# crowsonkb/style_transfer

Hardware: AMD Instinct MI355X
Metric: tile-iterations/sec, VGG-19 2048px/1024-tile (fwd+bwd, Gram/content losses, regularizers, Adam step) (higher is better)
Workload: dtype f32 (fp16x2-split MFMA, fp32 accumulate)

## Files before the change

include/stx.h:

```cpp
#ifndef STX_H_
#define STX_H_

#include <stddef.h>
#include <stdint.h>

#ifdef __cplusplus
extern "C" {
#endif

typedef struct stx_engine stx_engine;

typedef enum stx_status {
    STX_OK = 0,
    STX_ERR_ARG = -1,
    STX_ERR_HIP = -2,
    STX_ERR_STATE = -3,
    STX_ERR_UNSUPPORTED = -4,
    STX_ERR_NOMEM = -5
} stx_status;

typedef enum stx_mem { STX_HOST = 0, STX_DEVICE = 1 } stx_mem;

typedef enum stx_layer_type {
    STX_LAYER_INPUT = 0, STX_LAYER_CONV = 1, STX_LAYER_RELU = 2, STX_LAYER_POOL = 3
} stx_layer_type;

typedef enum stx_pool_mode { STX_POOL_MAX = 0, STX_POOL_AVE = 1 } stx_pool_mode;

typedef struct stx_layer_desc {
    const char *name;
    int type;
    const char *bottom;
    const char *top;
    int num_output;
    int kernel_size;
    int pad;
    int stride;
    int pool_mode;
} stx_layer_desc;

const char *stx_version(void);
const char *stx_last_error(void);
int stx_reread_env(void);
int stx_device_count(int *count);
int stx_device_name(int device, char *buf, size_t buf_len);

int stx_engine_create(int device, const stx_layer_desc *layers, int n_layers, stx_engine **out);
int stx_engine_create_shared(stx_engine *primary, stx_engine **out);
void stx_engine_destroy(stx_engine *e);
int stx_set_conv_weights(stx_engine *e, const char *conv_layer, const float *weights,
                         const float *bias, int mem);
int stx_sync(stx_engine *e);
int stx_fence(stx_engine *e, unsigned long long *ticket);
int stx_fence_wait(stx_engine *e, unsigned long long ticket);
int stx_engine_wait(stx_engine *e, stx_engine *other);
typedef enum stx_query {
    STX_Q_SHARED_ENGINES = 0,
    STX_Q_TARGET_UPLOADS = 1,
    STX_Q_TARGET_BYTES = 2,
    STX_Q_WEIGHT_BYTES = 3,
    STX_Q_TILE_EVALS = 4,
    STX_Q_PEERS_WITHOUT_ACCESS = 5,
    STX_Q_TILE_IO_DIRECT = 6,
    STX_Q_INJECT_SPECIALISED = 7,
    STX_Q_INJECT_VARIANTS = 8
} stx_query;
int stx_engine_query(stx_engine *e, int what, double *value);
int stx_engine_device(stx_engine *e, int *device);
int stx_engine_stream(stx_engine *e, void **hip_stream);

int stx_malloc(stx_engine *e, size_t bytes, void **dev_ptr);
int stx_free(stx_engine *e, void *dev_ptr);
int stx_memset_async(stx_engine *e, void *dev_ptr, int value, size_t bytes);
int stx_memcpy_async(stx_engine *e, void *dst, int dst_mem, const void *src, int src_mem,
                     size_t bytes);

typedef struct stx_content_target {
    int content_index;
    const char *layer;
    int channels, height, width;
    const float *features;
    int mem;
} stx_content_target;

typedef struct stx_style_target {
    int style_index;
    const char *layer;
    int channels;
    const float *gram;
    int mem;
} stx_style_target;

int stx_set_contents_and_styles(stx_engine *e, const stx_content_target *contents, int n_contents,
                                const stx_style_target *styles, int n_styles);

typedef struct stx_style_mask {
    int style_index;
    int H, W;
    const float *mask;
    int mem;
} stx_style_mask;
int stx_set_style_masks(stx_engine *e, const stx_style_mask *masks, int n);

int stx_set_content_mask(stx_engine *e, const float *mask, int H, int W, int mem);

typedef struct stx_stat_target {
    const char *layer;
    int channels;
    const float *mean;
    const float *sd;
    int mem;
    double weight;
} stx_stat_target;
int stx_set_stat_targets(stx_engine *e, const stx_stat_target *targets, int n);

typedef struct stx_nnfm_target {
    const char *layer;
    int channels;
    int rows;
    const float *bank;
    int mem;
    double weight;
} stx_nnfm_target;
int stx_set_nnfm_targets(stx_engine *e, const stx_nnfm_target *targets, int n);

typedef struct stx_nnfm_patch_target {
    const char *layer;
    int channels;
    int patch;
    int rows;
    const float *bank;
    int mem;
    double weight;
} stx_nnfm_patch_target;
int stx_set_nnfm_patch_targets(stx_engine *e, const stx_nnfm_patch_target *targets, int n);

typedef struct stx_nnfm_knn_target {
    const char *layer;
    int channels;
    int patch;
    int k;
    int rows;
    const float *bank;
    int mem;
    double weight;
} stx_nnfm_knn_target;
int stx_set_nnfm_knn_targets(stx_engine *e, const stx_nnfm_knn_target *targets, int n);

typedef struct stx_nnfm_cover_target {
    const char *layer;
    int channels;
    int patch;
    int k;
    int rows;
    const float *bank;
    int mem;
    double weight;
    float cover;
} stx_nnfm_cover_target;
int stx_set_nnfm_cover_targets(stx_engine *e, const stx_nnfm_cover_target *targets, int n);

#define STX_NNFM_MAX_SEGMENTS 8
typedef struct stx_nnfm_guided_target {
    const char *layer;
    int channels;
    int k;
    int segments;
    const int *seg_rows;
    const float *bank;
    int mem;
    double weight;
} stx_nnfm_guided_target;
int stx_set_nnfm_guided_targets(stx_engine *e, const stx_nnfm_guided_target *targets, int n,
                                const float *const *masks, int segments, int H, int W, int mask_mem);

struct stx_swd_target {
    const char *layer;
    int channels;
    int dirs;
    int quantiles;
    const float *V;
    const float *Tq;
    int mem;
    double weight;
};
int stx_set_swd_targets(stx_engine *e, const struct stx_swd_target *targets, int n);

struct stx_selfsim_target {
    const char *layer;
    int points;
    double weight;
};
int stx_set_selfsim_targets(stx_engine *e, const struct stx_selfsim_target *targets, int n);

int stx_features_tile(stx_engine *e, const float *img, int img_mem, int th, int tw,
                      const char *const *layers, int n_layers, float *const *out, int out_mem);

typedef struct stx_tap {
    const char *layer;
    double layer_weight;
    int is_content;
    double content_weight;
    int is_style;
    double style_weight;
    int is_dd;
    double dd_weight;
} stx_tap;

int stx_sc_grad_tile(stx_engine *e, const float *img, int img_mem, int th, int tw,
                     const int roll_xy[2], const int start_yx[2], const stx_tap *taps, int n_taps,
                     double *loss_out, float *grad_out, int grad_mem, int sync_now);

int stx_tile_buffers(stx_engine *e, int th, int tw, float **tile_in, float **grad_out);

int stx_gram_matrix(stx_engine *e, const float *feat, int feat_mem, int channels, int hw,
                    float *gram_out, int gram_mem);

int stx_feature_stats(stx_engine *e, const float *feat, int feat_mem, int channels, int hw,
// ... 145 lines not shown
```

style_transfer_amd/csrc/common.h:

```cpp
#pragma once

#include <hip/hip_runtime.h>

#include <vector>

#include <cstdarg>
#include <cstdio>
#include <functional>
#include <string>

#include "stx.h"

namespace stx {

constexpr float kEps = 1.1920928955078125e-07f;

void set_error(const char *fmt, ...);

const char *sw_env(const char *name);
void sw_reread();

#define STX_HIP(call)                                                                       \
    do {                                                                                    \
        hipError_t err__ = (call);                                                          \
        if (err__ != hipSuccess) {                                                          \
            ::stx::set_error("%s:%d: %s failed: %s", __FILE__, __LINE__, #call,            \
                             hipGetErrorString(err__));                                     \
            return STX_ERR_HIP;                                                             \
        }                                                                                   \
    } while (0)

#define STX_CHECK_LAUNCH()                                                                  \
    do {                                                                                    \
        hipError_t err__ = hipGetLastError();                                               \
        if (err__ != hipSuccess) {                                                          \
            ::stx::set_error("%s:%d: kernel launch failed: %s", __FILE__, __LINE__,        \
                             hipGetErrorString(err__));                                     \
            return STX_ERR_HIP;                                                             \
        }                                                                                   \
    } while (0)

#define STX_TRY(expr)                                                                       \
    do {                                                                                    \
        int rc__ = (expr);                                                                  \
        if (rc__ != STX_OK) return rc__;                                                    \
    } while (0)

inline int ceil_div(int a, int b) { return (a + b - 1) / b; }
inline int pooled_len(int n) { return n >= 2 ? (n - 2 + 1) / 2 + 1 : 1; }
constexpr int kBlocks = 1024;
inline int blocks_for(size_t n) {
    const size_t b = (n + 255) / 256;
    return b < (size_t)kBlocks ? (int)b : kBlocks;
}
#ifdef __HIPCC__
__device__ __forceinline__ float wave_sum_f(float v) {
#pragma unroll
    for (int off = 32; off > 0; off >>= 1) v += __shfl_down(v, off, 64);
    return v;
}

template <int NV>
__device__ __forceinline__ void block_partials(float (&v)[NV], float *partials) {
    __shared__ float red[NV][4];
#pragma unroll
    for (int k = 0; k < NV; ++k) {
        const float s = wave_sum_f(v[k]);
        if ((threadIdx.x & 63) == 0) red[k][threadIdx.x >> 6] = s;
    }
    __syncthreads();
    if (threadIdx.x == 0) {
#pragma unroll
        for (int k = 0; k < NV; ++k)
            partials[k * gridDim.x + blockIdx.x] = red[k][0] + red[k][1] + red[k][2] + red[k][3];
    }
}

__device__ __forceinline__ unsigned pool_max_code(float v00, float v01, float v10, float v11, bool hx,
                                                  bool hy) {
    unsigned arg = 0;
    float best = v00;
    if (hx && v01 > best) best = v01, arg = 1;
    if (hy && v10 > best) best = v10, arg = 2;
    if (hx && hy && v11 > best) best = v11, arg = 3;
    return arg | (best > 0.f ? 4u : 0u);
}
__device__ __forceinline__ unsigned pool_ave_code(float v00, float v01, float v10, float v11, bool hx,
                                                  bool hy) {
    return (v00 > 0.f ? 1u : 0u) | (hx && v01 > 0.f ? 2u : 0u) | (hy && v10 > 0.f ? 4u : 0u) |
           (hx && hy && v11 > 0.f ? 8u : 0u);
}
#endif


enum ConvEpilogue {
    kEpiForward = 0,
    kEpiDgrad = 1,
    kEpiSymm = 2,
    kEpiDgradInject = 3,
    kEpiPartial = 4
};

struct ContentWindow {
    int C, fh, fw;
    int ch, cw;
    int oy, ox;
    int sy, sx;
};

struct ConvInject {
    const float *sgrad = nullptr, *s_abs_sum = nullptr;
    float s_coef = 0.f;
    const float *content = nullptr, *c_sums = nullptr, *feat = nullptr;
    float c_coef = 0.f;
    ContentWindow win{};
};

struct ConvProblem {
    const float *x;
    const float *w;
    float *y;
    const float *bias;
    const float *mask;
    float *partials;
    int K, M, H, W;
    int ksize;
    int relu;
    int epilogue;
    ConvInject inject;
    unsigned char *pool_codes = nullptr;
    unsigned char *in_codes = nullptr;
    const unsigned char *mask_codes = nullptr;
    unsigned char *out_codes = nullptr;
    bool wants_codes = false;
    bool skip_y = false;
    float *pool_out = nullptr;
    int pool_mode = 0;
    float *splitk_ws = nullptr;
    size_t splitk_ws_floats = 0;
    long long *clock_out = nullptr;
    const unsigned *x_amax = nullptr;
    unsigned *y_amax = nullptr;
    const unsigned char *pin_codes = nullptr;
    int pin_mode = 0;
    bool pin_mask = false;
    int *variant_out = nullptr;
#ifdef STX_EXPERIMENT_BF3
    const void *x_split = nullptr;
#endif
};

enum class ConvFamily { Direct, Wino2, H2 };

struct ConvConfig {
    ConvFamily family;
    int id;
    int bm;
    int kc;
    int pr, pc;
    int threads;
    size_t lds_bytes;
};

ConvConfig conv_pick_config(int ksize, int K, int M, int H, int W);
ConvConfig conv_config_by_id(int id);
bool direct_takes_inject(const ConvConfig &cfg);
int conv_num_workgroups(const ConvConfig &cfg, int M, int H, int W);
size_t conv_packed_floats(const ConvConfig &cfg, int K, int M, int ksize);
int conv_pack_weights(hipStream_t s, const float *w_caffe, int Mo, int Ko, int ksize,
                      int transpose_flip, const ConvConfig &cfg, float *packed);
int conv_launch(hipStream_t s, const ConvConfig &cfg, const ConvProblem &p, bool packed_weights);
int direct_splitk_factor(const ConvConfig &cfg, const ConvProblem &p, bool packed_weights);

int splitk_reduce_launch(hipStream_t s, const ConvProblem &p, int ksplit);
int splitk_reduce_items_launch(hipStream_t s, const ConvProblem &p, const ConvConfig &cfg, int slices,
                               int item_base, int items);
__host__ __device__ inline void wino2_item_tiles(int lt, int m_tiles, int n_patches, int &pt, int &mt) {
    pt = lt / m_tiles;
    mt = lt - pt * m_tiles;
    if (m_tiles == 8 && (n_patches & 7) == 0) {
        const int g = lt >> 5, r = lt & 31;
        mt = (g & 1) * 4 + (r & 3);
        pt = (g >> 1) * 8 + (r >> 2);
    }
}

struct WinoArgs {
    const float *x;
    const float *w;
    float *y;
    const float *bias;
    const float *mask;
    int K, M, H, W;
    int n_chunks, tiles_x, tiles_y, m_tiles, ksplit;
    int w_tile_stride;
    int x_bytes, w_bytes;
    int relu;
    ConvInject inj;
    float *pool_out;
    int pool_mode;
    unsigned char *pool_codes;
    int skip_y = 0;
    unsigned char *out_codes = nullptr;
    unsigned char *in_codes = nullptr;
    const unsigned char *mask_codes = nullptr;
    long long *clock_out = nullptr;
    int item_base = 0;
    const unsigned *x_amax = nullptr;
    unsigned *y_amax = nullptr;
    const unsigned char *pin_codes = nullptr;
    int pin_mode = 0, pin_mask = 0;
#ifdef STX_EXPERIMENT_BF3
    int vp_rows = 0, vp_tp = 0;
#endif
};

bool conv_first_usable(int K, int M, int ksize);
int conv_first_workgroups(int H, int W);
int conv_first_launch(hipStream_t s, const float *x, const float *w_caffe, const float *bias, float *y,
                      int K, int H, int W, int relu, float *gram_partials, unsigned *y_amax = nullptr);

ConvConfig wino2_config(int geometry = 0);
int wino2_pick_geometry(int H, int W);
size_t wino2_packed_floats(int K, int M);
int wino2_pack_weights(hipStream_t s, const float *w_caffe, int Mo, int Ko, int transpose_flip,
                       float *packed);
int wino2_launch(hipStream_t s, const ConvConfig &cfg, const ConvProblem &p, int ksplit);
bool wino2_fuses_pool(const ConvProblem &p);
bool wino2_uses_relu_codes(const ConvProblem &p, int ksplit);
bool wino2_writes_out_codes(const ConvConfig &cfg, const ConvProblem &p);
int wino2_splitk_factor(const ConvConfig &cfg, const ConvProblem &p);
struct Wino2Tail { int items, slices; };
Wino2Tail wino2_tail_split(const ConvConfig &cfg, const ConvProblem &p);
int wino2_max_slices(const ConvConfig &cfg, const ConvProblem &p);

constexpr int kAmaxSlots = 64;
ConvConfig h2_config(int mb, int pb = 1);
ConvConfig h2_pick_config(const ConvProblem &p);
bool h2_usable(const ConvProblem &p);
size_t h2_packed_floats(int K, int M);
int h2_pack_weights(hipStream_t s, const float *w_caffe, int Mo, int Ko, int transpose_flip, float *packed);
int h2_launch(hipStream_t s, const ConvConfig &cfg, const ConvProblem &p, int ksplit);
enum { kH2Style = 1, kH2Content = 2, kH2MaskNibbles = 4, kH2MaskBlob = 8 };
int h2_variant(const ConvProblem &p, int pin, bool split);
int h2_launch_variant(hipStream_t s, const WinoArgs &a, int n_wg, int cfg_id, int pin, int var);
int h2_splitk_factor(const ConvConfig &cfg, const ConvProblem &p);
bool h2_fuses_pool(const ConvProblem &p);
bool h2_takes_pooled_input(const ConvConfig &cfg, const ConvProblem &p);
int absmax_launch(hipStream_t s, const float *x, size_t n, unsigned *slots);

size_t conv_small_packed_floats(int K);
int conv_small_pack(hipStream_t s, const float *w_caffe, int Mo, int Ko, int transpose_flip,
                    float *packed);
int conv_small_launch(hipStream_t s, const float *x, const float *packed, float *y,
                      const float *mask, int K, int M, int H, int W);

bool conv_h2_enabled();
struct ConvTuner { int device; hipStream_t stream; hipEvent_t ev0, ev1; std::function<int(const ConvConfig &, const float **)> bank; };
int conv_choose(const ConvProblem &p, bool winograd, const ConvTuner *tuner, ConvConfig *out);
struct ConvBank { int key; size_t floats; std::function<int(hipStream_t, const float *w_caffe, float *packed)> pack; };
ConvBank conv_bank(const ConvConfig &cfg, int dir, int Mo, int Ko, int ksize);
ConvBank conv_small_bank(int Mo, int Ko);
int conv_dispatch(hipStream_t s, const ConvConfig &cfg, const ConvProblem &p, double *flop_algorithmic,
                  double *flop_issued);
int conv_splitk_factor(const ConvConfig &cfg, const ConvProblem &p);
size_t conv_splitk_floats(const ConvConfig &cfg, const ConvProblem &p);
bool conv_takes_clock(const ConvConfig &cfg);
bool conv_fuses_pool(const ConvConfig &cfg, const ConvProblem &p);
bool conv_writes_pool_codes(const ConvConfig &cfg);
bool conv_reads_x_amax(const ConvConfig &cfg);
bool conv_leaves_y_amax(const ConvConfig &cfg);
bool conv_takes_inject(const ConvConfig &cfg);
bool conv_takes_pooled_input(const ConvConfig &cfg, const ConvProblem &p);
bool conv_uses_relu_codes(const ConvConfig &cfg, const ConvProblem &p, int ksplit);
bool conv_writes_out_codes(const ConvConfig &cfg, const ConvProblem &p, int ksplit);

int pool_forward_launch(hipStream_t s, const float *x, int C, int H, int W, int mode, float *y,
                        unsigned char *codes = nullptr);
int pool_backward_codes_launch(hipStream_t s, const float *dy, const unsigned char *codes, int C,
                               int H, int W, int mode, bool relu_mask, float *dx);
int pool_backward_launch(hipStream_t s, const float *dy, const float *x, int C, int H, int W,
                         int mode, bool relu_mask, float *dx);

struct GramPlan {
    int C, HW, splits, tiles;
    int parts;
    size_t partial_floats;
};
GramPlan gram_plan(int C, int HW);
bool gram_h2_usable(const float *feat, int C, int HW);
int gram_partials_launch(hipStream_t s, const float *feat, const GramPlan &plan, float *partials,
                         const unsigned *f_amax = nullptr);
int gram_finish_blocks(const GramPlan &plan);
int gram_finish_launch(hipStream_t s, const float *partials, const GramPlan &plan, float *gram_out,
                       const float *target, float *dsym, float *sumsq, unsigned short *pieces = nullptr,
                       const unsigned *f_amax = nullptr, float *block_out = nullptr);

size_t symm_pieces_elems(int C);
int symm_num_workgroups(int C, int HW);
bool symm_bf3_usable(const float *feat, const float *out, int C, int HW);
bool symm_h2_usable(const float *feat, const float *out, int C, int HW);
int symm_h2_launch(hipStream_t s, const float *feat, const float *dsym, const unsigned *d_amax, int n_damax,
                   const unsigned *f_amax, float *out, float *partials, int C, int HW);
int symm_bf3_launch(hipStream_t s, const float *feat, const float *dsym, unsigned short *pieces,
                    bool pieces_ready, float *out, float *partials, int C, int HW);

#ifdef __HIPCC__
__device__ __forceinline__ int content_origin_y(const ContentWindow &w) { return w.oy - w.sy; }
__device__ __forceinline__ int content_origin_x(const ContentWindow &w) { return w.ox - w.sx; }
__device__ __forceinline__ size_t content_index(const ContentWindow &w, int c, int y, int x) {
    int yy = (content_origin_y(w) + y) % w.ch;
    int xx = (content_origin_x(w) + x) % w.cw;
    if (yy < 0) yy += w.ch;
    if (xx < 0) xx += w.cw;
    return ((size_t)c * w.ch + yy) * w.cw + xx;
}
#endif

struct SumJob {
    const float *src;
    int n;
    float *dst;
};
int sum_jobs_launch(hipStream_t s, const SumJob *jobs, int n_jobs);
int content_sums_launch(hipStream_t s, const float *feat, const float *content,
                        const ContentWindow &win, float *sums , std::vector<SumJob> *defer = nullptr);
int inject_style_launch(hipStream_t s, float *diff, const float *sgrad, size_t n,
                        const float *abs_sum, float coef, bool accumulate, unsigned *y_amax = nullptr);
int inject_content_launch(hipStream_t s, float *diff, const float *feat, const float *content,
                          const ContentWindow &win, const float *sums, float coef, bool accumulate,
                          unsigned *y_amax = nullptr);
int relu_inplace_launch(hipStream_t s, float *x, size_t n);
int sum_partials_launch(hipStream_t s, const float *partials, int n, float *out);
int sum_partials2_launch(hipStream_t s, const float *a, int na, float *out_a, const float *b, int nb,
                         float *out_b);

constexpr int kMaskParts = 1024;
constexpr int kMaskSgradParts = 2048;
int mask_map_launch(hipStream_t s, const float *mask, int H, int W, int scale, float *out);
int mask_apply_launch(hipStream_t s, const float *feat, const float *map, const ContentWindow &win, float *fm,
                      float *m2_partials, int *n_parts);
int mask_target_launch(hipStream_t s, const float *gs, int C, const float *m2_partials, int n_parts, int HW,
                       float *out, float *a_out);
int mask_sgrad_launch(hipStream_t s, float *sgrad, const float *map, const ContentWindow &win, const float *a,
                      float *partials, int *n_parts);

constexpr int kContentMaskParts = 1024;
int content_mask_mean_launch(hipStream_t s, const float *map, const ContentWindow &win, float *a_out);
int content_mask_term_launch(hipStream_t s, const float *feat, const float *content, const float *map,
                             const ContentWindow &win, const float *a, float *sgrad, float *partials,
                             int *n_parts);

constexpr int kStatSlice = 16384;
constexpr float kStatEps = 1e-5f;
int stat_slices(int HW);
size_t stat_scratch_floats(int C, int HW);
int stat_partials_launch(hipStream_t s, const float *feat, int C, int HW, float *partials);
int stat_finish_launch(hipStream_t s, const float *partials, int C, int HW, const float *MU, const float *SD,
                       float *table, float *e_out, float *mean_out, float *sd_out);
int stat_grad_launch(hipStream_t s, const float *feat, int C, int HW, const float *table, float *sgrad,
                     float *abs_partials, int *n_parts);

constexpr int kSwdBlock = 8192;
constexpr int kSwdMaxDirs = 4096, kSwdMaxQuantiles = 65536, kSwdMaxPixels = 1 << 22;
int swd_padded(int n);
int swd_check(const char *who, int C, long long n, int D, int Q);
int swd_e_parts(int n, int D);
size_t swd_scratch_floats(int C, int n, int D);
size_t swd_work_floats(int n, int D);
int swd_project_launch(hipStream_t s, const float *feat, int C, int n, const float *V, int D, void *records);
int swd_sort_launch(hipStream_t s, void *records, int n, int D);
int swd_finish_launch(hipStream_t s, void *records, int n, int D, const float *Tq, int Q, float *G, int *rank_out,
                      float *e_parts);
int swd_sort_passes(int n);
int swd_grad_launch(hipStream_t s, const float *V, const float *G, int C, int n, int D, float *sgrad, float *abs_parts,
                    int *n_parts);
int swd_quantiles_launch(hipStream_t s, const void *records, int n, int D, int Q, float *out);

constexpr int kSelfsimMaxPoints = 4096;
constexpr float kSelfsimEps = 1e-6f;
struct SelfsimGrid {
    int g, gh, gw, N;
};
SelfsimGrid selfsim_grid(int h, int w, int points);
int selfsim_check(const char *who, int C, int points);
struct SelfsimSource {
    const float *p;
    int mh, mw, oy, ox;
};
struct SelfsimScratch {
    float *rows;
    float *inv_r;
    float *D;
    float *col_parts;
    float *u_parts;
    float *q;
    signed char *T;
    float *e_parts;
    float *abs_parts;
    size_t floats;
};
SelfsimScratch selfsim_scratch(float *base, int C, int N);
size_t selfsim_scratch_floats(int C, int N);
int selfsim_prepare_launch(hipStream_t s, const SelfsimSource &feat, const SelfsimSource &content, int C,
                           const SelfsimGrid &gr, const SelfsimScratch &x);
int selfsim_dist_launch(hipStream_t s, int C, int N, const SelfsimScratch &x);
int selfsim_cols_launch(hipStream_t s, int N, const SelfsimScratch &x, signed char *signs, int *n_e);
int selfsim_grad_launch(hipStream_t s, int C, int h, int w, const SelfsimGrid &gr, const SelfsimScratch &x,
                        float *sgrad, int *n_abs);

constexpr int kNnfmQ = 128, kNnfmB = 128, kNnfmK = 32, kNnfmMaxSlices = 64;
constexpr int kNnfmMaxK = 4;
struct NnfmPlan {
    int q_blocks, b_blocks, slices, blocks_per_slice;
};
NnfmPlan nnfm_plan(int n, int M);
size_t nnfm_pieces_floats(int rows, int C);
size_t nnfm_scratch_floats(int C, int n, int M, int patch = 1, int k = 1, bool cover = false);
struct NnfmCover {
    int *winner = nullptr;
    float *part_score = nullptr;
    int *part_idx = nullptr;
    int *cursor = nullptr;
    int *offsets = nullptr;
    int *unordered = nullptr;
    int *list = nullptr;
    float *cprime = nullptr;
    float *e_parts = nullptr;
// ... 140 lines not shown
```

style_transfer_amd/csrc/conv_dispatch.cpp:

```cpp
#include <algorithm>
#include <cstdlib>
#include <cstring>
#include <map>
#include <mutex>

#include "common.h"

namespace stx {

static int h2_min_k(bool forward) {
    const char *env = sw_env("STX_CONV_H2"), *envb = sw_env("STX_CONV_H2_BWD");
    return forward ? (env ? atoi(env) : 64) : envb ? atoi(envb) : env && atoi(env) <= 0 ? 0 : 64;
}

bool conv_h2_enabled() {
    const char *algo = sw_env("STX_CONV_ALGO");
    if (algo && *algo) return !strncmp(algo, "h2", 2);
    return h2_min_k(true) > 0 || h2_min_k(false) > 0;
}

static bool h2_choice(const ConvProblem &p, ConvConfig *out) {
    const char *algo = sw_env("STX_CONV_ALGO");
    int force = 0;
    if (algo && *algo) {
// ... 6 lines not shown
    const int min_k = h2_min_k(p.epilogue == kEpiForward);
    if (!force && (min_k <= 0 || p.K < min_k || p.M < 64)) return false;
    if (!h2_usable(p)) return false;
    *out = force == 1 ? h2_config(1) : force == 2 ? h2_config(2) : force == 3 ? h2_config(1, 2) : h2_pick_config(p);
    return true;
}

static bool wino_choice(const ConvProblem &p, bool winograd, ConvConfig *out) {
    if (p.ksize != 3 || p.K < 8 || p.M <= 4) return false;
    const char *algo = sw_env("STX_CONV_ALGO");
    if (algo && *algo) {
        if (!strcmp(algo, "direct")) return false;
        if (!strcmp(algo, "wino2")) { *out = wino2_config(wino2_pick_geometry(p.H, p.W)); return true; }
        if (!strcmp(algo, "wino2a")) { *out = wino2_config(0); return true; }
        if (!strcmp(algo, "wino2b")) { *out = wino2_config(1); return true; }
        if (!strcmp(algo, "wino2c")) { *out = wino2_config(2); return true; }
    }
    if (!winograd || p.M <= 32) return false;
    *out = wino2_config(wino2_pick_geometry(p.H, p.W));
    return true;
}

static std::mutex g_tuned_mutex;
static std::map<std::vector<int>, int> g_tuned;

static int direct_tune(const ConvTuner &t, ConvProblem p, ConvConfig *out) {
    if (p.ksize != 3 || p.K <= 4 || p.M <= 32) return STX_OK;
    if (conv_splitk_factor(*out, p) > 1 || conv_num_workgroups(conv_config_by_id(5), p.M, p.H, p.W) < 256)
        return STX_OK;
    const std::vector<int> key = {t.device, p.ksize, p.K, p.M, p.H, p.W, p.epilogue};
    {
        std::lock_guard<std::mutex> lock(g_tuned_mutex);
        auto it = g_tuned.find(key);
        if (it != g_tuned.end()) {
            *out = conv_config_by_id(it->second);
            return STX_OK;
        }
    }
    const int candidates[] = {0, 1, 2, 5};
    float best_ms = 1e30f;
    int best = out->id;
    for (int id : candidates) {
        const ConvConfig cfg = conv_config_by_id(id);
        if (cfg.bm > 64 && p.M <= 64) continue;
        STX_TRY(t.bank(cfg, &p.w));
        STX_TRY(conv_launch(t.stream, cfg, p, true));
        STX_HIP(hipEventRecord(t.ev0, t.stream));
        for (int r = 0; r < 2; ++r) STX_TRY(conv_launch(t.stream, cfg, p, true));
        STX_HIP(hipEventRecord(t.ev1, t.stream));
        STX_HIP(hipEventSynchronize(t.ev1));
        float ms = 0.f;
        STX_HIP(hipEventElapsedTime(&ms, t.ev0, t.ev1));
        if (ms < best_ms) {
            best_ms = ms;
            best = id;
        }
    }
    {
        std::lock_guard<std::mutex> lock(g_tuned_mutex);
        g_tuned[key] = best;
    }
    *out = conv_config_by_id(best);
    return STX_OK;
}

int conv_choose(const ConvProblem &p, bool winograd, const ConvTuner *tuner, ConvConfig *out) {
    if (h2_choice(p, out) || wino_choice(p, winograd, out)) return STX_OK;
    *out = conv_pick_config(p.ksize, p.K, p.M, p.H, p.W);
    return tuner ? direct_tune(*tuner, p, out) : STX_OK;
}

enum { kSlotWino2 = 256, kSlotH2 = 512, kSlotSmall = 768 };

ConvBank conv_bank(const ConvConfig &cfg, int dir, int Mo, int Ko, int ks) {
    const int M = dir ? Ko : Mo, K = dir ? Mo : Ko;
    switch (cfg.family) {
        case ConvFamily::Direct:
            return {dir * 1024 + cfg.id, conv_packed_floats(cfg, K, M, ks),
                    [=](hipStream_t s, const float *w, float *out) { return conv_pack_weights(s, w, Mo, Ko, ks, dir, cfg, out); }};
        case ConvFamily::Wino2:
            return {dir * 1024 + kSlotWino2, wino2_packed_floats(K, M),
                    [=](hipStream_t s, const float *w, float *out) { return wino2_pack_weights(s, w, Mo, Ko, dir, out); }};
        case ConvFamily::H2:
            return {dir * 1024 + kSlotH2, h2_packed_floats(K, M),
                    [=](hipStream_t s, const float *w, float *out) { return h2_pack_weights(s, w, Mo, Ko, dir, out); }};
    }
    return {};
}

ConvBank conv_small_bank(int Mo, int Ko) {
    return {1024 + kSlotSmall, conv_small_packed_floats(Mo),
            [=](hipStream_t s, const float *w, float *out) { return conv_small_pack(s, w, Mo, Ko, 1, out); }};
}


int conv_dispatch(hipStream_t s, const ConvConfig &cfg, const ConvProblem &p, double *flop_algorithmic,
                  double *flop_issued) {
    const double direct = 2.0 * p.M * p.K * p.ksize * p.ksize * (double)p.H * p.W;
    *flop_algorithmic += direct;
    switch (cfg.family) {
        case ConvFamily::Direct:
            *flop_issued += direct;
            return conv_launch(s, cfg, p, true);
        case ConvFamily::Wino2:
            *flop_issued += direct * 4.0 / 9.0;
            return wino2_launch(s, cfg, p, conv_splitk_factor(cfg, p));
        case ConvFamily::H2:
            *flop_issued += direct * (6.0 / 9.0) * (3.0 / 16.0);
            return h2_launch(s, cfg, p, conv_splitk_factor(cfg, p));
    }
    return STX_ERR_ARG;
}

int conv_splitk_factor(const ConvConfig &cfg, const ConvProblem &p) {
    if (p.ksize != 3 || (p.epilogue != kEpiForward && p.epilogue != kEpiDgrad)) return 1;
    return cfg.family == ConvFamily::Wino2 ? wino2_splitk_factor(cfg, p)
           : cfg.family == ConvFamily::H2  ? h2_splitk_factor(cfg, p)
                                           : direct_splitk_factor(cfg, p, true);
}

size_t conv_splitk_floats(const ConvConfig &cfg, const ConvProblem &p) {
    int f = conv_splitk_factor(cfg, p);
    if (cfg.family == ConvFamily::Wino2 && p.ksize == 3)
        f = std::max(f, wino2_max_slices(cfg, p));
    return f > 1 ? (size_t)f * p.M * p.H * p.W : 0;
}

bool conv_takes_clock(const ConvConfig &cfg) { return cfg.family != ConvFamily::Direct; }

bool conv_fuses_pool(const ConvConfig &cfg, const ConvProblem &p) {
    const char *env = sw_env("STX_POOL_FWD_FUSE");
    if ((env && atoi(env) == 0) || cfg.family == ConvFamily::Direct || conv_splitk_factor(cfg, p) != 1) return false;
    return cfg.family == ConvFamily::H2 ? h2_fuses_pool(p) : wino2_fuses_pool(p);
}

bool conv_writes_pool_codes(const ConvConfig &cfg) { return cfg.family != ConvFamily::Direct; }

bool conv_reads_x_amax(const ConvConfig &cfg) { return cfg.family == ConvFamily::H2; }

bool conv_leaves_y_amax(const ConvConfig &cfg) {
    return cfg.family == ConvFamily::H2 || (cfg.family == ConvFamily::Wino2 && conv_h2_enabled());
}

bool conv_takes_inject(const ConvConfig &cfg) { return cfg.family != ConvFamily::Direct || direct_takes_inject(cfg); }

bool conv_takes_pooled_input(const ConvConfig &cfg, const ConvProblem &p) {
    return cfg.family == ConvFamily::H2 && h2_takes_pooled_input(cfg, p);
}

bool conv_uses_relu_codes(const ConvConfig &cfg, const ConvProblem &p, int ksplit) {
    return cfg.family == ConvFamily::Wino2 && wino2_uses_relu_codes(p, ksplit);
}

bool conv_writes_out_codes(const ConvConfig &cfg, const ConvProblem &p, int ksplit) {
    const char *env = sw_env("STX_RELU_CODES");
    if ((env && atoi(env) == 0) || cfg.family == ConvFamily::Direct) return false;
    if (p.epilogue != kEpiForward || !p.relu || !p.out_codes || ksplit > 1) return false;
    return cfg.family == ConvFamily::H2 || wino2_writes_out_codes(cfg, p);
}

}
```

style_transfer_amd/csrc/conv_first.hip:

```cpp

#include <algorithm>
#include <cstdlib>

#include "bf16x3.h"
#include "common.h"

namespace stx {

namespace {

constexpr int kFP = 128;
constexpr int kFM = 64;
constexpr int kPW = kFP + 4;
constexpr int kPatch = 12 * kPW;
constexpr int kFLd = kFP + 4;
constexpr int kTile = kFM * kFLd;
constexpr int kNT = 256;
constexpr int kPL = (9 * (kFP + 2) + kNT - 1) / kNT;

typedef float f32x16 __attribute__((ext_vector_type(16)));
typedef float f32x4 __attribute__((ext_vector_type(4)));
typedef unsigned int u32x4f __attribute__((ext_vector_type(4)));

__device__ __forceinline__ int sgpr(int v) { return __builtin_amdgcn_readfirstlane(v); }
__device__ __forceinline__ void lds_barrier() { asm volatile("s_waitcnt lgkmcnt(0)\n\ts_barrier" ::: "memory"); }

struct FirstArgs {
    const float *x;
    const float *w;
    const float *bias;
    float *y;
    float *gram;
    unsigned *y_amax;
    int K, H, W, tiles_x, n_tiles, relu, vec_store, strided;
};

}

template <bool GRAM, int STORE>
__global__ __launch_bounds__(kNT, GRAM ? 2 : 3) void conv_first_kernel(FirstArgs a) {
    constexpr int kWork = 2 * kPatch + kTile;
    static_assert(kFM * kFM <= kWork, "the Gram tile must fit the working set");
    __shared__ __attribute__((aligned(16))) float lds[kWork];
    float *const patch = lds;
    float *const tile = lds + 2 * kPatch;
    const int tid = threadIdx.x, lane = tid & 63;
    const int wave = __builtin_amdgcn_readfirstlane(tid >> 6);
    const int l31 = lane & 31, half = lane >> 5;
    const size_t HW = (size_t)a.H * a.W;

    float aw[2][18];
#pragma unroll
    for (int s = 0; s < 18; ++s) {
        const int c = 2 * (s / 9) + half, tap = s % 9;
#pragma unroll
        for (int mb = 0; mb < 2; ++mb)
            aw[mb][s] = c < a.K ? a.w[((size_t)(mb * 32 + l31) * a.K + c) * 9 + tap] : 0.f;
    }
#pragma unroll
    for (int s = 0; s < 18; ++s) asm volatile("" ::"v"(aw[0][s]), "v"(aw[1][s]));
    float bias_r[2];
#pragma unroll
    for (int mb = 0; mb < 2; ++mb) bias_r[mb] = a.bias ? a.bias[mb * 32 + l31] : 0.f;
    asm volatile("" ::"v"(bias_r[0]), "v"(bias_r[1]));

    const __amdgpu_buffer_rsrc_t rx = __builtin_amdgcn_make_buffer_rsrc(
        const_cast<float *>(a.x), 0, (int)((size_t)a.K * HW * 4), 0x00020000);
    constexpr unsigned kOob = 0x80000000u;
    int p_row[kPL], p_col[kPL], p_off[kPL];
#pragma unroll
    for (int n = 0; n < kPL; ++n) {
        const int e = tid + n * kNT;
        const int pr = e / (kFP + 2), col = e - pr * (kFP + 2);
        const int c = pr / 3, r = pr - 3 * c;
        const bool live = e < 9 * (kFP + 2) && c < a.K;
        p_row[n] = live ? r - 1 : -(1 << 28);
        p_col[n] = col - 1;
        p_off[n] = (c * a.H + r - 1) * a.W + col - 1;
    }
    auto patch_load = [&](int t, float (&preg)[kPL]) {
        const int ty = sgpr(t < 0 ? -4 : t / a.tiles_x);
        const int x0 = sgpr(t < 0 ? 0 : (t - ty * a.tiles_x) * kFP);
        const int origin = sgpr(ty * a.W + x0);
#pragma unroll
        for (int n = 0; n < kPL; ++n) {
            const bool ok = (unsigned)(ty + p_row[n]) < (unsigned)a.H && (unsigned)(x0 + p_col[n]) < (unsigned)a.W;
            const unsigned off = ok ? (unsigned)(origin + p_off[n]) * 4u : kOob;
            preg[n] = __builtin_bit_cast(float, __builtin_amdgcn_raw_buffer_load_b32(rx, off, 0, 0));
        }
    };
    int p_dst[kPL];
#pragma unroll
    for (int n = 0; n < kPL; ++n) {
        const int e = tid + n * kNT;
        const int pr = e / (kFP + 2), col = e - pr * (kFP + 2);
        p_dst[n] = e < 9 * (kFP + 2) ? pr * kPW + col : -1;
    }
    auto patch_store = [&](int buf, const float (&preg)[kPL]) {
#pragma unroll
        for (int n = 0; n < kPL; ++n)
            if (p_dst[n] >= 0) patch[buf * kPatch + p_dst[n]] = preg[n];
    };

    f32x16 g[3];
    if (GRAM) {
#pragma unroll
        for (int b = 0; b < 3; ++b)
#pragma unroll
            for (int r = 0; r < 16; ++r) g[b][r] = 0.f;
    }

    const int per_wg = a.strided ? 1 : (a.n_tiles + (int)gridDim.x - 1) / (int)gridDim.x;
    const int grid = a.strided ? (int)gridDim.x : 1;
    const int t_begin = a.strided ? (int)blockIdx.x : (int)blockIdx.x * per_wg;
    const int t_end = a.strided ? a.n_tiles : (t_begin + per_wg < a.n_tiles ? t_begin + per_wg : a.n_tiles);
    const __amdgpu_buffer_rsrc_t ry = __builtin_amdgcn_make_buffer_rsrc(
        a.y, 0, STORE == 2 ? 0 : (int)(unsigned)((size_t)kFM * HW * 4), 0x00020000);
    constexpr unsigned kOobY = 0xfffffff0u;
    const int y_ch0 = tid >> 5, y_c4 = (tid & 31) * 4;
    const unsigned y_voff = (unsigned)(((size_t)y_ch0 * HW + y_c4) * 4);
    const bool track = a.y_amax != nullptr;
    float amax = 0.f;
    auto segment = [&](int t, int buf, const float (&pin)[kPL], float (&pout)[kPL]) {
        patch_load(t + 2 * grid < t_end ? t + 2 * grid : -1, pout);
        const int ty = sgpr(t / a.tiles_x), x0 = sgpr((t - ty * a.tiles_x) * kFP);

        f32x16 acc[2];
#pragma unroll
        for (int mb = 0; mb < 2; ++mb)
#pragma unroll
            for (int r = 0; r < 16; ++r) acc[mb][r] = 0.f;
        const float *pb = patch + buf * kPatch + half * (3 * kPW) + wave * 32 + l31;
#pragma unroll
        for (int s = 0; s < 18; ++s) {
            const int q = s / 9, ky = (s % 9) / 3, kx = s % 3;
            const float xv = pb[(2 * q * 3 + ky) * kPW + kx];
            acc[0] = __builtin_amdgcn_mfma_f32_32x32x2f32(xv, aw[0][s], acc[0], 0, 0, 0);
            acc[1] = __builtin_amdgcn_mfma_f32_32x32x2f32(xv, aw[1][s], acc[1], 0, 0, 0);
        }
        const bool ragged = x0 + kFP > a.W;
        const int room = a.W - x0 - wave * 32 - 4 * half;
#pragma unroll
        for (int mb = 0; mb < 2; ++mb)
#pragma unroll
            for (int j = 0; j < 4; ++j) {
                f32x4 v = {acc[mb][4 * j], acc[mb][4 * j + 1], acc[mb][4 * j + 2], acc[mb][4 * j + 3]};
                v += bias_r[mb];
                if (a.relu) {
                    v.x = fmaxf(v.x, 0.f), v.y = fmaxf(v.y, 0.f);
                    v.z = fmaxf(v.z, 0.f), v.w = fmaxf(v.w, 0.f);
                }
                if (ragged) {
                    v.x = 8 * j + 0 < room ? v.x : 0.f, v.y = 8 * j + 1 < room ? v.y : 0.f;
                    v.z = 8 * j + 2 < room ? v.z : 0.f, v.w = 8 * j + 3 < room ? v.w : 0.f;
                }
                if (track) amax = fmaxf(fmaxf(amax, fmaxf(fabsf(v.x), fabsf(v.y))), fmaxf(fabsf(v.z), fabsf(v.w)));
                *reinterpret_cast<f32x4 *>(tile + (mb * 32 + l31) * kFLd + wave * 32 + 8 * j + 4 * half) = v;
            }
        lds_barrier();

        {
            float *const yrow = a.y + (size_t)ty * a.W + x0;
            const unsigned origin = (unsigned)sgpr((ty * a.W + x0) * 4);
            const unsigned vo4 = x0 + y_c4 < a.W ? y_voff : kOobY;
#pragma unroll
            for (int n = 0; n < kFM * (kFP / 4) / kNT; ++n) {
                const f32x4 v = *reinterpret_cast<const f32x4 *>(tile + (y_ch0 + 8 * n) * kFLd + y_c4);
                if (STORE == 2) {
                    float *const dst = yrow + (size_t)(y_ch0 + 8 * n) * HW + y_c4;
                    if (x0 + y_c4 + 0 < a.W) dst[0] = v.x;
                    if (x0 + y_c4 + 1 < a.W) dst[1] = v.y;
                    if (x0 + y_c4 + 2 < a.W) dst[2] = v.z;
                    if (x0 + y_c4 + 3 < a.W) dst[3] = v.w;
                    continue;
                }
                const unsigned so = origin + (unsigned)sgpr((int)((unsigned)(8 * n) * (unsigned)HW * 4u));
                if (STORE == 0) {
                    __builtin_amdgcn_raw_buffer_store_b128(__builtin_bit_cast(u32x4f, v), ry, vo4, so, 0);
                } else {
                    const float vs[4] = {v.x, v.y, v.z, v.w};
#pragma unroll
                    for (int i = 0; i < 4; ++i)
                        __builtin_amdgcn_raw_buffer_store_b32(__builtin_bit_cast(unsigned, vs[i]), ry,
                                                              x0 + y_c4 + i < a.W ? y_voff + 4u * i : kOobY, so, 0);
                }
            }
        }
        if (GRAM) {
#pragma unroll
            for (int st = 0; st < 2; ++st) {
                bf16x8 p[2][3];
#pragma unroll
                for (int mb = 0; mb < 2; ++mb) {
                    const float *q = tile + (mb * 32 + l31) * kFLd + wave * 32 + st * 16 + half * 8;
                    const f32x4 lo = *reinterpret_cast<const f32x4 *>(q);
                    const f32x4 hi = *reinterpret_cast<const f32x4 *>(q + 4);
                    const float xv[8] = {lo.x, lo.y, lo.z, lo.w, hi.x, hi.y, hi.z, hi.w};
                    split3_bf16(xv, p[mb][0], p[mb][1], p[mb][2]);
                }
                g[0] = mfma_split6(p[0], p[0], g[0]);
                g[1] = mfma_split6(p[1], p[0], g[1]);
                g[2] = mfma_split6(p[1], p[1], g[2]);
            }
        }
        if (t + grid < t_end) patch_store(buf ^ 1, pin);
        lds_barrier();
    };

    for (int i = tid; i < 2 * kPatch; i += kNT) patch[i] = 0.f;
    lds_barrier();
    float pa[kPL], pb2[kPL];
    const int t0 = t_begin;
    if (t0 < t_end) {
        patch_load(t0, pa);
        patch_store(0, pa);
    }
    if (t0 + grid < t_end) patch_load(t0 + grid, pa);
    lds_barrier();
    for (int t = t0; t < t_end; t += 2 * grid) {
        segment(t, 0, pa, pb2);
        if (t + grid < t_end) segment(t + grid, 1, pb2, pa);
    }

    if (track) {
#pragma unroll
        for (int d = 32; d >= 1; d >>= 1) amax = fmaxf(amax, __shfl_xor(amax, d));
        lds_barrier();
        if (lane == 0) lds[wave] = amax;
        lds_barrier();
        if (tid == 0)
            atomicMax(a.y_amax + (blockIdx.x & (kAmaxSlots - 1)),
                      __builtin_bit_cast(unsigned, fmaxf(fmaxf(lds[0], lds[1]), fmaxf(lds[2], lds[3]))));
    }
    if (GRAM) {
        lds_barrier();
        float *const red = lds;
#pragma unroll 1
        for (int w = 0; w < 4; ++w) {
            if (wave == w) {
#pragma unroll
                for (int r = 0; r < 16; ++r) {
                    const int row = (r & 3) + 8 * (r >> 2) + 4 * half;
                    float *q0 = red + row * kFM + l31, *q1 = red + (32 + row) * kFM + l31;
                    q0[0] = w == 0 ? g[0][r] : q0[0] + g[0][r];
                    if (w == 0) q0[32] = 0.f;
                    q1[0] = w == 0 ? g[1][r] : q1[0] + g[1][r];
                    q1[32] = w == 0 ? g[2][r] : q1[32] + g[2][r];
                }
            }
            lds_barrier();
        }
        float *out = a.gram + (size_t)blockIdx.x * (kFM * kFM);
#pragma unroll
        for (int n = 0; n < 4; ++n) {
            const int e = tid + kNT * n;
            reinterpret_cast<float4 *>(out)[e] = reinterpret_cast<const float4 *>(red)[e];
        }
    }
}

bool conv_first_usable(int K, int M, int ksize) {
    const char *env = sw_env("STX_CONV_FIRST_FUSED");
    if (env && atoi(env) == 0) return false;
    return ksize == 3 && K >= 1 && K <= 3 && M == kFM;
}

int conv_first_workgroups(int H, int W) {
    const long tiles = (long)H * ceil_div(W, kFP);
    return (int)std::min<long>(tiles, 512);
}
static int conv_first_plain_workgroups(int H, int W) {
    const long tiles = (long)H * ceil_div(W, kFP);
    const char *env = sw_env("STX_FIRST_WGS");
    return (int)std::min<long>(tiles, env ? atoi(env) : 768);
}

int conv_first_launch(hipStream_t s, const float *x, const float *w_caffe, const float *bias, float *y,
                      int K, int H, int W, int relu, float *gram_partials, unsigned *y_amax) {
    if (4.0 * K * (double)H * W >= 2147483648.0) {
        set_error("conv_first_launch: a %d x %d plane is beyond the buffer-addressing limit", H, W);
        return STX_ERR_UNSUPPORTED;
    }
    FirstArgs a;
    a.x = x;
    a.w = w_caffe;
    a.bias = bias;
    a.y = y;
    a.gram = gram_partials;
    a.y_amax = y_amax;
    a.K = K;
    a.H = H;
    a.W = W;
    a.tiles_x = ceil_div(W, kFP);
    a.n_tiles = H * a.tiles_x;
    a.relu = relu;
    a.vec_store = W % 4 == 0 && (reinterpret_cast<uintptr_t>(y) & 15) == 0;
    const int grid = gram_partials ? conv_first_workgroups(H, W) : conv_first_plain_workgroups(H, W);
    {
        const char *env = sw_env("STX_FIRST_STRIDED");
        a.strided = env && atoi(env) != 0;
    }
    const int store = 4.0 * kFM * (double)H * W >= 4294967280.0 ? 2 : a.vec_store ? 0 : 1;
#define STX_FIRST(G, S) conv_first_kernel<G, S><<<grid, kNT, 0, s>>>(a)
    if (gram_partials) {
        if (store == 0) STX_FIRST(true, 0);
        else if (store == 1) STX_FIRST(true, 1);
        else STX_FIRST(true, 2);
    } else {
        if (store == 0) STX_FIRST(false, 0);
        else if (store == 1) STX_FIRST(false, 1);
        else STX_FIRST(false, 2);
    }
#undef STX_FIRST
    STX_CHECK_LAUNCH();
    return STX_OK;
}

}
```

style_transfer_amd/csrc/conv_h2.hip:

```cpp

#include <algorithm>
#include <cstdlib>
#include <type_traits>

#include "common.h"
#include "f16x2.h"

#ifndef STX_H2_SKIP
#define STX_H2_SKIP 0
#endif

namespace stx {

namespace {

typedef _Float16 f16x8 __attribute__((ext_vector_type(8)));
typedef float f32x16 __attribute__((ext_vector_type(16)));
typedef float f32x4 __attribute__((ext_vector_type(4)));
typedef float f32x2 __attribute__((ext_vector_type(2)));
typedef unsigned int u32x4 __attribute__((ext_vector_type(4)));
typedef unsigned int u32x3 __attribute__((ext_vector_type(3)));
typedef unsigned int u32x2v __attribute__((__vector_size__(2 * sizeof(unsigned int))));

constexpr int KC = 16;
constexpr int NT = 512;
constexpr int PC = 32, TX = PC / 2;
constexpr int EX_BYTES = 4 * 2 * 4 * 4 * 64 * 16;
template <int PB>
struct Geo {
    static constexpr int PR = 8 * PB;
    static constexpr int XR = PR + 2;
    static constexpr int RT = XR * TX;
    static constexpr int V_PIECE = RT * 32;
    static constexpr int V_BYTES = 4 * 2 * V_PIECE;
    static constexpr int FULL = RT * 4 / 512;
    static constexpr int NU = FULL + 1;
    static constexpr size_t kLds = (EX_BYTES > 2 * V_BYTES ? EX_BYTES : 2 * V_BYTES) + 64;
};
constexpr int FRAG = 1024;
constexpr int U_KY = 4 * 2 * FRAG;
constexpr int U_BLK = 3 * U_KY;
constexpr int kHeaderFloats = 64;

__device__ __forceinline__ int sgpr(int v) { return __builtin_amdgcn_readfirstlane(v); }

template <int I, int N, typename F>
__device__ __forceinline__ void static_for(F &&f) {
    if constexpr (I < N) {
        f(std::integral_constant<int, I>{});
        static_for<I + 1, N>(f);
    }
}

__device__ __forceinline__ void lds_barrier() {
    asm volatile("s_waitcnt lgkmcnt(0)\n\ts_barrier" ::: "memory");
}


}

#ifdef STX_H2_TIMING
__device__ long long g_h2_timing[8][8];
__device__ long long g_h2_epi[8][8];
#define STX_H2_STAMP(i) if (pass == 0) t_epi[i] = clock64()
#else
#define STX_H2_STAMP(i)
#endif

template <int EPI, int MB, int PB, int PIN, int VAR = 0>
__global__ __launch_bounds__(NT) void conv_h2_kernel(WinoArgs a) {
    static_assert(VAR == 0 || EPI == kEpiDgradInject, "variants are of the injecting epilogue");
    static_assert(VAR == 0 || (((VAR & 3) == 1 || (VAR & 3) == 2) && ((VAR >> 2) == 1 || (VAR >> 2) == 2)), "h2_variant's codes");
    const bool inj_style = VAR ? (VAR & 1) != 0 : a.inj.sgrad != nullptr;
    const bool inj_content = VAR ? (VAR & 2) != 0 : a.inj.content != nullptr;
    const bool mask_nibbles = VAR ? (VAR >> 2) == 1 : a.mask_codes != nullptr;
    const bool mask_blob = VAR ? (VAR >> 2) == 2 : !a.mask_codes && a.mask;
    using G = Geo<PB>;
    [[maybe_unused]] constexpr int PR = G::PR, RT = G::RT, V_PIECE = G::V_PIECE, V_BYTES = G::V_BYTES, NU = G::NU, FULL = G::FULL;
    constexpr size_t kLdsBytes = G::kLds;
    constexpr int NJ = 4 * PB;
    extern __shared__ __attribute__((aligned(16))) char ldsb[];
#ifdef STX_H2_TIMING
    const long long t_start = clock64(), w_start = wall_clock64();
#endif
    constexpr int BM = 64 * MB;

    const int tid = threadIdx.x, lane = tid & 63;
    const int wave = sgpr(tid >> 6);
    const int xi = wave & 3, wh = wave >> 2;
    const int l31 = lane & 31, half = lane >> 5;

    const int m_tiles = a.m_tiles, a_tiles_x = a.tiles_x, a_tiles_y = a.tiles_y, a_H = a.H, a_W = a.W;
    const int a_n_chunks = a.n_chunks, a_ksplit = a.ksplit, a_item_base = a.item_base, a_x_bytes = a.x_bytes,
              a_w_bytes = a.w_bytes;
    const float *const a_x = a.x, *const a_w = a.w;
    asm volatile("" ::"s"(m_tiles), "s"(a_tiles_x), "s"(a_tiles_y), "s"(a_H), "s"(a_W), "s"(a_n_chunks), "s"(a_ksplit),
                 "s"(a_item_base), "s"(a_x_bytes), "s"(a_w_bytes), "s"(a_x), "s"(a_w));
    const int nb = gridDim.x, xcd = blockIdx.x & 7, slot_x = blockIdx.x >> 3;
    const int q8 = nb >> 3, r8 = nb & 7;
    const int L = (xcd < r8 ? xcd * (q8 + 1) : r8 * (q8 + 1) + (xcd - r8) * q8) + slot_x;
    const int kslice = sgpr(EPI == kEpiPartial ? L % a_ksplit : 0);
    const int Lt = sgpr(EPI == kEpiPartial ? a_item_base + L / a_ksplit : L);
    int ptile, mtile;
    wino2_item_tiles(Lt, m_tiles, a_tiles_x * a_tiles_y, ptile, mtile);
    ptile = sgpr(ptile);
    mtile = sgpr(mtile);
    const int c_begin = sgpr(EPI == kEpiPartial ? 2 * (kslice * (a_n_chunks >> 1) / a_ksplit) : 0);
    const int c_end = sgpr(EPI == kEpiPartial ? 2 * ((kslice + 1) * (a_n_chunks >> 1) / a_ksplit) : a_n_chunks);
    const int y0 = sgpr((ptile / a_tiles_x) * PR);
    const int x0 = sgpr((ptile % a_tiles_x) * PC);
    const int m0 = mtile * BM;
    const int HW = a_H * a_W;
    const unsigned HW4 = (unsigned)HW * 4u;
    const int pih = (a_H + 1) >> 1, piw = (a_W + 1) >> 1;
    const unsigned XP4 = PIN ? (unsigned)(pih * piw) * 4u : HW4;

    constexpr unsigned kOob = 0x80000000u;
    const __amdgpu_buffer_rsrc_t rx = __builtin_amdgcn_make_buffer_rsrc(
        const_cast<float *>(a_x), 0, a_x_bytes, 0x00020000);
    const __amdgpu_buffer_rsrc_t rw = __builtin_amdgcn_make_buffer_rsrc(
        const_cast<float *>(a_w), 0, a_w_bytes, 0x00020000);
    const __amdgpu_buffer_rsrc_t rcx = __builtin_amdgcn_make_buffer_rsrc(
        const_cast<unsigned char *>(a.pin_codes), 0, PIN ? (a_x_bytes >> 2) + 3 : 0, 0x00020000);

    float sv = 0.f, out_scale = 0.f, out_scale2 = 0.f;
    auto read_scales = [&]() __attribute__((always_inline)) {
        typedef const __attribute__((address_space(4))) unsigned *kconst_u32;
        const kconst_u32 slots = (kconst_u32)(uintptr_t)a.x_amax, header = (kconst_u32)(uintptr_t)a_w;
        unsigned amax_bits = 0;
#pragma unroll
        for (int i = 0; i < kAmaxSlots; ++i) amax_bits = max(amax_bits, slots[i]);
        const int es = sgpr(h2_scale_exp(amax_bits));
        const int ew = sgpr((int)header[(a_w_bytes >> 2) + 1]);
        sv = pow2f(es);
        const int eo = -es - ew, eo1 = eo < -126 ? -126 : eo > 127 ? 127 : eo;
        out_scale = pow2f(eo1), out_scale2 = pow2f(eo - eo1);
    };

    const bool edge = x0 == 0 || x0 + PC + 2 > a.W;
    unsigned xvoff[NU], v_dst[NU];
    bool left[NU], ok2[NU], ok3[NU];
#pragma unroll
    for (int n = 0; n < NU; ++n) {
        const int u = tid + n * NT;
        const int rt = n < FULL ? u >> 2 : 128 * FULL + (tid >> 4);
        const int ch0 = n < FULL ? (u & 3) * 4 : tid & 15;
        const int st_r = rt / TX, st_t = rt % TX;
        const int st_y = y0 - 1 + st_r, st_x = x0 + 2 * st_t - 1;
        left[n] = st_x < 0;
        ok2[n] = st_x + 2 < a.W, ok3[n] = st_x + 3 < a.W;
        xvoff[n] = kOob;
        if (PIN) {
            const int w0 = (x0 >> 1) + st_t - 1;
            if ((unsigned)st_y < (unsigned)a.H && st_x + 1 < a.W)
                xvoff[n] = (unsigned)(ch0 * pih * piw + (st_y >> 1) * piw + (left[n] ? 0 : w0)) * 4u +
                           (unsigned)(st_y & 1) + ((st_y | 1) < a.H ? 2u : 0u);
        } else if ((unsigned)st_y < (unsigned)a.H && st_x + 1 < a.W)
            xvoff[n] = (unsigned)(ch0 * HW + st_y * a.W + (left[n] ? 0 : st_x)) * 4u;
        v_dst[n] = (unsigned)(rt * 32 + ((ch0 * 2) ^ ((st_t & 8) << 1)));
    }

    f32x4 xr[FULL][4], xe;
    auto x_fetch = [&](int n, unsigned soff) __attribute__((always_inline)) {
        if constexpr (PIN) {
            unsigned xo = xvoff[n];
            asm volatile("" : "+v"(xo));
            const u32x3 g = __builtin_amdgcn_raw_buffer_load_b96(rx, xo & ~3u, soff, 0);
            const unsigned cw = __builtin_amdgcn_raw_buffer_load_b32(rcx, xo >> 2, soff >> 2, 0);
            return __builtin_bit_cast(f32x4, u32x4{g.x, g.y, g.z, cw});
        } else {
            return __builtin_bit_cast(f32x4, __builtin_amdgcn_raw_buffer_load_b128(rx, xvoff[n], soff, 0));
        }
    };
    auto x_load = [&](int n, int chunk) __attribute__((always_inline)) {
        const unsigned xs = (unsigned)sgpr(chunk * KC) * XP4;
        if (n == FULL) {
            xe = x_fetch(FULL, xs);
        } else {
#pragma unroll
            for (int i = 0; i < 4; ++i) xr[n][i] = x_fetch(n, xs + (unsigned)i * XP4);
        }
    };
    auto border = [&](f32x4 d, int n) __attribute__((always_inline)) {
        f32x4 e;
        e.x = left[n] ? 0.f : d.x;
        e.y = left[n] ? d.x : d.y;
        e.z = left[n] ? d.y : d.z;
        e.w = left[n] ? d.z : d.w;
        e.z = ok2[n] ? e.z : 0.f;
        e.w = ok3[n] ? e.w : 0.f;
        return e;
    };
    struct Unpool {
        unsigned cmask, t_l, t_r, sh;
        float q0;
        bool ok4;
    };
    auto unpool_setup = [&](int n) __attribute__((always_inline)) {
        Unpool r;
        const unsigned keep = a.pin_mask ? 4u : 0u;
        r.cmask = keep | 3u;
        unsigned xo = xvoff[n], vd = v_dst[n];
        asm volatile("" : "+v"(xo), "+v"(vd));
        r.sh = (xo & 1u) << 1;
        r.t_l = keep | r.sh, r.t_r = r.t_l | 1u;
        r.q0 = (xo & 2u) ? 0.25f : 0.5f;
        r.ok4 = x0 + 2 * (int)((vd >> 5) & 15u) + 3 < a.W;
        return r;
    };
    auto unpool_channel = [&](f32x4 d, int n, const Unpool &r, bool fix) __attribute__((always_inline)) {
        constexpr bool is_max = PIN == 1 + STX_POOL_MAX;
        float g0 = d.x, g1 = d.y, g2 = d.z;
        const float dw = d.w;
        unsigned cw = __builtin_bit_cast(unsigned, dw);
        if (fix) {
            g2 = left[n] ? g1 : g2, g1 = left[n] ? g0 : g1;
            cw = left[n] ? cw << 8 : cw;
        }
        float p0, p1, p2, p3;
        if (is_max) {
            const unsigned b0 = cw & r.cmask, b1 = (cw >> 8) & r.cmask, b2 = (cw >> 16) & r.cmask;
            p0 = b0 == r.t_r ? g0 : 0.f;
            p1 = b1 == r.t_l ? g1 : 0.f;
            p2 = b1 == r.t_r ? g1 : 0.f;
            p3 = b2 == r.t_l ? g2 : 0.f;
        } else {
            const float q1 = fix && !ok2[n] ? r.q0 + r.q0 : r.q0, q2 = fix && !r.ok4 ? r.q0 + r.q0 : r.q0;
// ... 22 lines not shown
            __builtin_amdgcn_sched_barrier(0);
        }
    };
    auto component = [](f32x4 d, int c) __attribute__((always_inline)) {
        return c == 0 ? d.x - d.z : c == 1 ? d.y + d.z : c == 2 ? d.z - d.y : d.y - d.w;
    };
    auto piece = [&](int n, int c, char *vbuf, bool fix) __attribute__((always_inline)) {
        if (!PIN && c == 0 && fix) {
            asm volatile("");
#pragma unroll
            for (int i = 0; i < 4; ++i) xr[n][i] = border(xr[n][i], n);
        }
        float v[4];
#pragma unroll
        for (int i = 0; i < 4; ++i) v[i] = component(xr[n][i], c);
        unsigned h0, h1, l0, l1;
        if (STX_H2_SKIP & 64) {
            h0 = __builtin_bit_cast(unsigned, v[0]), h1 = __builtin_bit_cast(unsigned, v[1]);
            l0 = __builtin_bit_cast(unsigned, v[2]), l1 = __builtin_bit_cast(unsigned, v[3]);
        } else {
            asm("v_fma_mixlo_f16 %0, %4, %8, 0\n\t"
                "v_fma_mixhi_f16 %0, %5, %8, 0\n\t"
                "v_fma_mixlo_f16 %1, %6, %8, 0\n\t"
                "v_fma_mixhi_f16 %1, %7, %8, 0\n\t"
                "v_fma_mixlo_f16 %2, %4, %8, -%0 op_sel:[0,0,0] op_sel_hi:[0,0,1]\n\t"
                "v_fma_mixhi_f16 %2, %5, %8, -%0 op_sel:[0,0,1] op_sel_hi:[0,0,1]\n\t"
                "v_fma_mixlo_f16 %3, %6, %8, -%1 op_sel:[0,0,0] op_sel_hi:[0,0,1]\n\t"
                "v_fma_mixhi_f16 %3, %7, %8, -%1 op_sel:[0,0,1] op_sel_hi:[0,0,1]"
                : "=&v"(h0), "=&v"(h1), "=&v"(l0), "=&v"(l1)
                : "v"(v[0]), "v"(v[1]), "v"(v[2]), "v"(v[3]), "v"(sv));
        }
        if (STX_H2_SKIP & 32) {
            asm volatile("" :: "v"(h0), "v"(h1), "v"(l0), "v"(l1));
            return;
        }
        *reinterpret_cast<u32x2v *>(vbuf + v_dst[n] + (c * 2 + 0) * V_PIECE) = u32x2v{h0, h1};
        *reinterpret_cast<u32x2v *>(vbuf + v_dst[n] + (c * 2 + 1) * V_PIECE) = u32x2v{l0, l1};
    };
    auto piece_one = [&](int c, char *vbuf, bool fix) __attribute__((always_inline)) {
        if (!PIN && c == 0 && fix) {
            asm volatile("");
            xe = border(xe, FULL);
        }
        const float va = component(xe, c), vb = component(xe, c + 1);
        unsigned ha, hb, la, lb;
        asm("v_fma_mixlo_f16 %0, %4, %6, 0\n\t"
            "v_fma_mixlo_f16 %1, %5, %6, 0\n\t"
            "v_fma_mixlo_f16 %2, %4, %6, -%0 op_sel:[0,0,0] op_sel_hi:[0,0,1]\n\t"
            "v_fma_mixlo_f16 %3, %5, %6, -%1 op_sel:[0,0,0] op_sel_hi:[0,0,1]"
            : "=&v"(ha), "=&v"(hb), "=&v"(la), "=&v"(lb)
            : "v"(va), "v"(vb), "v"(sv));
        if (STX_H2_SKIP & 32) {
            asm volatile("" :: "v"(ha), "v"(hb), "v"(la), "v"(lb));
            return;
        }
        char *dst = vbuf + v_dst[FULL];
        *reinterpret_cast<unsigned short *>(dst + (c * 2 + 0) * V_PIECE) = (unsigned short)ha;
        *reinterpret_cast<unsigned short *>(dst + (c * 2 + 1) * V_PIECE) = (unsigned short)la;
        *reinterpret_cast<unsigned short *>(dst + (c * 2 + 2) * V_PIECE) = (unsigned short)hb;
        *reinterpret_cast<unsigned short *>(dst + (c * 2 + 3) * V_PIECE) = (unsigned short)lb;
    };
    auto stage_all = [&](int n, int buf) __attribute__((always_inline)) {
        char *vbuf = ldsb + buf * V_BYTES;
        if (PIN) unpool(n, edge);
        if (n == FULL) {
            piece_one(0, vbuf, edge);
            piece_one(2, vbuf, edge);
        } else {
#pragma unroll
            for (int c = 0; c < 4; ++c) piece(n, c, vbuf, edge);
        }
    };

    const unsigned a_voff = (unsigned)(xi * 2 * FRAG + lane * 16);
    const unsigned w_blk0 = (unsigned)(mtile * 2 * MB + wh * MB);
    constexpr bool LEAN = MB * PB == 2;
    f16x8 af[LEAN ? 2 : 3][MB][2];
    auto a_load = [&](int aslot, int ky, int chunk) __attribute__((always_inline)) {
#pragma unroll
        for (int b = 0; b < MB; ++b) {
            const unsigned ws = (unsigned)sgpr(
                (int)(((w_blk0 + b) * (unsigned)a.n_chunks + (unsigned)chunk) * U_BLK + (unsigned)ky * U_KY));
#pragma unroll
            for (int q = 0; q < 2; ++q)
                af[aslot][b][q] = __builtin_bit_cast(
                    f16x8, __builtin_amdgcn_raw_buffer_load_b128(rw, a_voff + q * FRAG, ws, 0));
        }
    };

    f32x16 acc[MB][NJ];
#pragma unroll
    for (int b = 0; b < MB; ++b)
#pragma unroll
        for (int j = 0; j < NJ; ++j)
#pragma unroll
            for (int r = 0; r < 16; ++r) acc[b][j][r] = 0.f;

    const unsigned b_base = (unsigned)(xi * 2 * V_PIECE + ((l31 >> 4) * 2 * TX + (l31 & 15)) * 32 +
                                       ((half * 16) ^ ((l31 & 8) << 1)));
    f16x8 bq[2][2];
    auto b_read = [&](int slot, int buf, int blk) __attribute__((always_inline)) {
        const int j = blk % NJ, ky = blk / NJ;
        const char *vb = ldsb + buf * V_BYTES + b_base + (4 * (j >> 1) + (j & 1) + ky) * TX * 32;
#pragma unroll
        for (int q = 0; q < 2; ++q) bq[slot][q] = *reinterpret_cast<const f16x8 *>(vb + q * V_PIECE);
    };

#ifdef STX_H2_TIMING
    const long long t_p0 = clock64();
#endif
    static_for<0, NU>([&](auto n_c) __attribute__((always_inline)) { x_load(decltype(n_c)::value, c_begin); });
    if (LEAN) {
        a_load(0, 0, c_begin);
    } else {
#pragma unroll
        for (int ky = 0; ky < 3; ++ky) a_load(ky, ky, c_begin);
    }
    __builtin_amdgcn_sched_barrier(0);
    read_scales();
#pragma unroll
    for (int b = 0; b < MB; ++b)
#pragma unroll
        for (int j = 0; j < NJ; ++j) asm volatile("" : "+v"(acc[b][j]));
    float s_scale = 0.f, c_scale = 0.f;
    if (EPI == kEpiDgradInject) {
        const float n = (float)((size_t)a.M * HW);
        if (inj_style) s_scale = a.inj.s_coef * (1.0f / (a.inj.s_abs_sum[0] / n + kEps));
        if (inj_content) c_scale = a.inj.c_coef * (1.0f / (a.inj.c_sums[1] / n + kEps));
    }
    const int hh = wave & 1, mrow = (wave >> 1) & 1, rqp = wave >> 2;
    const bool weven = (a.W & 1) == 0;
    const int xx0 = x0 + 2 * (l31 & 15);
    const unsigned plane_bytes = (unsigned)a.M * HW4;
    const __amdgpu_buffer_rsrc_t ry = __builtin_amdgcn_make_buffer_rsrc(
        a.y + (EPI == kEpiPartial ? (size_t)kslice * a.M * HW : 0), 0, (int)plane_bytes, 0x00020000);
    const __amdgpu_buffer_rsrc_t rmask = __builtin_amdgcn_make_buffer_rsrc(
        const_cast<float *>(a.mask), 0, a.mask ? (int)plane_bytes : 0, 0x00020000);
    const __amdgpu_buffer_rsrc_t rsg = __builtin_amdgcn_make_buffer_rsrc(
        const_cast<float *>(a.inj.sgrad), 0, a.inj.sgrad ? (int)plane_bytes : 0, 0x00020000);
    const __amdgpu_buffer_rsrc_t rft = __builtin_amdgcn_make_buffer_rsrc(
        const_cast<float *>(a.inj.feat), 0, a.inj.feat ? (int)plane_bytes : 0, 0x00020000);
    const __amdgpu_buffer_rsrc_t rbias = __builtin_amdgcn_make_buffer_rsrc(
        const_cast<float *>(a.bias), 0, a.bias ? a.M * 4 : 0, 0x00020000);
    const int ph = (a.H + 1) >> 1, pw = (a.W + 1) >> 1;
    const __amdgpu_buffer_rsrc_t rpool = __builtin_amdgcn_make_buffer_rsrc(
        a.pool_out, 0, a.pool_out ? a.M * ph * pw * 4 : 0, 0x00020000);
    const __amdgpu_buffer_rsrc_t rcodes = __builtin_amdgcn_make_buffer_rsrc(
        a.pool_codes, 0, a.pool_codes ? a.M * ph * pw : 0, 0x00020000);
    const int cph = (a.H + 1) >> 1, cpw = (a.W + 1) >> 1;
    const __amdgpu_buffer_rsrc_t rmc = __builtin_amdgcn_make_buffer_rsrc(
        const_cast<unsigned char *>(a.mask_codes), 0, a.mask_codes ? a.M * cph * cpw : 0, 0x00020000);
    const __amdgpu_buffer_rsrc_t roc = __builtin_amdgcn_make_buffer_rsrc(
        a.out_codes, 0, a.out_codes ? a.M * cph * cpw : 0, 0x00020000);
    const int M_ = a.M;
    struct LaneRows {
        int yy;
        unsigned vo[2][2], vpool, vmc;
    };
    const float *const content = a.inj.content;
    const int cw_ch = a.inj.win.ch, cw_cw = a.inj.win.cw, cw_oy = a.inj.win.oy - a.inj.win.sy,
              cw_ox = a.inj.win.ox - a.inj.win.sx;
    auto lane_rows = [&](int pbi) __attribute__((always_inline)) {
        LaneRows r;
        r.yy = y0 + 8 * pbi + 4 * mrow + 2 * (l31 >> 4);
        const unsigned lane_base = (unsigned)((4 * half) * HW + r.yy * a.W + xx0) * 4u;
#pragma unroll
        for (int y = 0; y < 2; ++y)
#pragma unroll
            for (int e = 0; e < 2; ++e)
                r.vo[y][e] = (r.yy + y < a.H && xx0 + e < a.W) ? lane_base + (unsigned)(y * a.W + e) * 4u : kOob;
        const bool in = r.yy < a.H && xx0 < a.W;
        r.vpool = in ? (unsigned)((4 * half) * ph * pw + (r.yy >> 1) * pw + (xx0 >> 1)) * 4u : kOob;
        r.vmc = in ? (unsigned)((4 * half) * cph * cpw + (r.yy >> 1) * cpw + (xx0 >> 1)) : kOob;
        return r;
    };
    constexpr bool HOIST = !(PIN && PB == 2);
    LaneRows rows0{};
    if (HOIST) rows0 = lane_rows(0);
    auto ld2 = [&](const __amdgpu_buffer_rsrc_t &rs, const LaneRows &lr, int y, unsigned so, auto even_c)
                   __attribute__((always_inline)) {
        if (decltype(even_c)::value)
            return __builtin_bit_cast(f32x2, __builtin_amdgcn_raw_buffer_load_b64(rs, lr.vo[y][0], so, 0));
        f32x2 v;
        v.x = __builtin_bit_cast(float, __builtin_amdgcn_raw_buffer_load_b32(rs, lr.vo[y][0], so, 0));
        v.y = __builtin_bit_cast(float, __builtin_amdgcn_raw_buffer_load_b32(rs, lr.vo[y][1], so, 0));
        return v;
    };
    auto st2 = [&](const __amdgpu_buffer_rsrc_t &rs, const LaneRows &lr, int y, unsigned so, f32x2 v, auto even_c)
                   __attribute__((always_inline)) {
        if (STX_H2_SKIP & 8) {
            if (v.x == 1.2345e-30f) __builtin_amdgcn_raw_buffer_store_b32(0u, rs, lr.vo[y][0], so, 0);
            return;
        }
        if (decltype(even_c)::value) {
            __builtin_amdgcn_raw_buffer_store_b64(__builtin_bit_cast(u32x2v, v), rs, lr.vo[y][0], so, 0);
        } else {
            const float v0 = v.x, v1 = v.y;
            __builtin_amdgcn_raw_buffer_store_b32(__builtin_bit_cast(unsigned, v0), rs, lr.vo[y][0], so, 0);
            __builtin_amdgcn_raw_buffer_store_b32(__builtin_bit_cast(unsigned, v1), rs, lr.vo[y][1], so, 0);
        }
    };
    int ccol[2] = {0, 0};
    auto content_columns = [&](const LaneRows &lr) __attribute__((always_inline)) {
        if (EPI == kEpiDgradInject && inj_content) {
#pragma unroll
            for (int e = 0; e < 2; ++e) {
                const bool ok = lr.yy < a.H && xx0 < a.W;
                const int x = ok ? (xx0 + e < a.W ? xx0 + e : xx0) : (e && 1 < a.W ? 1 : 0);
                int r = (cw_ox + x) % cw_cw;
                ccol[e] = r < 0 ? r + cw_cw : r;
            }
        }
    };
    if (HOIST) content_columns(rows0);
#ifdef STX_H2_TIMING
    __builtin_amdgcn_sched_barrier(0);
    const long long t_p1 = clock64();
    asm volatile("s_waitcnt vmcnt(0)" ::: "memory");
    const long long t_p2 = clock64();
#endif
    static_for<0, NU>([&](auto n_c) __attribute__((always_inline)) {
        constexpr int n = decltype(n_c)::value;
        stage_all(n, 0);
        if (c_begin + 1 < c_end) x_load(n, c_begin + 1);
    });
#ifdef STX_H2_TIMING
    __builtin_amdgcn_sched_barrier(0);
    const long long t_p3 = clock64();
#endif
    lds_barrier();
    b_read(0, 0, 0);

    constexpr int NBLK = 3 * NJ;
    constexpr int PER_BLK = 3 * MB, SLOTS = (NBLK - 1) * PER_BLK;
    constexpr int NQ = PIN ? 5 : 4, NQ1 = PIN ? 3 : 2;
    constexpr int NP = NQ * NU;
    constexpr int STEP = (SLOTS - 2) / NP;
#ifdef STX_H2_NO_BRANCH
    const bool edge_fix = false;
#else
    const bool edge_fix = edge;
#endif
    auto run_chunk = [&](auto buf_c, int chunk, auto more_c) __attribute__((always_inline)) {
        constexpr bool MORE = decltype(more_c)::value;
        constexpr int BUF = decltype(buf_c)::value, buf = BUF;
        char *vnext = ldsb + (buf ^ 1) * V_BYTES;
        static_for<0, NBLK>([&](auto blk_c) __attribute__((always_inline)) {
            constexpr int blk = decltype(blk_c)::value;
            constexpr int ky = blk / NJ, j = blk % NJ, slot = blk & 1;
            if (blk == NBLK - 1) {
                __builtin_amdgcn_sched_barrier(0);
                lds_barrier();
            }
            __builtin_amdgcn_sched_barrier(0);
            if (blk < NBLK - 1) b_read(slot ^ 1, buf, blk + 1);
            else if (MORE) b_read(0, buf ^ 1, 0);
            static_for<0, PER_BLK>([&](auto m_c) __attribute__((always_inline)) {
                constexpr int m = decltype(m_c)::value;
                constexpr int b = m % MB, t = m / MB;
                __builtin_amdgcn_sched_barrier(0);
                constexpr int as = LEAN ? (BUF + ky) & 1 : ky;
                acc[b][j] = __builtin_amdgcn_mfma_f32_32x32x16_f16(af[as][b][t == 0 ? 1 : 0],
                                                                   bq[slot][t == 1 ? 1 : 0], acc[b][j], 0, 0, 0);
                __builtin_amdgcn_sched_barrier(0);
                constexpr int s = blk * PER_BLK + m;
                if (LEAN && j == 0 && m == 0 && !(STX_H2_SKIP & 2)) {
                    if (ky < 2) a_load(as ^ 1, ky + 1, chunk);
                    else if (MORE) a_load(as ^ 1, 0, chunk + 1);
                }
                if (MORE && !(STX_H2_SKIP & 1) && s >= 1 && (s - 1) % STEP == 0) {
                    constexpr int k = (s - 1) / STEP;
                    constexpr int n = k % NU, q = k / NU;
                    if (k < NP && PIN && q == 0) unpool(n, edge_fix);
                    else if (k < NP && n < FULL) piece(n, q - (PIN ? 1 : 0), vnext, edge_fix);
                    else if (k < NP && q < NQ1) piece_one(2 * (q - (PIN ? 1 : 0)), vnext, edge_fix);
                }
                if (MORE && !(STX_H2_SKIP & 4)) {
                    static_for<0, NU>([&](auto u_c) __attribute__((always_inline)) {
                        constexpr int u = decltype(u_c)::value;
                        if (s == 1 + (((u < FULL ? NQ : NQ1) - 1) * NU + u) * STEP + 1 && chunk + 2 < c_end)
                            x_load(u, chunk + 2);
                    });
                }
            });
            if (!LEAN && j == NJ - 1 && MORE && !(STX_H2_SKIP & 2)) a_load(ky, ky, chunk + 1);
        });
        __builtin_amdgcn_sched_barrier(0);
    };
    using yes = std::integral_constant<bool, true>;
    using no = std::integral_constant<bool, false>;
    using b0 = std::integral_constant<int, 0>;
    using b1 = std::integral_constant<int, 1>;
#ifdef STX_H2_TIMING
    const long long t_loop = clock64(), w_loop = wall_clock64();
#endif
    const bool mark = a.clock_out != nullptr && (int)blockIdx.x == (int)(gridDim.x >> 1);
    long long mark_c = 0, mark_w = 0;
    if (mark) {
        mark_c = clock64();
        mark_w = wall_clock64();
    }
    {
        int chunk = c_begin;
        for (; chunk + 2 < c_end; chunk += 2) {
            run_chunk(b0{}, chunk, yes{});
            run_chunk(b1{}, chunk + 1, yes{});
        }
        run_chunk(b0{}, chunk, yes{});
        run_chunk(b1{}, chunk + 1, no{});
    }
    if (mark) {
        const long long dc = clock64() - mark_c, dw = wall_clock64() - mark_w;
        if (tid == 0) {
            a.clock_out[0] = dw >= 100 ? dc : 0;
            a.clock_out[1] = dw >= 100 ? dw : 0;
        }
    }
#ifdef STX_H2_TIMING
    const long long t_end = clock64(), w_end = wall_clock64();
#endif

    float amax = 0.f;
    f32x4 *ex = reinterpret_cast<f32x4 *>(ldsb);

#ifdef STX_H2_TIMING
    long long t_epi[4] = {0, 0, 0, 0};
#endif
    auto epilogue_pass = [&](auto pass_c, auto even_c) __attribute__((always_inline)) {
        constexpr int pass = decltype(pass_c)::value;
        constexpr int mbi = pass % MB, pbi = pass / MB;
        const LaneRows lr = pbi == 0 && HOIST ? rows0 : lane_rows(pbi);
        if (!HOIST && pass == 0) content_columns(lr);
        int crow[2] = {0, 0};
        if (EPI == kEpiDgradInject && inj_content) {
#pragma unroll
            for (int y = 0; y < 2; ++y) {
                const bool ok = lr.yy + y < a.H && xx0 < a.W;
                int q = (cw_oy + (ok ? lr.yy + y : 0)) % cw_ch;
                crow[y] = (q < 0 ? q + cw_ch : q) * cw_cw;
            }
        }
        const int cblk = m0 + (hh * MB + mbi) * 32;
        auto chan = [&](int n) __attribute__((always_inline)) {
            const int c0 = cblk + (n & 3) + 8 * (2 * rqp + (n >> 2));
            return sgpr(c0 < M_ ? c0 : M_);
        };
        float bs[8];
        f32x2 mk[16], sg[16];
        unsigned mkb[8];
#pragma unroll
        for (int n = 0; n < 8; ++n) {
            const int c = chan(n);
            const unsigned so = (unsigned)c * HW4;
            if (EPI == kEpiForward) {
                bs[n] = a.bias ? __builtin_bit_cast(float, __builtin_amdgcn_raw_buffer_load_b32(
                                                               rbias, (unsigned)half * 16u, (unsigned)c * 4u, 0))
                               : 0.f;
            } else if (EPI != kEpiPartial) {
                if (mask_nibbles) mkb[n] = __builtin_amdgcn_raw_buffer_load_b8(rmc, lr.vmc, (unsigned)(c * cph * cpw), 0);
#pragma unroll
                for (int y = 0; y < 2; ++y) {
                    if (mask_blob && !(STX_H2_SKIP & 16)) mk[2 * n + y] = ld2(rmask, lr, y, so, even_c);
                    if (EPI == kEpiDgradInject && inj_style) sg[2 * n + y] = ld2(rsg, lr, y, so, even_c);
                }
            }
        }
        STX_H2_STAMP(0);
        __syncthreads();
        STX_H2_STAMP(1);
#pragma unroll
        for (int j = 0; j < 4; ++j)
#pragma unroll
            for (int rq = 0; rq < 4; ++rq)
                ex[(((xi * 2 + wh) * 4 + j) * 4 + rq) * 64 + lane] =
                    f32x4{acc[mbi][4 * pbi + j][4 * rq], acc[mbi][4 * pbi + j][4 * rq + 1],
                          acc[mbi][4 * pbi + j][4 * rq + 2], acc[mbi][4 * pbi + j][4 * rq + 3]};
        __syncthreads();
        STX_H2_STAMP(2);
#pragma unroll
        for (int rqi = 0; rqi < 2; ++rqi) {
            const int rq = 2 * rqp + rqi;
            f32x4 o[2][2];
#pragma unroll
            for (int s = 0; s < 2; ++s) {
                f32x4 p[4];
#pragma unroll
                for (int c = 0; c < 4; ++c) p[c] = ex[(((c * 2 + hh) * 4 + 2 * mrow + s) * 4 + rq) * 64 + lane];
                o[s][0] = (p[0] + p[1] + p[2]) * out_scale * out_scale2;
                o[s][1] = (p[1] - p[2] - p[3]) * out_scale * out_scale2;
            }
#pragma unroll
            for (int e = 0; e < 4; ++e) {
                const int n = 4 * rqi + e;
                const int c = chan(n);
                const unsigned so = (unsigned)c * HW4;
                f32x2 v[2];
#pragma unroll
                for (int y = 0; y < 2; ++y) v[y] = f32x2{o[y][0][e], o[y][1][e]};
                if (EPI == kEpiForward) {
                    if (a.bias) {
#pragma unroll
                        for (int y = 0; y < 2; ++y) v[y].x += bs[n], v[y].y += bs[n];
                    }
                    if (a.relu) {
#pragma unroll
                        for (int y = 0; y < 2; ++y) v[y].x = fmaxf(v[y].x, 0.f), v[y].y = fmaxf(v[y].y, 0.f);
                    }
                } else if (EPI != kEpiPartial) {
#pragma unroll
                    for (int y = 0; y < 2; ++y) {
                        if (mask_nibbles) {
                            const unsigned nib = mkb[n] >> (2 * y);
                            v[y].x = (nib & 1u) ? v[y].x : 0.f;
                            v[y].y = (nib & 2u) ? v[y].y : 0.f;
                        } else if (mask_blob && !(STX_H2_SKIP & 16)) {
                            v[y].x = mk[2 * n + y].x > 0.f ? v[y].x : 0.f;
                            v[y].y = mk[2 * n + y].y > 0.f ? v[y].y : 0.f;
                        }
                        if (EPI == kEpiDgradInject) {
                            if (inj_content) {
                                const f32x2 ft = ld2(rft, lr, y, so, even_c);
                                const int mm = c + 4 * half;
                                const int cm = mm < a.M ? mm : 0;
                                const float *cp = content + (size_t)cm * cw_ch * cw_cw + crow[y];
                                v[y].x += c_scale * (ft.x - cp[ccol[0]]);
                                v[y].y += c_scale * (ft.y - cp[ccol[1]]);
                            }
                            if (inj_style) {
                                v[y].x += s_scale * sg[2 * n + y].x;
                                v[y].y += s_scale * sg[2 * n + y].y;
                            }
                        }
                    }
                }
#pragma unroll
                for (int y = 0; y < 2; ++y) {
                    if (EPI != kEpiForward || !a.skip_y) st2(ry, lr, y, so, v[y], even_c);
                    if (EPI != kEpiPartial)
                        amax = fmaxf(amax, fmaxf(lr.vo[y][0] != kOob ? fabsf(v[y].x) : 0.f,
                                                 lr.vo[y][1] != kOob ? fabsf(v[y].y) : 0.f));
                }
                if (EPI == kEpiForward && a.out_codes) {
                    const unsigned nib = (lr.vo[0][0] != kOob && v[0].x > 0.f ? 1u : 0u) |
                                         (lr.vo[0][1] != kOob && v[0].y > 0.f ? 2u : 0u) |
                                         (lr.vo[1][0] != kOob && v[1].x > 0.f ? 4u : 0u) |
                                         (lr.vo[1][1] != kOob && v[1].y > 0.f ? 8u : 0u);
                    __builtin_amdgcn_raw_buffer_store_b8((unsigned char)nib, roc, lr.vmc, (unsigned)(c * cph * cpw), 0);
                }
                if (EPI == kEpiForward && a.pool_out) {
                    const bool hy = lr.yy + 1 < a.H, hx = decltype(even_c)::value || xx0 + 1 < a.W;
                    float pr;
                    if (a.pool_mode == STX_POOL_MAX) {
                        pr = hx ? fmaxf(v[0].x, v[0].y) : v[0].x;
                        if (hy) pr = hx ? fmaxf(fmaxf(pr, v[1].x), v[1].y) : fmaxf(pr, v[1].x);
                    } else {
                        pr = (v[0].x + (hx ? v[0].y : 0.f) + (hy ? v[1].x : 0.f) + (hx && hy ? v[1].y : 0.f)) *
                             (hy ? (hx ? 0.25f : 0.5f) : (hx ? 0.5f : 1.0f));
                    }
                    __builtin_amdgcn_raw_buffer_store_b32(__builtin_bit_cast(unsigned, pr), rpool, lr.vpool,
                                                          (unsigned)c * (unsigned)(ph * pw * 4), 0);
                    if (a.pool_codes) {
                        const unsigned code = a.pool_mode == STX_POOL_MAX
                                                  ? pool_max_code(v[0].x, v[0].y, v[1].x, v[1].y, hx, hy)
                                                  : pool_ave_code(v[0].x, v[0].y, v[1].x, v[1].y, hx, hy);
                        __builtin_amdgcn_raw_buffer_store_b8((unsigned char)code, rcodes, lr.vpool >> 2,
                                                             (unsigned)c * (unsigned)(ph * pw), 0);
                    }
                }
            }
        }
    };
    static_for<0, MB * PB>([&](auto pass_c) __attribute__((always_inline)) {
        [[maybe_unused]] constexpr int pass = decltype(pass_c)::value;
        if (weven) epilogue_pass(pass_c, yes{});
        else epilogue_pass(pass_c, no{});
        STX_H2_STAMP(3);
    });
    if (EPI != kEpiPartial && a.y_amax) {
#pragma unroll
        for (int d = 32; d >= 1; d >>= 1) amax = fmaxf(amax, __shfl_xor(amax, d));
        float *wmax = reinterpret_cast<float *>(ldsb + kLdsBytes - 64);
        if (lane == 0) wmax[wave] = amax;
        __syncthreads();
        if (tid == 0) {
#pragma unroll
            for (int w = 1; w < 8; ++w) amax = fmaxf(amax, wmax[w]);
            atomicMax(a.y_amax + (blockIdx.x & (kAmaxSlots - 1)), __builtin_bit_cast(unsigned, amax));
        }
    }
#ifdef STX_H2_TIMING
    if (blockIdx.x == gridDim.x - 3 && lane == 0) {
        g_h2_timing[wave][0] = t_loop - t_start, g_h2_timing[wave][1] = t_end - t_loop;
        g_h2_timing[wave][2] = clock64() - t_end;
        g_h2_timing[wave][3] = w_loop - w_start, g_h2_timing[wave][4] = w_end - w_loop;
        g_h2_timing[wave][5] = wall_clock64() - w_end;
        for (int i = 0; i < 4; ++i) g_h2_epi[wave][i] = t_epi[i] - t_end;
        g_h2_epi[wave][4] = t_p0 - t_start, g_h2_epi[wave][5] = t_p1 - t_p0, g_h2_epi[wave][6] = t_p2 - t_p1, g_h2_epi[wave][7] = t_p3 - t_p2;
    }
#endif
}

template <int EPI, int MB, int PB, int PIN = 0, int VAR = 0>
static int h2_launch_epi(hipStream_t s, const WinoArgs &args, int n_wg) {
    auto kern = conv_h2_kernel<EPI, MB, PB, PIN, VAR>;
    constexpr size_t kLdsBytes = Geo<PB>::kLds;
    hipError_t e = hipFuncSetAttribute(reinterpret_cast<const void *>(kern),
                                       hipFuncAttributeMaxDynamicSharedMemorySize, (int)kLdsBytes);
    if (e != hipSuccess) {
        set_error("hipFuncSetAttribute(lds=%zu): %s", kLdsBytes, hipGetErrorString(e));
        return STX_ERR_HIP;
    }
    kern<<<n_wg, NT, kLdsBytes, s>>>(args);
    STX_CHECK_LAUNCH();
    return STX_OK;
}

#if defined(STX_H2_VARIANTS_ONLY) || !(defined(STX_H2_SPLIT_UNITS) || defined(STX_H2_DEV_SUBSET))
int h2_launch_variant(hipStream_t s, const WinoArgs &a, int n_wg, int cfg_id, int pin, int var) {
#define STX_H2_VAR(V, P)                                                                                      \
    if (var == (V) && pin == (P))                                                                             \
        return cfg_id == 1   ? h2_launch_epi<kEpiDgradInject, 2, 1, P, V>(s, a, n_wg)                         \
               : cfg_id == 2 ? h2_launch_epi<kEpiDgradInject, 1, 2, P, V>(s, a, n_wg)                         \
                             : h2_launch_epi<kEpiDgradInject, 1, 1, P, V>(s, a, n_wg);
    STX_H2_VAR(kH2Style | kH2MaskNibbles, 0)
    STX_H2_VAR(kH2Style | kH2MaskBlob, 0)
    STX_H2_VAR(kH2Content | kH2MaskNibbles, 0)
    STX_H2_VAR(kH2Content | kH2MaskBlob, 0)
    STX_H2_VAR(kH2Style | kH2MaskNibbles, 1 + STX_POOL_MAX)
    STX_H2_VAR(kH2Style | kH2MaskBlob, 1 + STX_POOL_MAX)
    STX_H2_VAR(kH2Style | kH2MaskNibbles, 1 + STX_POOL_AVE)
    STX_H2_VAR(kH2Style | kH2MaskBlob, 1 + STX_POOL_AVE)
#undef STX_H2_VAR
    set_error("h2_launch_variant: no specialised body %d for a pooled input of kind %d", var, pin);
    return STX_ERR_UNSUPPORTED;
}
#endif
#ifndef STX_H2_VARIANTS_ONLY

__global__ __launch_bounds__(256) void absmax_kernel(const float *__restrict__ x, size_t n, unsigned *slots) {
    float m = 0.f;
    const size_t head = ((16 - (reinterpret_cast<size_t>(x) & 15)) & 15) >> 2;
    const size_t h = head < n ? head : n;
    const size_t n4 = (n - h) >> 2;
    const f32x4 *x4 = reinterpret_cast<const f32x4 *>(x + h);
    for (size_t i = blockIdx.x * (size_t)256 + threadIdx.x; i < n4; i += (size_t)gridDim.x * 256) {
        const f32x4 v = x4[i];
        m = fmaxf(fmaxf(m, fmaxf(fabsf(v.x), fabsf(v.y))), fmaxf(fabsf(v.z), fabsf(v.w)));
    }
    if (blockIdx.x == 0) {
        if (threadIdx.x < h) m = fmaxf(m, fabsf(x[threadIdx.x]));
        const size_t tail = h + (n4 << 2);
        if (tail + threadIdx.x < n && threadIdx.x < 4) m = fmaxf(m, fabsf(x[tail + threadIdx.x]));
    }
#pragma unroll
    for (int d = 32; d >= 1; d >>= 1) m = fmaxf(m, __shfl_xor(m, d));
    __shared__ float wmax[4];
    if ((threadIdx.x & 63) == 0) wmax[threadIdx.x >> 6] = m;
    __syncthreads();
    if (threadIdx.x == 0)
        atomicMax(slots + (blockIdx.x & (kAmaxSlots - 1)),
                  __builtin_bit_cast(unsigned, fmaxf(fmaxf(wmax[0], wmax[1]), fmaxf(wmax[2], wmax[3]))));
}

int absmax_launch(hipStream_t s, const float *x, size_t n, unsigned *slots) {
    STX_HIP(hipMemsetAsync(slots, 0, kAmaxSlots * sizeof(unsigned), s));
    if ((reinterpret_cast<size_t>(x) & 3) != 0) {
        set_error("absmax_launch: the array is not float-aligned");
        return STX_ERR_ARG;
    }
    const int blocks = (int)std::min<size_t>((n / 4 + 2047) / 2048 + 1, 1024);
    absmax_kernel<<<blocks, 256, 0, s>>>(x, n, slots);
    STX_CHECK_LAUNCH();
    return STX_OK;
}

size_t h2_packed_floats(int K, int M) {
    return (size_t)ceil_div(M, 32) * ceil_div(K, KC) * (U_BLK / 4) + kHeaderFloats;
}

__device__ __forceinline__ float h2_u(const float *__restrict__ w, int Ko, int transpose_flip, int m, int k,
                                      int ky, int x) {
    float g[3];
#pragma unroll
    for (int b = 0; b < 3; ++b) {
        const int t = ky * 3 + b;
        g[b] = transpose_flip ? w[((size_t)k * Ko + m) * 9 + (8 - t)] : w[((size_t)m * Ko + k) * 9 + t];
    }
    return x == 0 ? g[0] : x == 1 ? (g[0] + g[1] + g[2]) * 0.5f : x == 2 ? (g[0] - g[1] + g[2]) * 0.5f : g[2];
}

__global__ void h2_bank_max_kernel(const float *__restrict__ w, int Ko, int transpose_flip, int M, int K,
                                   unsigned *header) {
    const size_t total = (size_t)M * K * 12;
    float mx = 0.f;
    for (size_t idx = blockIdx.x * (size_t)blockDim.x + threadIdx.x; idx < total;
         idx += (size_t)gridDim.x * blockDim.x) {
        const int x = idx % 4, ky = (idx / 4) % 3;
        const size_t mk = idx / 12;
        mx = fmaxf(mx, fabsf(h2_u(w, Ko, transpose_flip, (int)(mk / K), (int)(mk % K), ky, x)));
    }
#pragma unroll
    for (int d = 32; d >= 1; d >>= 1) mx = fmaxf(mx, __shfl_xor(mx, d));
    __shared__ float wmax[4];
    if ((threadIdx.x & 63) == 0) wmax[threadIdx.x >> 6] = mx;
    __syncthreads();
    if (threadIdx.x == 0)
        atomicMax(header, __builtin_bit_cast(unsigned, fmaxf(fmaxf(wmax[0], wmax[1]), fmaxf(wmax[2], wmax[3]))));
}

__global__ void h2_pack_kernel(const float *__restrict__ w, int Ko, int transpose_flip, int M, int K,
                               int n_chunks, unsigned short *__restrict__ packed, size_t total,
                               unsigned *header) {
    const int ew = h2_scale_exp(header[0]);
    const float sw = pow2f(ew);
    if (blockIdx.x == 0 && threadIdx.x == 0) header[1] = (unsigned)ew;
    for (size_t idx = blockIdx.x * (size_t)blockDim.x + threadIdx.x; idx < total;
         idx += (size_t)gridDim.x * blockDim.x) {
        size_t r = idx;
        const int e = r % 8; r /= 8;
        const int l31 = r % 32; r /= 32;
        const int half = r % 2; r /= 2;
        const int piece = r % 2; r /= 2;
        const int x = r % 4; r /= 4;
        const int ky = r % 3; r /= 3;
        const int chunk = r % n_chunks;
        const int mblk = r / n_chunks;
        const int m = mblk * 32 + l31, k = chunk * KC + half * 8 + e;
        _Float16 out = (_Float16)0.f;
        if (m < M && k < K) {
            const float u = h2_u(w, Ko, transpose_flip, m, k, ky, x) * sw;
            const _Float16 hi = (_Float16)u;
            out = piece == 0 ? hi : (_Float16)(u - (float)hi);
        }
        packed[idx] = __builtin_bit_cast(unsigned short, out);
    }
}

int h2_pack_weights(hipStream_t s, const float *w_caffe, int Mo, int Ko, int transpose_flip, float *packed) {
    const int M = transpose_flip ? Ko : Mo;
    const int K = transpose_flip ? Mo : Ko;
    const size_t bank_floats = h2_packed_floats(K, M) - kHeaderFloats;
    unsigned *header = reinterpret_cast<unsigned *>(packed + bank_floats);
    STX_HIP(hipMemsetAsync(header, 0, kHeaderFloats * sizeof(float), s));
    h2_bank_max_kernel<<<(int)std::min<size_t>(((size_t)M * K * 12 + 255) / 256, 256), 256, 0, s>>>(
        w_caffe, Ko, transpose_flip, M, K, header);
    STX_CHECK_LAUNCH();
    const size_t total = bank_floats * 2;
    h2_pack_kernel<<<(int)std::min<size_t>((total + 255) / 256, 8192), 256, 0, s>>>(
        w_caffe, Ko, transpose_flip, M, K, ceil_div(K, KC), reinterpret_cast<unsigned short *>(packed), total,
        header);
    STX_CHECK_LAUNCH();
    return STX_OK;
}

ConvConfig h2_config(int mb, int pb) {
    const bool two = mb != 2 && pb == 2;
    return {ConvFamily::H2, mb == 2 ? 1 : two ? 2 : 0, mb == 2 ? 128 : 64, KC, two ? 16 : 8, PC, NT,
            two ? Geo<2>::kLds : Geo<1>::kLds};
}

bool h2_usable(const ConvProblem &p) {
    if (p.ksize != 3 || p.K % (2 * KC) != 0 || p.K < 2 * KC) return false;
    if (p.epilogue != kEpiForward && p.epilogue != kEpiDgrad) return false;
    if (p.epilogue == kEpiForward && (p.wants_codes || p.in_codes)) return false;
    const double xb = 4.0 * p.K * (double)p.H * p.W, yb = 4.0 * p.M * (double)p.H * p.W;
    const double wb = 4.0 * (double)h2_packed_floats(p.K, p.M);
    return xb < 2147483648.0 && yb < 2147483648.0 && wb < 2147483648.0;
}

static double h2_plan(const ConvConfig &cfg, const ConvProblem &p, int *factor) {
    const int n_pairs = p.K / (2 * KC);
    const long n = (long)ceil_div(p.M, cfg.bm) * ceil_div(p.H, cfg.pr) * ceil_div(p.W, PC);
    const double out_mb = 4e-6 * p.M * (double)p.H * p.W;
    const double t_chunk = cfg.id == 1 ? 2.75 : cfg.id == 2 ? 3.5 : 2.0, t_fixed = cfg.id != 0 ? 17.0 : 8.5;
    const bool may_split = p.epilogue == kEpiForward || p.epilogue == kEpiDgrad;
    double best_cost = 0;
    int best = 1;
    for (int f = 1; f <= 8 && (f == 1 || (may_split && n_pairs / f >= 2)); ++f) {
        const double rounds = (double)ceil_div((int)std::min<long>(n * f, 1 << 30), 256);
        double c = rounds * (2.0 * ceil_div(n_pairs, f) * t_chunk + t_fixed);
        if (f > 1) c += (f + 1) * out_mb / 3.0 + 5.0;
        if (f == 1 || c < best_cost) {
            best_cost = c;
            best = f;
        }
    }
    *factor = best;
    return best_cost;
}

int h2_splitk_factor(const ConvConfig &cfg, const ConvProblem &p) {
    int f;
    h2_plan(cfg, p, &f);
    return f;
}

ConvConfig h2_pick_config(const ConvProblem &p) {
    int f;
    ConvConfig best = h2_config(1, 1);
    double best_cost = h2_plan(best, p, &f);
    const ConvConfig cand[2] = {h2_config(2, 1), h2_config(1, 2)};
    for (int i = 0; i < 2; ++i) {
        if (i == 0 && p.M % 128 != 0) continue;
        const double c = h2_plan(cand[i], p, &f);
        if (c < best_cost) best_cost = c, best = cand[i];
    }
    return best;
}

bool h2_takes_pooled_input(const ConvConfig &cfg, const ConvProblem &p) {
    return p.epilogue == kEpiDgrad && h2_usable(p) && h2_splitk_factor(cfg, p) == 1;
}

bool h2_fuses_pool(const ConvProblem &p) {
    return p.pool_out && p.epilogue == kEpiForward && (((size_t)p.y | (size_t)p.pool_out) & 7) == 0;
}

#ifdef STX_H2_DEV_SUBSET
template __global__ void conv_h2_kernel<0, 2, 1, 0>(WinoArgs);
template __global__ void conv_h2_kernel<0, 1, 2, 0>(WinoArgs);
template __global__ void conv_h2_kernel<1, 2, 1, 0>(WinoArgs);
template __global__ void conv_h2_kernel<3, 2, 1, 0>(WinoArgs);
template __global__ void conv_h2_kernel<3, 1, 2, 1>(WinoArgs);
template __global__ void conv_h2_kernel<3, 2, 1, 0, kH2Style | kH2MaskNibbles>(WinoArgs);
template __global__ void conv_h2_kernel<3, 2, 1, 0, kH2Content | kH2MaskNibbles>(WinoArgs);
template __global__ void conv_h2_kernel<3, 1, 2, 1, kH2Style | kH2MaskBlob>(WinoArgs);
template __global__ void conv_h2_kernel<3, 2, 1, 1, kH2Style | kH2MaskNibbles>(WinoArgs);
#else
int h2_variant(const ConvProblem &p, int pin, bool split) {
    if (split || p.epilogue != kEpiDgrad) return 0;
    const bool style = p.inject.sgrad != nullptr, content = p.inject.content != nullptr;
    if (style == content) return 0;
    if (!p.mask_codes && !p.mask) return 0;
    if (content && pin) return 0;
    const char *env = sw_env("STX_H2_INJECT_GENERIC");
    if (env && atoi(env) != 0) return 0;
    return (style ? kH2Style : kH2Content) | (p.mask_codes ? kH2MaskNibbles : kH2MaskBlob);
}

int h2_launch(hipStream_t s, const ConvConfig &cfg, const ConvProblem &p, int ksplit) {
    if (!h2_usable(p) || !p.x_amax) {
        set_error("h2_launch: unsupported problem (K %d, epilogue %d, input maximum %s)", p.K, p.epilogue,
                  p.x_amax ? "given" : "missing");
        return STX_ERR_UNSUPPORTED;
    }
    WinoArgs a;
    a.x = p.x;
    a.w = p.w;
    a.y = p.y;
    a.bias = p.bias;
    a.mask = p.mask;
    a.K = p.K;
    a.M = p.M;
    a.H = p.H;
    a.W = p.W;
    a.n_chunks = p.K / KC;
    a.tiles_x = ceil_div(p.W, PC);
    a.tiles_y = ceil_div(p.H, cfg.pr);
    a.m_tiles = ceil_div(p.M, cfg.bm);
    a.ksplit = 1;
    a.w_tile_stride = 0;
    a.relu = p.relu;
    a.inj = p.inject;
    a.pool_out = nullptr;
    a.pool_codes = nullptr;
    a.pool_mode = p.pool_mode;
    a.x_bytes = (int)(4.0 * p.K * (double)p.H * p.W);
    const bool pin = p.pin_codes != nullptr;
    if (pin) {
        if (!h2_takes_pooled_input(cfg, p) || ksplit > 1) {
            set_error("h2_launch: a pooled input goes with unsplit backward launches only");
            return STX_ERR_UNSUPPORTED;
        }
        a.x_bytes = (int)(4.0 * p.K * (double)((p.H + 1) / 2) * ((p.W + 1) / 2));
        a.pin_codes = p.pin_codes;
        a.pin_mode = p.pin_mode;
        a.pin_mask = p.pin_mask ? 1 : 0;
    }
    a.w_bytes = (int)(4 * (h2_packed_floats(p.K, p.M) - kHeaderFloats));
    a.clock_out = p.clock_out;
    a.x_amax = p.x_amax;
    a.y_amax = p.y_amax;
    a.mask_codes = p.epilogue == kEpiDgrad ? p.mask_codes : nullptr;
    a.out_codes = p.epilogue == kEpiForward && p.relu ? p.out_codes : nullptr;
    const bool inject = p.epilogue == kEpiDgrad && (p.inject.sgrad || p.inject.content);
    int n_wg = a.m_tiles * a.tiles_x * a.tiles_y;
    const bool split = ksplit > 1 && p.splitk_ws && p.splitk_ws_floats >= (size_t)ksplit * p.M * p.H * p.W;
    if (split) {
        a.ksplit = ksplit;
        a.y = p.splitk_ws;
        a.y_amax = nullptr;
        a.mask_codes = nullptr;
        a.out_codes = nullptr;
        n_wg *= ksplit;
    } else if (h2_fuses_pool(p)) {
        a.pool_out = p.pool_out;
        a.pool_codes = p.pool_codes;
        a.skip_y = p.skip_y && p.pool_codes != nullptr;
    }
    const int epi = split ? kEpiPartial : inject ? kEpiDgradInject : p.epilogue;
    const int pin_kind = pin ? 1 + p.pin_mode : 0;
    const int var = h2_variant(p, pin_kind, split);
    if (p.variant_out) *p.variant_out = var;
    if (var) return h2_launch_variant(s, a, n_wg, cfg.id, pin_kind, var);
#define STX_H2_CASE(E)                                                                   \
    case E:                                                                              \
        STX_TRY(cfg.id == 1   ? (h2_launch_epi<E, 2, 1>(s, a, n_wg))                   \
                : cfg.id == 2 ? (h2_launch_epi<E, 1, 2>(s, a, n_wg))                   \
                                : (h2_launch_epi<E, 1, 1>(s, a, n_wg)));                 \
        break;
#define STX_H2_PIN_CASE(E, P)                                                            \
    case E:                                                                              \
        STX_TRY(cfg.id == 1   ? (h2_launch_epi<E, 2, 1, P>(s, a, n_wg))                \
                : cfg.id == 2 ? (h2_launch_epi<E, 1, 2, P>(s, a, n_wg))                \
                                : (h2_launch_epi<E, 1, 1, P>(s, a, n_wg)));              \
        break;
    if (pin && p.pin_mode == STX_POOL_MAX) {
        switch (epi) {
            STX_H2_PIN_CASE(kEpiDgrad, 1 + STX_POOL_MAX)
            STX_H2_PIN_CASE(kEpiDgradInject, 1 + STX_POOL_MAX)
        }
        return STX_OK;
    }
    if (pin) {
        switch (epi) {
            STX_H2_PIN_CASE(kEpiDgrad, 1 + STX_POOL_AVE)
            STX_H2_PIN_CASE(kEpiDgradInject, 1 + STX_POOL_AVE)
        }
        return STX_OK;
    }
#undef STX_H2_PIN_CASE
    switch (epi) {
        STX_H2_CASE(kEpiForward)
        STX_H2_CASE(kEpiDgrad)
        STX_H2_CASE(kEpiDgradInject)
        STX_H2_CASE(kEpiPartial)
        default:
            set_error("h2_launch: no kernel for epilogue %d", p.epilogue);
            return STX_ERR_UNSUPPORTED;
    }
#undef STX_H2_CASE
    return split ? splitk_reduce_launch(s, p, ksplit) : STX_OK;
}
#endif
#endif

}
```

style_transfer_amd/csrc/engine.cpp:

```cpp

#include <algorithm>
#include <atomic>
#include <cstdlib>
#include <cstring>

#include "engine.h"

namespace stx {

static thread_local std::string g_error;

void set_error(const char *fmt, ...) {
    char buf[1024];
    va_list ap;
    va_start(ap, fmt);
    vsnprintf(buf, sizeof buf, fmt, ap);
    va_end(ap);
    g_error = buf;
}

int alloc_scalars(stx_engine *e, size_t n, size_t *index) {
    stx_engine::ScalarArena &a = e->A();
    if (a.used + n > e->scalars_cap) {
        set_error("scalar arena exhausted (%zu + %zu > %zu)", a.used, n, e->scalars_cap);
// ... 194 lines not shown
        return (int)e->blobs.size() - 1;
    };
    for (int i = 0; i < n_layers; ++i) {
        const stx_layer_desc &d = layers[i];
        Layer L;
        L.name = d.name ? d.name : "";
        L.bottom = d.bottom ? d.bottom : "";
        L.top = d.top ? d.top : "";
        L.type = d.type;
        L.num_output = d.num_output;
        L.ksize = d.kernel_size;
        L.pad = d.pad;
        L.stride = d.stride;
        L.pool_mode = d.pool_mode;
        if (L.top.empty()) {
            set_error("layer %d (%s) has no top blob", i, L.name.c_str());
            return STX_ERR_ARG;
        }
        if (i == 0) {
            L.top_blob = add_blob(L.top, d.num_output > 0 ? d.num_output : 3, 0);
        } else {
            auto it = e->blob_index.find(L.bottom);
            if (it == e->blob_index.end()) {
                set_error("layer %s: unknown bottom blob '%s'", L.name.c_str(), L.bottom.c_str());
                return STX_ERR_ARG;
            }
            L.bottom_blob = it->second;
            if (L.type == STX_LAYER_RELU) {
                if (L.top != L.bottom) {
                    set_error("layer %s: only in-place ReLU is supported", L.name.c_str());
                    return STX_ERR_UNSUPPORTED;
                }
                L.top_blob = L.bottom_blob;
                e->blobs[L.top_blob].relu = true;
            } else if (L.type == STX_LAYER_CONV) {
                if (!((L.ksize == 3 && L.pad == 1) || (L.ksize == 1 && L.pad == 0))) {
                    set_error("layer %s: only 3x3/pad 1 and 1x1/pad 0 convolutions are supported",
                              L.name.c_str());
                    return STX_ERR_UNSUPPORTED;
                }
                if (e->blob_index.count(L.top)) {
                    set_error("layer %s: top blob '%s' already exists", L.name.c_str(), L.top.c_str());
                    return STX_ERR_UNSUPPORTED;
                }
                L.top_blob = add_blob(L.top, L.num_output, i);
                if (!joined) {
                    ConvParams &cp = e->sh->conv[i];
                    cp.cin = e->blobs[L.bottom_blob].channels;
                    cp.cout = L.num_output;
                    cp.ks = L.ksize;
                }
            } else if (L.type == STX_LAYER_POOL) {
                if (L.ksize != 2 || L.stride != 2 ||
                    (L.pool_mode != STX_POOL_MAX && L.pool_mode != STX_POOL_AVE)) {
                    set_error("layer %s: only 2x2 stride-2 MAX/AVE pooling is supported",
                              L.name.c_str());
                    return STX_ERR_UNSUPPORTED;
                }
                if (e->blob_index.count(L.top)) {
                    set_error("layer %s: top blob '%s' already exists", L.name.c_str(), L.top.c_str());
                    return STX_ERR_UNSUPPORTED;
                }
                L.top_blob = add_blob(L.top, e->blobs[L.bottom_blob].channels, i);
            } else {
                set_error("layer %s: unsupported type %d", L.name.c_str(), L.type);
                return STX_ERR_UNSUPPORTED;
            }
        }
        e->layer_index[L.name] = i;
        e->layers.push_back(std::move(L));
    }
    {
        std::vector<int> h224(e->blobs.size(), 224);
        for (size_t li = 1; li < e->layers.size(); ++li) {
            const Layer &L = e->layers[li];
            if (L.type == STX_LAYER_CONV) h224[L.top_blob] = h224[L.bottom_blob];
            if (L.type == STX_LAYER_POOL) h224[L.top_blob] = pooled_len(h224[L.bottom_blob]);
        }
        for (size_t bi = 0; bi < e->blobs.size(); ++bi) e->blobs[bi].scale = 224 / h224[bi];
    }
    enable_peer_access(device);
    STX_HIP(hipStreamCreateWithFlags(&e->stream, hipStreamNonBlocking));
    for (int i = 0; i < stx_engine::kTimed; ++i) {
        STX_HIP(hipEventCreate(&e->ev_start[i]));
        STX_HIP(hipEventCreate(&e->ev_stop[i]));
    }
    STX_HIP(hipEventCreate(&e->ev_tune0));
    STX_HIP(hipEventCreate(&e->ev_tune1));
    if (const char *env = sw_env("STX_AUTOTUNE")) e->autotune = atoi(env) != 0;
    if (const char *env = sw_env("STX_POOL_CODES")) e->pool_codes = atoi(env) != 0;
    if (const char *env = sw_env("STX_WINOGRAD")) e->winograd = atoi(env) != 0;
    e->scalars_cap = kScalarFloats;
    for (stx_engine::ScalarArena &a : e->arena) {
        STX_TRY(a.scalars.ensure(e->scalars_cap * sizeof(float)));
        STX_HIP(hipHostMalloc(reinterpret_cast<void **>(&a.host), e->scalars_cap * sizeof(float),
                              hipHostMallocDefault));
        STX_TRY(a.dscalars.ensure(e->dscalars_cap * sizeof(double)));
        STX_HIP(hipHostMalloc(reinterpret_cast<void **>(&a.dhost), e->dscalars_cap * sizeof(double),
                              hipHostMallocDefault));
        STX_HIP(hipEventCreateWithFlags(&a.fence, hipEventDisableTiming));
    }
    STX_TRY(e->red_scratch.ensure(9 * kBlocks * sizeof(float)));
    {
        std::lock_guard<std::mutex> lock(e->sh->mutex);
        e->sh->members.push_back(e.get());
    }
    *out = e.release();
    return STX_OK;
}

extern "C" {

int stx_engine_create(int device, const stx_layer_desc *layers, int n_layers, stx_engine **out) {
    return build_engine(device, layers, n_layers, nullptr, out);
}

int stx_engine_create_shared(stx_engine *primary, stx_engine **out) {
    if (!primary || !out) {
        set_error("stx_engine_create_shared: bad arguments");
        return STX_ERR_ARG;
    }
    std::vector<stx_layer_desc> descs(primary->layers.size());
    for (size_t i = 0; i < descs.size(); ++i) {
        const Layer &L = primary->layers[i];
        stx_layer_desc &d = descs[i];
        d.name = L.name.c_str();
        d.type = L.type;
        d.bottom = L.bottom.empty() ? nullptr : L.bottom.c_str();
        d.top = L.top.c_str();
        d.num_output = i == 0 ? primary->blobs[L.top_blob].channels : L.num_output;
        d.kernel_size = L.ksize;
        d.pad = L.pad;
        d.stride = L.stride;
        d.pool_mode = L.pool_mode;
    }
    STX_TRY(primary->set_device());
    for (stx_engine *m : primary->sh->members) STX_HIP(hipStreamSynchronize(m->stream));
    return build_engine(primary->device, descs.data(), (int)descs.size(), primary->sh, out);
}

void stx_engine_destroy(stx_engine *e) {
    if (!e) return;
    (void)hipSetDevice(e->device);
    if (e->stream) (void)hipStreamSynchronize(e->stream);
    for (auto &b : e->sgrad) b->release();
    e->marks_buf.release();
    e->amax.release();
    e->audit_buf.release();
    for (Blob &b : e->blobs) {
        b.data.release();
        b.diff.release();
        b.codes.release();
        b.relu_codes.release();
    }
    for (hipEvent_t ev : e->fence_events) (void)hipEventDestroy(ev);
    bool last;
    {
        std::lock_guard<std::mutex> lock(e->sh->mutex);
        auto &m = e->sh->members;
        m.erase(std::remove(m.begin(), m.end(), e), m.end());
        last = m.empty();
    }
    if (last) {
        for (auto &kv : e->sh->conv) {
            kv.second.w.release();
            kv.second.b.release();
            for (auto &p : kv.second.packed) p.second->release();
        }
        clear_all_targets(*e->sh);
    }
    DevBuf *bufs[] = {&e->selfsim_io, &e->swd_work, &e->swd_io, &e->nnfm_scratch, &e->stat_scratch, &e->masked_feat, &e->masked_target, &e->splitk, &e->gram_partials, &e->gram, &e->dsym, &e->dsym_pieces, &e->symm_partials,
                      &e->upload, &e->red_scratch, &e->swt_scratch, &e->lap_scratch, &e->first_gram, &e->color_sums};
    for (DevBuf *b : bufs) b->release();
    for (stx_engine::SwtTable &t : e->swt_tables) t.taps.release();
    for (stx_engine::ScalarArena &a : e->arena) {
        a.scalars.release();
        a.dscalars.release();
        if (a.host) (void)hipHostFree(a.host);
        if (a.dhost) (void)hipHostFree(a.dhost);
        if (a.fence) (void)hipEventDestroy(a.fence);
    }
    for (auto &pe : e->prof) {
        (void)hipEventDestroy(pe.start);
        (void)hipEventDestroy(pe.stop);
    }
    for (hipEvent_t ev : e->event_pool) (void)hipEventDestroy(ev);
    for (int i = 0; i < stx_engine::kTimed; ++i) {
        if (e->ev_start[i]) (void)hipEventDestroy(e->ev_start[i]);
        if (e->ev_stop[i]) (void)hipEventDestroy(e->ev_stop[i]);
    }
    if (e->ev_tune0) (void)hipEventDestroy(e->ev_tune0);
    if (e->ev_tune1) (void)hipEventDestroy(e->ev_tune1);
    if (e->stream) (void)hipStreamDestroy(e->stream);
    delete e;
}

int stx_set_conv_weights(stx_engine *e, const char *conv_layer, const float *weights,
                         const float *bias, int mem) {
    if (!e || !conv_layer || !weights) return STX_ERR_ARG;
    STX_TRY(e->set_device());
    auto it = e->layer_index.find(conv_layer);
    if (it == e->layer_index.end() || e->layers[it->second].type != STX_LAYER_CONV) {
        set_error("stx_set_conv_weights: '%s' is not a convolution layer", conv_layer);
        return STX_ERR_ARG;
    }
    std::lock_guard<std::mutex> lock(e->sh->mutex);
    const bool shared = e->sh->members.size() > 1;
    if (shared) STX_TRY(quiesce_members(e));
    ConvParams &cp = e->sh->conv[it->second];
    const size_t nw = (size_t)cp.cout * cp.cin * cp.ks * cp.ks;
    STX_TRY(cp.w.ensure(nw * sizeof(float)));
    STX_TRY(cp.b.ensure((size_t)cp.cout * sizeof(float)));
    STX_TRY(copy_in(e, cp.w.ptr, weights, mem, nw * sizeof(float)));
    if (bias)
        STX_TRY(copy_in(e, cp.b.ptr, bias, mem, (size_t)cp.cout * sizeof(float)));
    else
        STX_HIP(hipMemsetAsync(cp.b.ptr, 0, (size_t)cp.cout * sizeof(float), e->stream));
    if (mem == STX_HOST || shared) STX_HIP(hipStreamSynchronize(e->stream));
    for (auto &p : cp.packed) p.second->release();
    cp.packed.clear();
    cp.set = true;
    return STX_OK;
}

int stx_sync(stx_engine *e) {
    if (!e) return STX_ERR_ARG;
    STX_TRY(e->set_device());
    return do_sync(e);
}

int stx_fence(stx_engine *e, unsigned long long *ticket) {
    if (!e || !ticket) return STX_ERR_ARG;
    STX_TRY(e->set_device());
    stx_engine::ScalarArena &a = e->A();
    STX_HIP(hipEventRecord(a.fence, e->stream));
    a.ticket = e->next_ticket++;
    *ticket = a.ticket;
    e->cur ^= 1;
    stx_engine::ScalarArena &b = e->A();
    if (b.ticket) {
        STX_HIP(hipEventSynchronize(b.fence));
        publish_arena(b);
    }
    return STX_OK;
}

int stx_fence_wait(stx_engine *e, unsigned long long ticket) {
    if (!e) return STX_ERR_ARG;
    STX_TRY(e->set_device());
    for (stx_engine::ScalarArena &a : e->arena) {
        if (a.ticket && a.ticket == ticket) {
            STX_HIP(hipEventSynchronize(a.fence));
            publish_arena(a);
        }
    }
    return STX_OK;
}

int stx_engine_device(stx_engine *e, int *device) {
    if (!e || !device) return STX_ERR_ARG;
    *device = e->device;
    return STX_OK;
}

int stx_engine_stream(stx_engine *e, void **hip_stream) {
    if (!e || !hip_stream) return STX_ERR_ARG;
    *hip_stream = e->stream;
    return STX_OK;
}

int stx_engine_wait(stx_engine *e, stx_engine *other) {
    if (!e || !other) return STX_ERR_ARG;
    if (e == other) return STX_OK;
    constexpr size_t kRing = 16;
    STX_TRY(other->set_device());
    if (other->fence_events.size() < kRing) {
        hipEvent_t ev;
        STX_HIP(hipEventCreateWithFlags(&ev, hipEventDisableTiming));
        other->fence_events.push_back(ev);
        other->fence_next = other->fence_events.size() - 1;
    }
    hipEvent_t ev = other->fence_events[other->fence_next];
    other->fence_next = (other->fence_next + 1) % kRing;
    STX_HIP(hipEventRecord(ev, other->stream));
    STX_TRY(e->set_device());
    STX_HIP(hipStreamWaitEvent(e->stream, ev, 0));
    return STX_OK;
}

int stx_engine_query(stx_engine *e, int what, double *value) {
    if (!e || !value) return STX_ERR_ARG;
    std::lock_guard<std::mutex> lock(e->sh->mutex);
    switch (what) {
        case STX_Q_SHARED_ENGINES: *value = (double)e->sh->members.size(); break;
        case STX_Q_TARGET_UPLOADS: *value = (double)e->sh->target_uploads; break;
        case STX_Q_TARGET_BYTES: *value = e->sh->target_bytes; break;
        case STX_Q_WEIGHT_BYTES: {
            double b = 0;
            for (auto &kv : e->sh->conv) {
                b += (double)kv.second.w.bytes + (double)kv.second.b.bytes;
                for (auto &p : kv.second.packed) b += (double)p.second->bytes;
            }
            *value = b;
            break;
        }
        case STX_Q_TILE_EVALS: *value = (double)e->n_tile_evals; break;
        case STX_Q_PEERS_WITHOUT_ACCESS: *value = (double)peers_without_access(e->device); break;
        case STX_Q_TILE_IO_DIRECT: *value = (double)e->n_tile_io_direct; break;
        case STX_Q_INJECT_SPECIALISED: *value = (double)e->n_inject_specialised; break;
        case STX_Q_INJECT_VARIANTS: *value = (double)e->inject_variants; break;
        default:
            set_error("stx_engine_query: unknown item %d", what);
            return STX_ERR_ARG;
    }
    return STX_OK;
}

int stx_malloc(stx_engine *e, size_t bytes, void **dev_ptr) {
    if (!e || !dev_ptr) return STX_ERR_ARG;
    STX_TRY(e->set_device());
    hipError_t err = hipMalloc(dev_ptr, bytes ? bytes : 4);
    if (err != hipSuccess) {
        set_error("hipMalloc(%zu): %s", bytes, hipGetErrorString(err));
        return STX_ERR_NOMEM;
    }
    return STX_OK;
}

int stx_free(stx_engine *e, void *dev_ptr) {
    if (!e) return STX_ERR_ARG;
    STX_TRY(e->set_device());
    if (dev_ptr) STX_HIP(hipFree(dev_ptr));
    return STX_OK;
}

int stx_memset_async(stx_engine *e, void *dev_ptr, int value, size_t bytes) {
    if (!e || !dev_ptr) return STX_ERR_ARG;
    STX_TRY(e->set_device());
    STX_HIP(hipMemsetAsync(dev_ptr, value, bytes, e->stream));
    return STX_OK;
}

int stx_memcpy_async(stx_engine *e, void *dst, int dst_mem, const void *src, int src_mem,
                     size_t bytes) {
    if (!e || !dst || !src) return STX_ERR_ARG;
    STX_TRY(e->set_device());
    hipMemcpyKind kind = hipMemcpyDefault;
    if (dst_mem == STX_HOST && src_mem == STX_HOST) kind = hipMemcpyHostToHost;
    if (dst_mem == STX_HOST && src_mem == STX_DEVICE) kind = hipMemcpyDeviceToHost;
    if (dst_mem == STX_DEVICE && src_mem == STX_HOST) kind = hipMemcpyHostToDevice;
    STX_HIP(hipMemcpyAsync(dst, src, bytes, kind, e->stream));
    return STX_OK;
}

int stx_profile_enable(stx_engine *e, int on) {
    if (!e) return STX_ERR_ARG;
    STX_TRY(e->set_device());
    STX_HIP(hipStreamSynchronize(e->stream));
    for (auto &pe : e->prof) {
        e->event_pool.push_back(pe.start);
        e->event_pool.push_back(pe.stop);
    }
    e->prof.clear();
    e->profiling = on != 0;
    return STX_OK;
}

int stx_profile_read(stx_engine *e, char *buf, size_t buf_len, size_t *needed) {
    if (!e || (!buf && buf_len)) return STX_ERR_ARG;
    STX_TRY(e->set_device());
    STX_HIP(hipStreamSynchronize(e->stream));
    std::string out;
    std::vector<long long> marks((size_t)e->marks_used * 2);
    if (!marks.empty())
        STX_HIP(hipMemcpy(marks.data(), e->marks_buf.ptr, marks.size() * sizeof(long long), hipMemcpyDeviceToHost));
    for (auto &pe : e->prof) {
        float ms = 0.f;
        STX_HIP(hipEventElapsedTime(&ms, pe.start, pe.stop));
        double mhz = 0.0;
        if (pe.mark >= 0 && (size_t)pe.mark * 2 + 1 < marks.size() && marks[2 * pe.mark + 1] > 0)
            mhz = (double)marks[2 * pe.mark] / (double)marks[2 * pe.mark + 1] * 100.0;
        char line[256];
        snprintf(line, sizeof line, "%s\t%.6f\t%.6e\t%.1f\n", pe.label.c_str(), ms, pe.flops, mhz);
        out += line;
        e->event_pool.push_back(pe.start);
        e->event_pool.push_back(pe.stop);
    }
    e->prof.clear();
    if (needed) *needed = out.size() + 1;
    if (buf_len) {
        const size_t n = std::min(buf_len - 1, out.size());
        memcpy(buf, out.data(), n);
        buf[n] = 0;
    }
    return STX_OK;
}

int stx_amax_audit(stx_engine *e, int on) {
    if (!e) return STX_ERR_ARG;
    STX_TRY(e->set_device());
    STX_HIP(hipStreamSynchronize(e->stream));
    e->audit.clear();
    e->amax_audit = false;
    if (on)
        STX_TRY(e->audit_buf.ensure(kMaxAmaxAudit * 2 * kAmaxSlots * sizeof(unsigned)));
    else
        e->audit_buf.release();
    e->amax_audit = on != 0;
    return STX_OK;
}

int stx_amax_audit_read(stx_engine *e, char *buf, size_t buf_len, size_t *needed) {
    if (!e || (!buf && buf_len)) return STX_ERR_ARG;
    STX_TRY(e->set_device());
    STX_HIP(hipStreamSynchronize(e->stream));
    std::string out;
    std::vector<unsigned> words(e->audit.size() * 2 * kAmaxSlots);
    if (!words.empty())
        STX_HIP(hipMemcpy(words.data(), e->audit_buf.ptr, words.size() * sizeof(unsigned), hipMemcpyDeviceToHost));
    for (size_t i = 0; i < e->audit.size(); ++i) {
        const stx_engine::AuditEntry &a = e->audit[i];
        const unsigned *rec = words.data() + 2 * i * kAmaxSlots, *meas = rec + kAmaxSlots;
        const unsigned recorded = *std::max_element(rec, rec + kAmaxSlots);
        const unsigned measured = *std::max_element(meas, meas + kAmaxSlots);
        char line[256];
        snprintf(line, sizeof line, "%s\t%s\t%s\t%s\t%08x\t%08x\n", a.consumer.c_str(), a.blob.c_str(),
                 a.diff ? "diff" : "data", a.source.c_str(), recorded, measured);
        out += line;
    }
    e->audit.clear();
    if (needed) *needed = out.size() + 1;
    if (buf_len) {
        const size_t n = std::min(buf_len - 1, out.size());
        memcpy(buf, out.data(), n);
        buf[n] = 0;
    }
    return STX_OK;
}

int stx_last_tile_ms(stx_engine *e, float *ms) {
    if (!e || !ms) return STX_ERR_ARG;
    if (!e->timed) {
        set_error("stx_last_tile_ms: no tile has been evaluated");
        return STX_ERR_STATE;
    }
    STX_TRY(e->set_device());
    int pick = e->ev_cur;
    for (int k = 0; k < e->ev_recorded; ++k) {
        const int i = (e->ev_cur - k + stx_engine::kTimed) % stx_engine::kTimed;
        const hipError_t q = hipEventQuery(e->ev_stop[i]);
        if (q == hipSuccess) {
            pick = i;
            break;
        }
        (void)hipGetLastError();
    }
    STX_HIP(hipEventSynchronize(e->ev_stop[pick]));
    STX_HIP(hipEventElapsedTime(ms, e->ev_start[pick], e->ev_stop[pick]));
    return STX_OK;
}

int stx_clock_marks(stx_engine *e, int on) {
    if (!e) return STX_ERR_ARG;
// ... 35 lines not shown
```

style_transfer_amd/csrc/engine.h:

```cpp
#pragma once

#include <deque>
#include <map>
#include <memory>
#include <mutex>
#include <string>
#include <vector>

#include "common.h"

namespace stx {

struct DevBuf {
    void *ptr = nullptr;
    size_t bytes = 0;
    int ensure(size_t need) {
        if (need <= bytes) return STX_OK;
        if (ptr) STX_HIP(hipFree(ptr));
        ptr = nullptr;
        bytes = 0;
        const size_t want = (need + 255) & ~(size_t)255;
        hipError_t err = hipMalloc(&ptr, want);
        if (err != hipSuccess) {
            set_error("hipMalloc(%zu bytes) failed: %s", want, hipGetErrorString(err));
            ptr = nullptr;
            return STX_ERR_NOMEM;
        }
        bytes = want;
        return STX_OK;
    }
    void release() {
        if (ptr) (void)hipFree(ptr);
        ptr = nullptr;
        bytes = 0;
    }
    float *f() const { return static_cast<float *>(ptr); }
};

struct Layer {
    std::string name, bottom, top;
    int type = 0, num_output = 0, ksize = 0, pad = 0, stride = 1, pool_mode = 0;
    int bottom_blob = -1, top_blob = -1;
};

struct Blob {
    std::string name;
    int channels = 0;
    int producer = -1;
    bool relu = false;
    int scale = 1;
    int h = 0, w = 0;
    DevBuf data, diff;
    DevBuf codes;
    bool codes_valid = false;
    DevBuf relu_codes;
    bool relu_codes_valid = false;
    bool relu_codes_wanted = false;
    int amax_data = -1, amax_diff = -1;
    size_t count() const { return (size_t)channels * h * w; }
};

struct ConvParams {
    int cin = 0, cout = 0, ks = 0;
    DevBuf w, b;
    bool set = false;
    std::map<int, std::unique_ptr<DevBuf>> packed;
};

struct ContentTarget {
    int index, blob, C, h, w;
    std::unique_ptr<DevBuf> feat;
    void release() { feat->release(); }
};

struct StyleTarget {
    int index, blob, C;
    std::unique_ptr<DevBuf> gram;
    void release() { gram->release(); }
};

struct StyleMask {
    int index, blob, h, w;
    std::unique_ptr<DevBuf> map;
    void release() { map->release(); }
};

struct ContentMask {
    int blob, h, w;
    std::unique_ptr<DevBuf> map;
    void release() { map->release(); }
};

struct StatTarget {
    int blob, C;
    double weight;
    std::unique_ptr<DevBuf> ms;
    void release() { ms->release(); }
};

struct NnfmTarget {
    int blob, C, rows;
    double weight;
    std::unique_ptr<DevBuf> bank, pieces;
    int patch = 1, k = 1;
    float cover = 0.f;
    NnfmSegments segs{};
    int mh = 0, mw = 0;
    std::unique_ptr<DevBuf> maps;
    const unsigned short *pieces_hi_lo() const { return static_cast<const unsigned short *>(pieces->ptr); }
    void release() {
        bank->release();
        pieces->release();
        if (maps) maps->release();
    }
};

struct SwdTarget {
    int blob, C, D, Q;
    double weight;
    std::unique_ptr<DevBuf> vt;
    const float *V() const { return vt->f(); }
    const float *Tq() const { return vt->f() + (size_t)D * C; }
    void release() { vt->release(); }
};

struct SelfsimTarget {
    int blob, points;
    double weight;
    void release() {}
};

struct LossTerm {
    size_t scalar_index;
    double coef;
};

struct PendingLoss {
    double *out;
    std::vector<LossTerm> terms;
    std::vector<LossTerm> dterms;
};

struct SharedState {
    std::map<int, ConvParams> conv;
    std::vector<ContentTarget> contents;
    std::vector<StyleTarget> styles;
    std::vector<StyleMask> masks;
    std::vector<StatTarget> stats;
    std::vector<ContentMask> cmasks;
    std::vector<NnfmTarget> nnfms;
    std::vector<SwdTarget> swds;
    std::vector<SelfsimTarget> selfsims;
    int n_contents = 0, n_styles = 0;
    std::vector<stx_engine *> members;
    std::mutex mutex;
    size_t target_uploads = 0;
    double target_bytes = 0;
};

}

using namespace stx;

struct stx_engine {
    int device = 0;
    hipStream_t stream = nullptr;
    bool clock_marks = false;
    DevBuf marks_buf;
    int marks_used = 0, last_mark = -1;
    std::vector<std::unique_ptr<DevBuf>> sgrad;
    static constexpr int kTimed = 4;
    hipEvent_t ev_start[kTimed] = {}, ev_stop[kTimed] = {};
    int ev_cur = 0;
    int ev_recorded = 0;
    hipEvent_t ev_tune0 = nullptr, ev_tune1 = nullptr;
    bool timed = false;
    double flop_algorithmic = 0, flop_issued = 0;
    std::vector<Layer> layers;
    std::vector<Blob> blobs;
    std::map<std::string, int> blob_index, layer_index;
    std::shared_ptr<SharedState> sh;

    DevBuf splitk;
    DevBuf amax;
    unsigned *amax_slots(int blob, bool diff) const {
        return static_cast<unsigned *>(amax.ptr) + ((size_t)(diff ? blobs.size() : 0) + blob) * kAmaxSlots;
    }
    int amax_ensure() {
        return amax.ensure((2 * blobs.size() + 2) * kAmaxSlots * sizeof(unsigned));
    }
    DevBuf first_gram;
    int first_gram_blob = -1, first_gram_parts = 0;
    bool first_gram_valid = false;
    DevBuf gram_partials, gram, dsym, dsym_pieces, symm_partials, upload;
    DevBuf term_scratch;
    DevBuf masked_feat, masked_target;
    DevBuf stat_scratch;
    DevBuf nnfm_scratch;
    DevBuf swd_work;
    DevBuf swd_io;
    DevBuf selfsim_io;
    struct ScalarArena {
        DevBuf scalars;
        float *host = nullptr;
        size_t used = 0;
        DevBuf dscalars;
        double *dhost = nullptr;
        size_t dused = 0;
        std::vector<PendingLoss> pending;
        hipEvent_t fence = nullptr;
        unsigned long long ticket = 0;
    };
    ScalarArena arena[2];
    int cur = 0;
    unsigned long long next_ticket = 1;
    ScalarArena &A() { return arena[cur]; }
    size_t scalars_cap = 0;
    size_t n_tile_evals = 0;
    size_t n_tile_io_direct = 0;
    size_t n_inject_specialised = 0;
    unsigned inject_variants = 0;
    std::vector<hipEvent_t> fence_events;
    size_t fence_next = 0;
    size_t dscalars_cap = 64;
    DevBuf red_scratch;
    DevBuf color_sums;
    DevBuf swt_scratch;
    struct SwtTable {
        int order, levels, N, ntaps, hl;
        DevBuf taps;
    };
    std::vector<SwtTable> swt_tables;
    DevBuf lap_scratch;

    bool winograd = true;
    bool autotune = true;
    bool pool_codes = true;

    bool profiling = false;
    struct ProfEntry {
        std::string label;
        double flops;
        hipEvent_t start, stop;
        int mark = -1;
    };
    std::vector<ProfEntry> prof;
    std::vector<hipEvent_t> event_pool;

    bool amax_audit = false;
    struct AuditEntry {
        std::string consumer, blob, source;
        bool diff;
    };
    std::vector<AuditEntry> audit;
    DevBuf audit_buf;

    int set_device() {
        STX_HIP(hipSetDevice(device));
        return STX_OK;
    }
    int find_blob(const char *name) const {
        if (!name) return -1;
        auto it = blob_index.find(name);
        return it == blob_index.end() ? -1 : it->second;
    }
};

namespace stx {
#pragma GCC visibility push(hidden)

struct ProfScope {
    stx_engine *e;
    int index = -1;
    hipStream_t stream;
    ProfScope(stx_engine *eng, const std::string &label, double flops, hipStream_t on = nullptr)
        : e(eng), stream(on ? on : eng->stream) {
        if (!e->profiling) return;
        auto take = [&]() {
            hipEvent_t ev = nullptr;
            if (!e->event_pool.empty()) {
                ev = e->event_pool.back();
                e->event_pool.pop_back();
            } else if (hipEventCreate(&ev) != hipSuccess) {
                ev = nullptr;
            }
            return ev;
        };
        stx_engine::ProfEntry pe{label, flops, take(), take()};
        if (!pe.start || !pe.stop) return;
        (void)hipEventRecord(pe.start, stream);
        e->prof.push_back(pe);
        index = (int)e->prof.size() - 1;
    }
    ~ProfScope() {
        if (index < 0) return;
        (void)hipEventRecord(e->prof[index].stop, stream);
        e->prof[index].mark = e->last_mark;
        e->last_mark = -1;
    }
};

constexpr int kMaxClockMarks = 16384;

int alloc_scalars(stx_engine *e, size_t n, size_t *index);
int alloc_dscalars(stx_engine *e, size_t n, size_t *index);
int copy_in(stx_engine *e, void *dst, const void *src, int mem, size_t bytes);
int copy_out(stx_engine *e, void *dst, int mem, const void *src, size_t bytes);
int do_sync(stx_engine *e);
int quiesce_members(stx_engine *e);
template <class T>
inline void clear_targets(std::vector<T> &targets) {
    for (T &t : targets) t.release();
    targets.clear();
}
inline void clear_dependent_targets(SharedState &sh) {
    clear_targets(sh.masks);
    clear_targets(sh.stats);
    clear_targets(sh.cmasks);
    clear_targets(sh.nnfms);
    clear_targets(sh.swds);
    clear_targets(sh.selfsims);
}
inline void clear_all_targets(SharedState &sh) {
    clear_targets(sh.contents);
    clear_targets(sh.styles);
    sh.n_contents = sh.n_styles = 0;
    clear_dependent_targets(sh);
}
ConvProblem conv_fwd_problem(const float *x, float *y, const float *bias, int Cin, int Cout, int H, int W,
                             int ks, int relu);
ConvProblem conv_bwd_problem(const float *dy, float *dx, const float *mask, int Cout, int Cin, int H, int W,
                             int ks);
int attach_splitk(stx_engine *e, const ConvConfig &cfg, ConvProblem &p);
int launch_conv(stx_engine *e, const ConvConfig &cfg, const ConvProblem &problem);
int amax_scratch(stx_engine *e, unsigned **out);
constexpr size_t kMaxAmaxAudit = 2048;
int amax_audit_note(stx_engine *e, hipStream_t stream, const std::string &consumer, const std::string &blob,
                    bool diff, const unsigned *slots, const float *x, size_t n);
struct Tap {
    int blob;
    const stx_tap *t;
};

struct TileCall {
    const float *img;
    int img_mem, th, tw, rx, ry, start[2];
    const stx_tap *taps;
    int n_taps;
    float *grad_out;
    int grad_mem;
};

enum class TermKind { Content, MaskedContent, Style, MaskedStyle, Stat, Nnfm, NnfmGuided, Swd, Selfsim, Dream };
constexpr size_t kNoSlot = ~(size_t)0;
constexpr size_t kResidualScalars = 2 + 2 * 1024;

struct PlannedTerm {
    TermKind kind;
    int tap;
    const float *target, *mask;
    ContentWindow win;
    double coef;
    size_t scalars;
    size_t scratch_off, scratch_len;
    size_t sgrad_off;
    const NnfmTarget *nnfm = nullptr;
    const SwdTarget *swd = nullptr;
    int points = 0;
};

struct TilePlan {
    std::vector<Tap> order;
    std::vector<char> needed;
    std::vector<int> tap_of;
// ... 66 lines not shown
```

style_transfer_amd/csrc/tile_path.cpp:

```cpp

#include <algorithm>
#include <cmath>
#include <cstdlib>

#include "engine.h"

namespace stx {

ConvProblem conv_fwd_problem(const float *x, float *y, const float *bias, int Cin, int Cout, int H, int W,
                             int ks, int relu) {
    ConvProblem p{};
    p.x = x;
    p.y = y;
    p.bias = bias;
    p.K = Cin;
    p.M = Cout;
    p.H = H;
    p.W = W;
    p.ksize = ks;
    p.relu = relu;
    p.epilogue = kEpiForward;
    return p;
}

ConvProblem conv_bwd_problem(const float *dy, float *dx, const float *mask, int Cout, int Cin, int H, int W,
                             int ks) {
    ConvProblem p{};
    p.x = dy;
    p.y = dx;
    p.mask = mask;
    p.K = Cout;
    p.M = Cin;
    p.H = H;
    p.W = W;
    p.ksize = ks;
    p.epilogue = kEpiDgrad;
    return p;
}

static double conv_flops(int K, int M, int H, int W, int ks) {
    return 2.0 * K * M * ks * ks * (double)H * W;
}

static int shape_blobs(stx_engine *e, int th, int tw, const std::vector<char> &needed, bool with_diff) {
    Blob &in = e->blobs[e->layers[0].top_blob];
    in.h = th;
    in.w = tw;
    for (size_t li = 1; li < e->layers.size(); ++li) {
        const Layer &L = e->layers[li];
        if (L.type == STX_LAYER_RELU) continue;
        const Blob &b = e->blobs[L.bottom_blob];
        Blob &t = e->blobs[L.top_blob];
        if (L.type == STX_LAYER_CONV) {
            t.h = b.h;
            t.w = b.w;
        } else {
            t.h = pooled_len(b.h);
            t.w = pooled_len(b.w);
        }
    }
    for (size_t bi = 0; bi < e->blobs.size(); ++bi) {
        if (!needed[bi]) continue;
        Blob &b = e->blobs[bi];
        STX_TRY(b.data.ensure(b.count() * sizeof(float)));
        if (with_diff) STX_TRY(b.diff.ensure(b.count() * sizeof(float)));
    }
    return STX_OK;
}

static void mark_ancestors(const stx_engine *e, int blob, std::vector<char> &needed) {
    while (blob >= 0 && !needed[blob]) {
        needed[blob] = 1;
        const int p = e->blobs[blob].producer;
        if (p <= 0) break;
        blob = e->layers[p].bottom_blob;
    }
}

static int get_bank(stx_engine *e, int layer, const ConvBank &bank, const float **out) {
    std::lock_guard<std::mutex> lock(e->sh->mutex);
    ConvParams &cp = e->sh->conv[layer];
    if (!cp.set) {
        set_error("weights of layer %s were never set", e->layers[layer].name.c_str());
        return STX_ERR_STATE;
    }
    auto it = cp.packed.find(bank.key);
    if (it == cp.packed.end()) {
        std::unique_ptr<DevBuf> buf(new DevBuf);
        STX_TRY(buf->ensure(bank.floats * sizeof(float)));
        STX_TRY(bank.pack(e->stream, cp.w.f(), buf->f()));
        if (e->sh->members.size() > 1) STX_HIP(hipStreamSynchronize(e->stream));
        it = cp.packed.emplace(bank.key, std::move(buf)).first;
    }
    *out = it->second->f();
    return STX_OK;
}

static int get_packed(stx_engine *e, int layer, int dir, const ConvConfig &cfg, const float **out) {
    const ConvParams &cp = e->sh->conv[layer];
    return get_bank(e, layer, conv_bank(cfg, dir, cp.cout, cp.cin, cp.ks), out);
}

static int choose_conv(stx_engine *e, int li, int dir, const ConvProblem &p, ConvConfig *out) {
    const ConvTuner tuner{e->device, e->stream, e->ev_tune0, e->ev_tune1, [=](const ConvConfig &cfg, const float **w) {
                              return get_packed(e, li, dir, cfg, w);
                          }};
    return conv_choose(p, e->winograd, e->autotune ? &tuner : nullptr, out);
}

int attach_splitk(stx_engine *e, const ConvConfig &cfg, ConvProblem &p) {
    const size_t need = conv_splitk_floats(cfg, p);
    if (!need) return STX_OK;
    STX_TRY(e->splitk.ensure(need * sizeof(float)));
    p.splitk_ws = e->splitk.f();
    p.splitk_ws_floats = e->splitk.bytes / sizeof(float);
    return STX_OK;
}

int launch_conv(stx_engine *e, const ConvConfig &cfg, const ConvProblem &problem) {
    ConvProblem p = problem;
    e->last_mark = -1;
    if (e->clock_marks && conv_takes_clock(cfg) && e->marks_used < kMaxClockMarks) {
        e->last_mark = e->marks_used++;
        p.clock_out = static_cast<long long *>(e->marks_buf.ptr) + 2 * (size_t)e->last_mark;
    }
    int var = 0;
    p.variant_out = &var;
    const int rc = conv_dispatch(e->stream, cfg, p, &e->flop_algorithmic, &e->flop_issued);
    if (var) {
        ++e->n_inject_specialised;
        e->inject_variants |= 1u << var;
    }
    return rc;
}

static int amax_for(stx_engine *e, int blob, bool diff, const std::string &consumer, const unsigned **out) {
    Blob &b = e->blobs[blob];
    int &src = diff ? b.amax_diff : b.amax_data;
    if (src < 0) {
        ProfScope scope(e, std::string("absmax ") + b.name, 0.0);
        STX_TRY(absmax_launch(e->stream, diff ? b.diff.f() : b.data.f(), b.count(), e->amax_slots(blob, diff)));
        src = blob;
    } else if (e->amax_audit) {
        STX_TRY(amax_audit_note(e, e->stream, consumer, b.name, diff, e->amax_slots(src, diff),
                                diff ? b.diff.f() : b.data.f(), b.count()));
    }
    *out = e->amax_slots(src, diff);
    return STX_OK;
}

int amax_audit_note(stx_engine *e, hipStream_t stream, const std::string &consumer, const std::string &blob,
                    bool diff, const unsigned *slots, const float *x, size_t n) {
    if (!e->amax_audit) return STX_OK;
    if (e->audit.size() >= kMaxAmaxAudit) {
        set_error("stx_amax_audit: more than %zu hand-offs since the last stx_amax_audit_read", kMaxAmaxAudit);
        return STX_ERR_STATE;
    }
    const size_t group = (size_t)(slots - static_cast<const unsigned *>(e->amax.ptr)) / kAmaxSlots;
    const size_t nb = e->blobs.size();
    const std::string source = group < 2 * nb ? e->blobs[group % nb].name : "(scratch)";
    unsigned *const rec = static_cast<unsigned *>(e->audit_buf.ptr) + 2 * e->audit.size() * kAmaxSlots;
    STX_HIP(hipMemcpyAsync(rec, slots, kAmaxSlots * sizeof(unsigned), hipMemcpyDeviceToDevice, stream));
    STX_TRY(absmax_launch(stream, x, n, rec + kAmaxSlots));
    e->audit.push_back(stx_engine::AuditEntry{consumer, blob, source, diff});
    return STX_OK;
}

int amax_scratch(stx_engine *e, unsigned **out) {
    STX_TRY(e->amax_ensure());
    *out = e->amax_slots((int)e->blobs.size(), true);
    return STX_OK;
}

struct FwdConvPlan {
    bool force_relu;
    const Layer *pool;
    int pool_li;
    bool top_unobserved;
    bool conv_reader;
    bool relu_codes;
};

static FwdConvPlan plan_fwd_conv(const stx_engine *e, size_t li, const std::vector<char> &needed, int relu_blob,
                                 bool relu_codes, const std::vector<char> &observed) {
    const Layer &L = e->layers[li];
    FwdConvPlan plan{L.top_blob == relu_blob, nullptr, -1, false, false, relu_codes};
    int readers = 0;
    for (size_t lj = li + 1; lj < e->layers.size(); ++lj) {
        const Layer &P = e->layers[lj];
        if (P.type == STX_LAYER_RELU || P.bottom_blob != L.top_blob) continue;
        ++readers;
        plan.conv_reader |= P.type == STX_LAYER_CONV && needed[P.top_blob];
        if (!plan.pool && P.type == STX_LAYER_POOL && needed[P.top_blob] && P.ksize == 2 && P.stride == 2 &&
            P.pad == 0 && !e->blobs[P.top_blob].relu && P.top_blob != relu_blob) {
            plan.pool = &P;
            plan.pool_li = (int)lj;
        }
    }
    plan.top_unobserved = plan.pool && !observed[L.top_blob] && L.top_blob != relu_blob && readers == 1;
    return plan;
}

static int run_conv_forward(stx_engine *e, int li, const FwdConvPlan &plan, bool *pooled) {
    const Layer &L = e->layers[li];
    const Layer *const pool = plan.pool;
    Blob &b = e->blobs[L.bottom_blob];
    Blob &t = e->blobs[L.top_blob];
    const ConvParams &cp = e->sh->conv[li];
    ConvProblem p = conv_fwd_problem(b.data.f(), t.data.f(), cp.b.f(), cp.cin, cp.cout, b.h, b.w, cp.ks,
                                     (t.relu || plan.force_relu) ? 1 : 0);
    const double direct = conv_flops(cp.cin, cp.cout, b.h, b.w, cp.ks);
    *pooled = false;
    if (conv_first_usable(cp.cin, cp.cout, cp.ks) && !pool) {
        b.relu_codes_valid = false;
        b.relu_codes_wanted = false;
        t.relu_codes_valid = false;
        unsigned *y_amax = nullptr;
        t.amax_data = -1;
        if (conv_h2_enabled()) {
            y_amax = e->amax_slots(L.top_blob, false);
            t.amax_data = L.top_blob;
        }
        float *gram = nullptr;
        if (L.top_blob == e->first_gram_blob) {
            const int parts = conv_first_workgroups(b.h, b.w);
            STX_TRY(e->first_gram.ensure(((size_t)parts * 64 * 64 + 64 * 64 / 64 + 64) * sizeof(float)));
            gram = e->first_gram.f();
            e->first_gram_parts = parts;
            e->first_gram_valid = true;
        }
        ProfScope scope(e, "fwd " + L.name, direct);
        e->flop_algorithmic += direct;
        e->flop_issued += direct;
        return conv_first_launch(e->stream, p.x, cp.w.f(), cp.b.f(), p.y, cp.cin, b.h, b.w, p.relu, gram, y_amax);
    }
    ConvConfig cfg;
    STX_TRY(choose_conv(e, li, 0, p, &cfg));
    b.relu_codes_wanted = !conv_reads_x_amax(cfg) && !b.relu_codes_valid && plan.relu_codes && b.relu && b.channels <= 128;
    p.wants_codes = b.relu_codes_wanted;
    t.amax_data = -1;
    if (conv_reads_x_amax(cfg)) STX_TRY(amax_for(e, L.bottom_blob, false, "fwd " + L.name, &p.x_amax));
    if (conv_leaves_y_amax(cfg)) {
        p.y_amax = e->amax_slots(L.top_blob, false);
        t.amax_data = L.top_blob;
    }
    STX_TRY(get_packed(e, li, 0, cfg, &p.w));
    STX_TRY(attach_splitk(e, cfg, p));
    if (b.relu_codes_wanted) {
        const size_t bytes = (size_t)b.channels * ((b.h + 1) / 2) * ((b.w + 1) / 2);
        STX_TRY(b.relu_codes.ensure(bytes));
        p.in_codes = static_cast<unsigned char *>(b.relu_codes.ptr);
        b.relu_codes_valid = conv_uses_relu_codes(cfg, p, conv_splitk_factor(cfg, p));
        if (!b.relu_codes_valid) p.in_codes = nullptr;
    }
    if (pool) {
        Blob &pt = e->blobs[pool->top_blob];
        p.pool_out = pt.data.f();
        p.pool_mode = pool->pool_mode;
        pt.codes_valid = false;
        pt.amax_data = -1;
        if (conv_fuses_pool(cfg, p)) {
            *pooled = true;
            pt.amax_data = t.amax_data;
            if (conv_writes_pool_codes(cfg) && e->pool_codes) {
                STX_TRY(pt.codes.ensure(pt.count() + 4));
                p.pool_codes = static_cast<unsigned char *>(pt.codes.ptr);
                pt.codes_valid = true;
                p.skip_y = plan.top_unobserved;
            }
        } else {
            p.pool_out = nullptr;
        }
    }
    t.relu_codes_valid = false;
    if (plan.relu_codes && t.relu && plan.conv_reader && conv_h2_enabled()) {
        const size_t bytes = (size_t)t.channels * ((t.h + 1) / 2) * ((t.w + 1) / 2);
        STX_TRY(t.relu_codes.ensure(bytes));
        p.out_codes = static_cast<unsigned char *>(t.relu_codes.ptr);
        t.relu_codes_valid = conv_writes_out_codes(cfg, p, conv_splitk_factor(cfg, p));
        if (!t.relu_codes_valid) p.out_codes = nullptr;
    }
    ProfScope scope(e, "fwd " + L.name, direct);
    return launch_conv(e, cfg, p);
}

static ConvProblem conv_backward_shape(stx_engine *e, int li) {
    const Layer &L = e->layers[li];
    const Blob &b = e->blobs[L.bottom_blob];
    const ConvParams &cp = e->sh->conv[li];
    return conv_bwd_problem(nullptr, nullptr, nullptr, cp.cout, cp.cin, b.h, b.w, cp.ks);
}

static bool conv_backward_takes_pooled(stx_engine *e, int li) {
    const char *env = sw_env("STX_POOL_BWD_FUSE");
    if (env && atoi(env) == 0) return false;
    const ConvProblem p = conv_backward_shape(e, li);
    ConvConfig cfg;
    return p.ksize == 3 && p.M > 4 && conv_choose(p, e->winograd, nullptr, &cfg) == STX_OK &&
           conv_takes_pooled_input(cfg, p);
}

static bool conv_backward_reads_amax(stx_engine *e, int li) {
    const ConvProblem p = conv_backward_shape(e, li);
    ConvConfig cfg;
    return !(p.ksize == 3 && p.M <= 4) && conv_choose(p, e->winograd, nullptr, &cfg) == STX_OK && conv_reads_x_amax(cfg);
}

static int run_conv_backward(stx_engine *e, int li, const ConvInject *inj, bool *fused, const Layer *pooled) {
    const Layer &L = e->layers[li];
    Blob &b = e->blobs[L.bottom_blob];
    const Blob &t = e->blobs[L.top_blob];
    const ConvParams &cp = e->sh->conv[li];
    ConvProblem p = conv_backward_shape(e, li);
    p.x = t.diff.f();
    p.y = b.diff.f();
    p.mask = b.relu ? b.data.f() : nullptr;
    p.mask_codes = b.relu && b.relu_codes_valid ? static_cast<const unsigned char *>(b.relu_codes.ptr) : nullptr;
    p.wants_codes = b.relu && b.relu_codes_wanted;
    if (cp.ks == 3 && cp.cin <= 4) {
        if (fused) *fused = false;
        const float *packed = nullptr;
        STX_TRY(get_bank(e, li, conv_small_bank(cp.cout, cp.cin), &packed));
        const double direct = conv_flops(cp.cout, cp.cin, b.h, b.w, cp.ks);
        ProfScope scope(e, "bwd " + L.name, direct);
        e->flop_algorithmic += direct;
        e->flop_issued += direct * 4.0 / p.M;
        return conv_small_launch(e->stream, p.x, packed, p.y, p.mask, p.K, p.M, p.H, p.W);
    }
    ConvConfig cfg;
    STX_TRY(choose_conv(e, li, 1, p, &cfg));
    const bool can_fuse = inj && conv_takes_inject(cfg);
    if (fused) *fused = can_fuse;
    if (can_fuse) p.inject = *inj;
    b.amax_diff = -1;
    if (pooled) {
        const Blob &pt = e->blobs[pooled->top_blob];
        if (!conv_takes_pooled_input(cfg, p) || !pt.codes_valid) {
            set_error("run_conv_backward: %s cannot take the gradient of %s pooled", L.name.c_str(), pt.name.c_str());
            return STX_ERR_UNSUPPORTED;
        }
        p.x = pt.diff.f();
        p.pin_codes = static_cast<const unsigned char *>(pt.codes.ptr);
        p.pin_mode = pooled->pool_mode;
        p.pin_mask = t.relu;
        STX_TRY(amax_for(e, pooled->top_blob, true, "bwd " + L.name, &p.x_amax));
    } else if (conv_reads_x_amax(cfg)) {
        STX_TRY(amax_for(e, L.top_blob, true, "bwd " + L.name, &p.x_amax));
    }
    if (conv_leaves_y_amax(cfg)) {
        p.y_amax = e->amax_slots(L.bottom_blob, true);
        b.amax_diff = L.bottom_blob;
    }
    STX_TRY(get_packed(e, li, 1, cfg, &p.w));
    STX_TRY(attach_splitk(e, cfg, p));
    ProfScope scope(e, "bwd " + L.name, conv_flops(cp.cout, cp.cin, b.h, b.w, cp.ks));
    return launch_conv(e, cfg, p);
}

static int begin_timing(stx_engine *e) {
    e->ev_cur = (e->ev_cur + 1) % stx_engine::kTimed;
    STX_HIP(hipEventRecord(e->ev_start[e->ev_cur], e->stream));
    e->flop_algorithmic = e->flop_issued = 0;
    return STX_OK;
}

static int end_timing(stx_engine *e) {
    STX_HIP(hipEventRecord(e->ev_stop[e->ev_cur], e->stream));
    if (e->ev_recorded < stx_engine::kTimed) ++e->ev_recorded;
    e->timed = true;
    return STX_OK;
}

static int sc_grad_prepare(stx_engine *e, const TileCall &c, TilePlan &plan) {
    std::vector<Tap> &order = plan.order;
    const stx_tap *taps = c.taps;
    const int n_taps = c.n_taps;
    const auto tapped = [&](int blob) {
        return std::any_of(order.begin(), order.end(), [=](const Tap &o) { return o.blob == blob; });
    };
    const auto has_statistics = [&](int blob) {
        return std::any_of(e->sh->stats.begin(), e->sh->stats.end(), [=](const StatTarget &t) { return t.blob == blob; }) ||
               std::any_of(e->sh->nnfms.begin(), e->sh->nnfms.end(), [=](const NnfmTarget &t) { return t.blob == blob; }) ||
               std::any_of(e->sh->swds.begin(), e->sh->swds.end(), [=](const SwdTarget &t) { return t.blob == blob; }) ||
               std::any_of(e->sh->selfsims.begin(), e->sh->selfsims.end(),
                           [=](const SelfsimTarget &t) { return t.blob == blob; });
    };
    for (int i = 0; i < n_taps; ++i) {
        const int blob = e->find_blob(taps[i].layer);
        if (blob <= 0) {
            set_error("stx_sc_grad_tile: unknown tap layer '%s'",
                      taps[i].layer ? taps[i].layer : "(null)");
            return STX_ERR_ARG;
        }
        if (tapped(blob)) {
            set_error("stx_sc_grad_tile: layer '%s' is tapped twice", taps[i].layer);
            return STX_ERR_ARG;
        }
        if (!taps[i].is_content && !taps[i].is_style && !taps[i].is_dd && !has_statistics(blob)) continue;
        order.push_back(Tap{blob, &taps[i]});
    }
    for (const StatTarget &st : e->sh->stats) {
        if (tapped(st.blob)) continue;
        stx_tap t{};
        t.layer_weight = 1.0;
        plan.extra.push_back(t);
        order.push_back(Tap{st.blob, &plan.extra.back()});
    }
    for (const NnfmTarget &nt : e->sh->nnfms) {
        if (tapped(nt.blob)) continue;
        stx_tap t{};
        t.layer_weight = 1.0;
        plan.extra.push_back(t);
        order.push_back(Tap{nt.blob, &plan.extra.back()});
    }
    for (const SwdTarget &wt : e->sh->swds) {
        if (tapped(wt.blob)) continue;
        stx_tap t{};
        t.layer_weight = 1.0;
        plan.extra.push_back(t);
        order.push_back(Tap{wt.blob, &plan.extra.back()});
    }
    for (const SelfsimTarget &ft : e->sh->selfsims) {
        if (tapped(ft.blob)) continue;
        stx_tap t{};
        t.layer_weight = 1.0;
        plan.extra.push_back(t);
        order.push_back(Tap{ft.blob, &plan.extra.back()});
    }
    if (order.empty()) {
        set_error("stx_sc_grad_tile: no content, style or Deep-Dream layer");
        return STX_ERR_ARG;
    }
    std::sort(order.begin(), order.end(), [](const Tap &a, const Tap &b) { return a.blob > b.blob; });
    std::vector<char> &needed = plan.needed;
    needed.assign(e->blobs.size(), 0);
    mark_ancestors(e, order[0].blob, needed);
    std::vector<int> &tap_of = plan.tap_of;
    tap_of.assign(e->blobs.size(), -1);
    for (size_t i = 0; i < order.size(); ++i) {
        if (!needed[order[i].blob]) {
            set_error("stx_sc_grad_tile: tapped layers must lie on one path through the network "
                      "('%s' does not feed '%s')", e->blobs[order[i].blob].name.c_str(),
                      e->blobs[order[0].blob].name.c_str());
            return STX_ERR_UNSUPPORTED;
        }
        tap_of[order[i].blob] = (int)i;
    }
    for (const Tap &tp : order) {
        if (tp.t->is_content && e->sh->n_contents == 0) {
            set_error("stx_sc_grad_tile: no content targets set");
            return STX_ERR_STATE;
        }
        if (tp.t->is_style && e->sh->n_styles == 0) {
            set_error("stx_sc_grad_tile: no style targets set");
            return STX_ERR_STATE;
        }
    }
    STX_TRY(shape_blobs(e, c.th, c.tw, needed, true));
    plan.sums_late = !(sw_env("STX_SUMS_LATE") && !atoi(sw_env("STX_SUMS_LATE")));
    plan.interleave = !(sw_env("STX_TERMS_LATE") && atoi(sw_env("STX_TERMS_LATE")));
    return plan_terms(e, c, plan);
}

static int blob_done(TileRun *run, int blob) {
    const int k = run ? run->plan.tap_of[blob] : -1;
    return k >= 0 ? queue_tap_terms(*run, (size_t)k) : STX_OK;
}

static int forward(stx_engine *e, const std::vector<char> &needed, int relu_blob, TileRun *run,
                   bool relu_codes, const std::vector<char> &observed) {
    int pooled_layer = -1;
    STX_TRY(e->amax_ensure());
    STX_HIP(hipMemsetAsync(e->amax_slots(0, false), 0, 2 * e->blobs.size() * kAmaxSlots * sizeof(unsigned), e->stream));
    for (Blob &b : e->blobs) {
        b.amax_data = -1;
        b.relu_codes_valid = false;
    }
    for (size_t li = 1; li < e->layers.size(); ++li) {
        const Layer &L = e->layers[li];
        if (L.type == STX_LAYER_RELU || !needed[L.top_blob]) continue;
        const Blob &b = e->blobs[L.bottom_blob];
        Blob &t = e->blobs[L.top_blob];
        if (L.type == STX_LAYER_CONV) {
            const FwdConvPlan plan = plan_fwd_conv(e, li, needed, relu_blob, relu_codes, observed);
            bool pooled = false;
            STX_TRY(run_conv_forward(e, (int)li, plan, &pooled));
            if (pooled) pooled_layer = plan.pool_li;
            STX_TRY(blob_done(run, L.top_blob));
            if (pooled) STX_TRY(blob_done(run, plan.pool->top_blob));
        } else if ((int)li == pooled_layer) {
            continue;
        } else {
            {
                ProfScope scope(e, "fwd " + L.name, 0.0);
                unsigned char *codes = nullptr;
                t.codes_valid = false;
                if (e->pool_codes) {
                    STX_TRY(t.codes.ensure(t.count() + 4));
                    codes = static_cast<unsigned char *>(t.codes.ptr);
                    t.codes_valid = true;
                }
                STX_TRY(pool_forward_launch(e->stream, b.data.f(), b.channels, b.h, b.w, L.pool_mode,
                                            t.data.f(), codes));
                t.amax_data = b.amax_data;
                if (t.relu || L.top_blob == relu_blob)
                    STX_TRY(relu_inplace_launch(e->stream, t.data.f(), t.count()));
            }
            STX_TRY(blob_done(run, L.top_blob));
        }
    }
    return STX_OK;
}

static int backward_walk(TileRun &run) {
    stx_engine *e = run.e;
    const int data_blob = e->layers[0].top_blob;
    int cur = run.plan.order[0].blob;
    for (Blob &b : e->blobs) b.amax_diff = -1;
    {
        bool written = false;
        STX_TRY(inject_terms(run, 0, written));
        if (!written)
            STX_HIP(hipMemsetAsync(e->blobs[cur].diff.ptr, 0, e->blobs[cur].count() * sizeof(float),
                                   e->stream));
    }
    const Layer *pooled = nullptr;
    while (cur != data_blob) {
        const int li = e->blobs[cur].producer;
        const Layer &L = e->layers[li];
        Blob &bot = e->blobs[L.bottom_blob];
        const Blob &top = e->blobs[cur];
        const int k = run.plan.tap_of[L.bottom_blob];
        bool fused = false;
        if (L.type == STX_LAYER_POOL && top.codes_valid && k < 0 && L.ksize == 2 && L.stride == 2 && L.pad == 0 &&
            e->layers[bot.producer].type == STX_LAYER_CONV && conv_backward_takes_pooled(e, bot.producer)) {
            pooled = &L;
            cur = L.bottom_blob;
            continue;
        }
        if (L.type == STX_LAYER_CONV) {
            ConvInject inj{};
            if (k >= 0 && tap_fusable(run, (size_t)k)) {
                inj = make_inject(run, (size_t)k, bot);
                fused = true;
            }
            STX_TRY(run_conv_backward(e, li, fused ? &inj : nullptr, &fused, pooled));
            pooled = nullptr;
        } else {
            if (top.amax_diff < 0 && e->layers[bot.producer].type == STX_LAYER_CONV &&
                conv_backward_reads_amax(e, bot.producer)) {
                const unsigned *unused;
                STX_TRY(amax_for(e, cur, true, "bwd " + L.name, &unused));
            }
            ProfScope scope(e, "bwd " + L.name, 0.0);
            if (top.codes_valid)
                STX_TRY(pool_backward_codes_launch(
                    e->stream, top.diff.f(), static_cast<const unsigned char *>(top.codes.ptr),
                    bot.channels, bot.h, bot.w, L.pool_mode, bot.relu, bot.diff.f()));
            else
                STX_TRY(pool_backward_launch(e->stream, top.diff.f(), bot.data.f(), bot.channels,
                                             bot.h, bot.w, L.pool_mode, bot.relu, bot.diff.f()));
            bot.amax_diff = top.amax_diff;
        }
        cur = L.bottom_blob;
        if (k >= 0 && !fused) {
            bool written = true;
            STX_HIP(hipMemsetAsync(e->amax_slots(L.bottom_blob, true), 0, kAmaxSlots * sizeof(unsigned), e->stream));
            STX_TRY(inject_terms(run, (size_t)k, written));
        }
    }
    return STX_OK;
}

static void first_gram_setup(stx_engine *e, const TilePlan &plan) {
    const int data_blob = e->layers[0].top_blob;
    e->first_gram_blob = -1;
    e->first_gram_valid = false;
    for (const PlannedTerm &t : plan.terms) {
        const int blob = plan.order[t.tap].blob, pl = e->blobs[blob].producer;
        if (t.kind == TermKind::Style && e->first_gram_blob < 0 && pl > 0 && e->layers[pl].type == STX_LAYER_CONV &&
            e->layers[pl].bottom_blob == data_blob && e->blobs[blob].channels == 64)
            e->first_gram_blob = blob;
    }
}

static int sc_grad_run(stx_engine *e, const TilePlan &plan, PendingLoss &pl) {
    const std::vector<Tap> &order = plan.order;
    TileRun run{e, plan, pl, std::vector<std::vector<Term>>(order.size()), {}};
    while (e->sgrad.size() < order.size()) e->sgrad.emplace_back(new DevBuf);
    for (size_t k = 0; k < order.size(); ++k) STX_TRY(e->sgrad[k]->ensure(plan.sgrad_floats[k] * sizeof(float)));
    STX_TRY(e->term_scratch.ensure(plan.scratch_floats * sizeof(float)));
    STX_TRY(begin_timing(e));
    std::vector<char> observed(e->blobs.size(), 0);
    for (const Tap &tp : order) observed[tp.blob] = 1;
    first_gram_setup(e, plan);
    STX_TRY(forward(e, plan.needed, order[0].blob, plan.interleave ? &run : nullptr, true, observed));
    if (!plan.interleave) {
        for (size_t k = order.size(); k-- > 0;) STX_TRY(queue_tap_terms(run, k));
    }
    if (!run.sum_jobs.empty()) {
        ProfScope scope(e, "sums", 0.0);
        STX_TRY(sum_jobs_launch(e->stream, run.sum_jobs.data(), (int)run.sum_jobs.size()));
    }
    STX_TRY(backward_walk(run));
    STX_TRY(end_timing(e));
    STX_HIP(hipMemcpyAsync(e->A().host, e->A().scalars.ptr, e->A().used * sizeof(float),
                           hipMemcpyDeviceToHost, e->stream));
    return STX_OK;
}

static bool local_device_floats(const stx_engine *e, const void *p, int mem) {
    if (mem == STX_HOST || (reinterpret_cast<uintptr_t>(p) & 3) != 0) return false;
    hipPointerAttribute_t attr{};
    if (hipPointerGetAttributes(&attr, p) != hipSuccess) {
        (void)hipGetLastError();
        return false;
    }
    return attr.type == hipMemoryTypeDevice && attr.device == e->device;
}

static bool ranges_overlap(const void *a, const void *b, size_t bytes) {
    const uintptr_t x = reinterpret_cast<uintptr_t>(a), y = reinterpret_cast<uintptr_t>(b);
    return x < y + bytes && y < x + bytes;
}

static void tile_io_direct(stx_engine *e, const TileCall &c, const TilePlan &plan, bool *in_direct, bool *out_direct) {
    const int data_blob = e->layers[0].top_blob;
    const Blob &in = e->blobs[data_blob];
    const size_t bytes = in.count() * sizeof(float);
// ... 263 lines not shown
```

style_transfer_amd/lib.py:

```python

import ctypes
import os

_HERE = os.path.dirname(os.path.abspath(__file__))
LIB_PATH = os.environ.get('STX_LIB') or os.path.join(_HERE, 'csrc', 'libstx.so')

HOST, DEVICE = 0, 1
LAYER_INPUT, LAYER_CONV, LAYER_RELU, LAYER_POOL = 0, 1, 2, 3
POOL_MAX, POOL_AVE = 0, 1
(Q_SHARED_ENGINES, Q_TARGET_UPLOADS, Q_TARGET_BYTES, Q_WEIGHT_BYTES, Q_TILE_EVALS,
 Q_PEERS_WITHOUT_ACCESS, Q_TILE_IO_DIRECT, Q_INJECT_SPECIALISED, Q_INJECT_VARIANTS) = range(9)

c_float_p = ctypes.POINTER(ctypes.c_float)
c_double_p = ctypes.POINTER(ctypes.c_double)
c_int_p = ctypes.POINTER(ctypes.c_int)


class StxError(RuntimeError):

    def __init__(self, func, code, message):
        super().__init__('%s failed with status %d: %s' % (func, code, message))
        self.code = code


class LayerDesc(ctypes.Structure):
    _fields_ = [('name', ctypes.c_char_p), ('type', ctypes.c_int), ('bottom', ctypes.c_char_p),
                ('top', ctypes.c_char_p), ('num_output', ctypes.c_int),
                ('kernel_size', ctypes.c_int), ('pad', ctypes.c_int), ('stride', ctypes.c_int),
                ('pool_mode', ctypes.c_int)]


class ContentTarget(ctypes.Structure):
    _fields_ = [('content_index', ctypes.c_int), ('layer', ctypes.c_char_p),
                ('channels', ctypes.c_int), ('height', ctypes.c_int), ('width', ctypes.c_int),
                ('features', ctypes.c_void_p), ('mem', ctypes.c_int)]


class StyleTarget(ctypes.Structure):
    _fields_ = [('style_index', ctypes.c_int), ('layer', ctypes.c_char_p),
                ('channels', ctypes.c_int), ('gram', ctypes.c_void_p), ('mem', ctypes.c_int)]


class StyleMask(ctypes.Structure):
    _fields_ = [('style_index', ctypes.c_int), ('H', ctypes.c_int), ('W', ctypes.c_int),
                ('mask', ctypes.c_void_p), ('mem', ctypes.c_int)]


class StatTarget(ctypes.Structure):
    _fields_ = [('layer', ctypes.c_char_p), ('channels', ctypes.c_int), ('mean', ctypes.c_void_p),
                ('sd', ctypes.c_void_p), ('mem', ctypes.c_int), ('weight', ctypes.c_double)]


class NnfmTarget(ctypes.Structure):
    _fields_ = [('layer', ctypes.c_char_p), ('channels', ctypes.c_int), ('rows', ctypes.c_int),
                ('bank', ctypes.c_void_p), ('mem', ctypes.c_int), ('weight', ctypes.c_double)]


class NnfmPatchTarget(ctypes.Structure):
    _fields_ = [('layer', ctypes.c_char_p), ('channels', ctypes.c_int), ('patch', ctypes.c_int),
                ('rows', ctypes.c_int), ('bank', ctypes.c_void_p), ('mem', ctypes.c_int),
                ('weight', ctypes.c_double)]


class NnfmKnnTarget(ctypes.Structure):
    _fields_ = [('layer', ctypes.c_char_p), ('channels', ctypes.c_int), ('patch', ctypes.c_int),
                ('k', ctypes.c_int), ('rows', ctypes.c_int), ('bank', ctypes.c_void_p), ('mem', ctypes.c_int),
                ('weight', ctypes.c_double)]


class NnfmCoverTarget(ctypes.Structure):
    _fields_ = [('layer', ctypes.c_char_p), ('channels', ctypes.c_int), ('patch', ctypes.c_int),
                ('k', ctypes.c_int), ('rows', ctypes.c_int), ('bank', ctypes.c_void_p), ('mem', ctypes.c_int),
                ('weight', ctypes.c_double), ('cover', ctypes.c_float)]


NNFM_MAX_SEGMENTS = 8


class NnfmGuidedTarget(ctypes.Structure):
    _fields_ = [('layer', ctypes.c_char_p), ('channels', ctypes.c_int), ('k', ctypes.c_int),
                ('segments', ctypes.c_int), ('seg_rows', ctypes.POINTER(ctypes.c_int)), ('bank', ctypes.c_void_p),
                ('mem', ctypes.c_int), ('weight', ctypes.c_double)]


class SwdTarget(ctypes.Structure):
    _fields_ = [('layer', ctypes.c_char_p), ('channels', ctypes.c_int), ('dirs', ctypes.c_int),
                ('quantiles', ctypes.c_int), ('V', ctypes.c_void_p), ('Tq', ctypes.c_void_p), ('mem', ctypes.c_int),
                ('weight', ctypes.c_double)]


class SelfsimTarget(ctypes.Structure):
    _fields_ = [('layer', ctypes.c_char_p), ('points', ctypes.c_int), ('weight', ctypes.c_double)]


class Tap(ctypes.Structure):
    _fields_ = [('layer', ctypes.c_char_p), ('layer_weight', ctypes.c_double),
                ('is_content', ctypes.c_int), ('content_weight', ctypes.c_double),
                ('is_style', ctypes.c_int), ('style_weight', ctypes.c_double),
                ('is_dd', ctypes.c_int), ('dd_weight', ctypes.c_double)]


_vp, _i, _sz, _d = ctypes.c_void_p, ctypes.c_int, ctypes.c_size_t, ctypes.c_double
SIGNATURES = {
    'stx_reread_env': [],
    'stx_device_count': [c_int_p],
    'stx_device_name': [_i, ctypes.c_char_p, _sz],
    'stx_engine_create': [_i, ctypes.POINTER(LayerDesc), _i, ctypes.POINTER(_vp)],
    'stx_engine_create_shared': [_vp, ctypes.POINTER(_vp)],
    'stx_engine_wait': [_vp, _vp],
    'stx_engine_query': [_vp, _i, c_double_p],
    'stx_set_conv_weights': [_vp, ctypes.c_char_p, _vp, _vp, _i],
    'stx_sync': [_vp],
    'stx_fence': [_vp, ctypes.POINTER(ctypes.c_ulonglong)],
    'stx_fence_wait': [_vp, ctypes.c_ulonglong],
    'stx_engine_device': [_vp, c_int_p],
    'stx_engine_stream': [_vp, ctypes.POINTER(_vp)],
    'stx_malloc': [_vp, _sz, ctypes.POINTER(_vp)],
    'stx_free': [_vp, _vp],
    'stx_memset_async': [_vp, _vp, _i, _sz],
    'stx_memcpy_async': [_vp, _vp, _i, _vp, _i, _sz],
    'stx_set_contents_and_styles': [_vp, ctypes.POINTER(ContentTarget), _i,
                                    ctypes.POINTER(StyleTarget), _i],
    'stx_set_style_masks': [_vp, ctypes.POINTER(StyleMask), _i],
    'stx_set_stat_targets': [_vp, ctypes.POINTER(StatTarget), _i],
    'stx_set_nnfm_targets': [_vp, ctypes.POINTER(NnfmTarget), _i],
    'stx_set_nnfm_patch_targets': [_vp, ctypes.POINTER(NnfmPatchTarget), _i],
    'stx_set_nnfm_knn_targets': [_vp, ctypes.POINTER(NnfmKnnTarget), _i],
    'stx_set_nnfm_cover_targets': [_vp, ctypes.POINTER(NnfmCoverTarget), _i],
    'stx_set_nnfm_guided_targets': [_vp, ctypes.POINTER(NnfmGuidedTarget), _i, ctypes.POINTER(ctypes.c_void_p), _i, _i,
                                    _i, _i],
    'stx_set_swd_targets': [_vp, ctypes.POINTER(SwdTarget), _i],
    'stx_set_selfsim_targets': [_vp, ctypes.POINTER(SelfsimTarget), _i],
    'stx_set_content_mask': [_vp, _vp, _i, _i, _i],
    'stx_features_tile': [_vp, _vp, _i, _i, _i, ctypes.POINTER(ctypes.c_char_p), _i,
                          ctypes.POINTER(_vp), _i],
    'stx_sc_grad_tile': [_vp, _vp, _i, _i, _i, c_int_p, c_int_p, ctypes.POINTER(Tap), _i,
                         c_double_p, _vp, _i, _i],
    'stx_tile_buffers': [_vp, _i, _i, ctypes.POINTER(_vp), ctypes.POINTER(_vp)],
    'stx_gram_matrix': [_vp, _vp, _i, _i, _i, _vp, _i],
    'stx_feature_stats': [_vp, _vp, _i, _i, _i, _vp, _vp, _i],
    'stx_swd_target': [_vp, _vp, _i, _i, _i, _i, _vp, _i, _i, _vp],
    'stx_nnfm_bank': [_vp, _vp, _i, _i, _i, _i, _i, _vp, _i],
    'stx_nnfm_patch_bank': [_vp, _vp, _i, _i, _i, _i, _i, _i, _vp, _i],
    'stx_image_cut_tile': [_vp, _vp, _i, _i, c_int_p, _i, _i, _i, _i, _vp],
    'stx_image_put_tile': [_vp, _vp, _i, _i, c_int_p, _i, _i, _i, _i, _vp],
    'stx_image_mask_map': [_vp, _vp, _i, _i, _i, _vp],
    'stx_map_place': [_vp, _vp, _i, _i, _i, _i, _i, _vp, _i, _i],
    'stx_map_roll_add': [_vp, _vp, _vp, _i, _i, _i, c_int_p, _d, _d],
    'stx_image_resample': [_vp, _vp, _i, _i, _i, _vp, _i, _i, c_int_p, c_double_p, _i, c_int_p,
                           c_double_p, _i, _i],
    'stx_image_regularizers': [_vp, _vp, _vp, _i, _i, c_float_p, _d, _d, _d, _d, _vp, _d,
                               c_int_p, c_double_p],
    'stx_image_swt_haar': [_vp, _vp, _vp, _i, _i, c_int_p, _d, _d, c_double_p],
    'stx_image_swt_haar_levels': [_vp, _vp, _vp, _i, _i, _i, c_int_p, _d, _d, c_double_p],
    'stx_image_swt_daub_levels': [_vp, _vp, _vp, _i, _i, _i, _i, c_int_p, _d, _d, c_double_p],
    'stx_image_lap_target': [_vp, _vp, _i, _i, _i, c_int_p, _vp],
    'stx_image_lap': [_vp, _vp, _vp, _i, _i, _i, c_int_p, c_double_p, _vp, _d, c_double_p],
    'stx_image_photo': [_vp, _vp, _vp, _vp, _i, _i, _d, _d, c_double_p],
    'stx_adam_step': [_vp, _vp, _vp, _vp, _vp, _vp, _vp, _sz, _d, _d, _d, _d, _d, _d, _d],
    'stx_vec_dot': [_vp, _vp, _vp, _sz, c_double_p],
    'stx_vec_axpy': [_vp, _d, _vp, _vp, _sz],
    'stx_vec_scale': [_vp, _d, _vp, _sz],
    'stx_vec_mean_abs': [_vp, _vp, _sz, c_double_p],
    'stx_vec_dot_async': [_vp, _vp, _vp, _sz, _vp],
# ... 90 lines not shown
```

Baseline: 271.8.

## Pack conv1_1 ReLU signs into bitmasks for the conv1_2 backward mask

The first conv kernel can now emit a packed 1-bit-per-pixel ReLU sign mask, built by OR-ing sign nibbles across wave halves with permlane32_swap. The H2 dgrad kernel for the next layer gets new specialised variants that read this bitmask instead of the full-precision activation blob or nibble codes when applying the ReLU mask. The aim is to cut backward-pass memory traffic on the largest 64-channel layer, at the cost of an extra small store in the forward kernel and many more template instantiations.

```diff
diff --git a/include/stx.h b/include/stx.h
--- a/include/stx.h
+++ b/include/stx.h
@@ -63,7 +63,8 @@
     STX_Q_PEERS_WITHOUT_ACCESS = 5,
     STX_Q_TILE_IO_DIRECT = 6,
     STX_Q_INJECT_SPECIALISED = 7,
-    STX_Q_INJECT_VARIANTS = 8
+    STX_Q_INJECT_VARIANTS = 8,
+    STX_Q_RELU_BITS_LAUNCHES = 9
 } stx_query;
 int stx_engine_query(stx_engine *e, int what, double *value);
 int stx_engine_device(stx_engine *e, int *device);
diff --git a/style_transfer_amd/csrc/common.h b/style_transfer_amd/csrc/common.h
--- a/style_transfer_amd/csrc/common.h
+++ b/style_transfer_amd/csrc/common.h
@@ -131,6 +131,7 @@
     unsigned char *pool_codes = nullptr;
     unsigned char *in_codes = nullptr;
     const unsigned char *mask_codes = nullptr;
+    const unsigned *mask_bits = nullptr;
     unsigned char *out_codes = nullptr;
     bool wants_codes = false;
     bool skip_y = false;
@@ -204,6 +205,7 @@
     unsigned char *out_codes = nullptr;
     unsigned char *in_codes = nullptr;
     const unsigned char *mask_codes = nullptr;
+    const unsigned *mask_bits = nullptr;
     long long *clock_out = nullptr;
     int item_base = 0;
     const unsigned *x_amax = nullptr;
@@ -217,8 +219,10 @@
 
 bool conv_first_usable(int K, int M, int ksize);
 int conv_first_workgroups(int H, int W);
+size_t conv_first_bits_bytes(int H, int W);
 int conv_first_launch(hipStream_t s, const float *x, const float *w_caffe, const float *bias, float *y,
-                      int K, int H, int W, int relu, float *gram_partials, unsigned *y_amax = nullptr);
+                      int K, int H, int W, int relu, float *gram_partials, unsigned *y_amax = nullptr,
+                      unsigned *relu_bits = nullptr);
 
 ConvConfig wino2_config(int geometry = 0);
 int wino2_pick_geometry(int H, int W);
@@ -241,8 +245,9 @@
 size_t h2_packed_floats(int K, int M);
 int h2_pack_weights(hipStream_t s, const float *w_caffe, int Mo, int Ko, int transpose_flip, float *packed);
 int h2_launch(hipStream_t s, const ConvConfig &cfg, const ConvProblem &p, int ksplit);
-enum { kH2Style = 1, kH2Content = 2, kH2MaskNibbles = 4, kH2MaskBlob = 8 };
-int h2_variant(const ConvProblem &p, int pin, bool split);
+enum { kH2Style = 1, kH2Content = 2, kH2MaskNibbles = 4, kH2MaskBlob = 8, kH2MaskBits = 12 };
+int h2_variant(const ConvProblem &p, int pin, bool split, bool bits = false);
+bool h2_reads_relu_bits(const ConvConfig &cfg, const ConvProblem &p, int ksplit);
 int h2_launch_variant(hipStream_t s, const WinoArgs &a, int n_wg, int cfg_id, int pin, int var);
 int h2_splitk_factor(const ConvConfig &cfg, const ConvProblem &p);
 bool h2_fuses_pool(const ConvProblem &p);
@@ -274,6 +279,7 @@
 bool conv_takes_pooled_input(const ConvConfig &cfg, const ConvProblem &p);
 bool conv_uses_relu_codes(const ConvConfig &cfg, const ConvProblem &p, int ksplit);
 bool conv_writes_out_codes(const ConvConfig &cfg, const ConvProblem &p, int ksplit);
+bool conv_reads_relu_bits(const ConvConfig &cfg, const ConvProblem &p, int ksplit);
 
 int pool_forward_launch(hipStream_t s, const float *x, int C, int H, int W, int mode, float *y,
                         unsigned char *codes = nullptr);
diff --git a/style_transfer_amd/csrc/conv_dispatch.cpp b/style_transfer_amd/csrc/conv_dispatch.cpp
--- a/style_transfer_amd/csrc/conv_dispatch.cpp
+++ b/style_transfer_amd/csrc/conv_dispatch.cpp
@@ -182,6 +182,12 @@
     return cfg.family == ConvFamily::Wino2 && wino2_uses_relu_codes(p, ksplit);
 }
 
+bool conv_reads_relu_bits(const ConvConfig &cfg, const ConvProblem &p, int ksplit) {
+    const char *env = sw_env("STX_RELU_BITS"), *codes = sw_env("STX_RELU_CODES");
+    if ((env && atoi(env) == 0) || (codes && atoi(codes) == 0)) return false;
+    return cfg.family == ConvFamily::H2 && h2_reads_relu_bits(cfg, p, ksplit);
+}
+
 bool conv_writes_out_codes(const ConvConfig &cfg, const ConvProblem &p, int ksplit) {
     const char *env = sw_env("STX_RELU_CODES");
     if ((env && atoi(env) == 0) || cfg.family == ConvFamily::Direct) return false;
diff --git a/style_transfer_amd/csrc/conv_first.hip b/style_transfer_amd/csrc/conv_first.hip
--- a/style_transfer_amd/csrc/conv_first.hip
+++ b/style_transfer_amd/csrc/conv_first.hip
@@ -24,6 +24,15 @@
 
 __device__ __forceinline__ int sgpr(int v) { return __builtin_amdgcn_readfirstlane(v); }
 __device__ __forceinline__ void lds_barrier() { asm volatile("s_waitcnt lgkmcnt(0)\n\ts_barrier" ::: "memory"); }
+__device__ __forceinline__ unsigned or_across_halves(unsigned lo, unsigned hi, int half) {
+#if __has_builtin(__builtin_amdgcn_permlane32_swap)
+    const auto r = __builtin_amdgcn_permlane32_swap(lo, hi, false, false);
+    return r[0] | r[1];
+#else
+    const unsigned got = __shfl_xor(half ? lo : hi, 32);
+    return (half ? hi : lo) | got;
+#endif
+}
 
 struct FirstArgs {
     const float *x;
@@ -32,12 +41,13 @@
     float *y;
     float *gram;
     unsigned *y_amax;
+    unsigned *bits;
     int K, H, W, tiles_x, n_tiles, relu, vec_store, strided;
 };
 
 }
 
-template <bool GRAM, int STORE>
+template <bool GRAM, int STORE, bool BITS>
 __global__ __launch_bounds__(kNT, GRAM ? 2 : 3) void conv_first_kernel(FirstArgs a) {
     constexpr int kWork = 2 * kPatch + kTile;
     static_assert(kFM * kFM <= kWork, "the Gram tile must fit the working set");
@@ -120,6 +130,10 @@
     const int y_ch0 = tid >> 5, y_c4 = (tid & 31) * 4;
     const unsigned y_voff = (unsigned)(((size_t)y_ch0 * HW + y_c4) * 4);
     const bool track = a.y_amax != nullptr;
+    const int bw_row = (a.W + 31) >> 5;
+    const __amdgpu_buffer_rsrc_t rb = __builtin_amdgcn_make_buffer_rsrc(
+        a.bits, 0, BITS ? (int)(unsigned)((size_t)kFM * a.H * bw_row * 4) : 0, 0x00020000);
+    const unsigned b_voff = (unsigned)((size_t)lane * a.H * bw_row * 4);
     float amax = 0.f;
     auto segment = [&](int t, int buf, const float (&pin)[kPL], float (&pout)[kPL]) {
         patch_load(t + 2 * grid < t_end ? t + 2 * grid : -1, pout);
@@ -140,6 +154,7 @@
         }
         const bool ragged = x0 + kFP > a.W;
         const int room = a.W - x0 - wave * 32 - 4 * half;
+        unsigned sign[2] = {0u, 0u};
 #pragma unroll
         for (int mb = 0; mb < 2; ++mb)
 #pragma unroll
@@ -155,8 +170,13 @@
                     v.z = 8 * j + 2 < room ? v.z : 0.f, v.w = 8 * j + 3 < room ? v.w : 0.f;
                 }
                 if (track) amax = fmaxf(fmaxf(amax, fmaxf(fabsf(v.x), fabsf(v.y))), fmaxf(fabsf(v.z), fabsf(v.w)));
+                if (BITS)
+                    sign[mb] |= ((v.x > 0.f ? 1u : 0u) | (v.y > 0.f ? 2u : 0u) | (v.z > 0.f ? 4u : 0u) |
+                                 (v.w > 0.f ? 8u : 0u)) << (8 * j);
                 *reinterpret_cast<f32x4 *>(tile + (mb * 32 + l31) * kFLd + wave * 32 + 8 * j + 4 * half) = v;
             }
+        unsigned word = 0u;
+        if (BITS) word = or_across_halves(sign[0] << (4 * half), sign[1] << (4 * half), half);
         lds_barrier();
 
         {
@@ -186,6 +206,9 @@
                 }
             }
         }
+        if (BITS)
+            __builtin_amdgcn_raw_buffer_store_b32(word, rb, x0 + wave * 32 < a.W ? b_voff : kOobY,
+                                                  (unsigned)sgpr((ty * bw_row + (x0 >> 5) + wave) * 4), 0);
         if (GRAM) {
 #pragma unroll
             for (int st = 0; st < 2; ++st) {
@@ -275,8 +298,13 @@
     return (int)std::min<long>(tiles, env ? atoi(env) : 768);
 }
 
+size_t conv_first_bits_bytes(int H, int W) {
+    const double bytes = 4.0 * kFM * (double)H * ceil_div(W, 32);
+    return bytes < 4294967280.0 ? (size_t)bytes : 0;
+}
+
 int conv_first_launch(hipStream_t s, const float *x, const float *w_caffe, const float *bias, float *y,
-                      int K, int H, int W, int relu, float *gram_partials, unsigned *y_amax) {
+                      int K, int H, int W, int relu, float *gram_partials, unsigned *y_amax, unsigned *relu_bits) {
     if (4.0 * K * (double)H * W >= 2147483648.0) {
         set_error("conv_first_launch: a %d x %d plane is beyond the buffer-addressing limit", H, W);
         return STX_ERR_UNSUPPORTED;
@@ -288,6 +316,11 @@
     a.y = y;
     a.gram = gram_partials;
     a.y_amax = y_amax;
+    if (relu_bits && (!relu || !conv_first_bits_bytes(H, W))) {
+        set_error("conv_first_launch: no ReLU row bits for this launch (relu %d, %d x %d)", relu, H, W);
+        return STX_ERR_UNSUPPORTED;
+    }
+    a.bits = relu_bits;
     a.K = K;
     a.H = H;
     a.W = W;
@@ -301,7 +334,11 @@
         a.strided = env && atoi(env) != 0;
     }
     const int store = 4.0 * kFM * (double)H * W >= 4294967280.0 ? 2 : a.vec_store ? 0 : 1;
-#define STX_FIRST(G, S) conv_first_kernel<G, S><<<grid, kNT, 0, s>>>(a)
+#define STX_FIRST(G, S)                                                   \
+    do {                                                                  \
+        if (relu_bits) conv_first_kernel<G, S, true><<<grid, kNT, 0, s>>>(a); \
+        else conv_first_kernel<G, S, false><<<grid, kNT, 0, s>>>(a);      \
+    } while (0)
     if (gram_partials) {
         if (store == 0) STX_FIRST(true, 0);
         else if (store == 1) STX_FIRST(true, 1);
diff --git a/style_transfer_amd/csrc/conv_h2.hip b/style_transfer_amd/csrc/conv_h2.hip
--- a/style_transfer_amd/csrc/conv_h2.hip
+++ b/style_transfer_amd/csrc/conv_h2.hip
@@ -69,10 +69,11 @@
 
 template <int EPI, int MB, int PB, int PIN, int VAR = 0>
 __global__ __launch_bounds__(NT) void conv_h2_kernel(WinoArgs a) {
-    static_assert(VAR == 0 || EPI == kEpiDgradInject, "variants are of the injecting epilogue");
-    static_assert(VAR == 0 || (((VAR & 3) == 1 || (VAR & 3) == 2) && ((VAR >> 2) == 1 || (VAR >> 2) == 2)), "h2_variant's codes");
+    static_assert(VAR == 0 || EPI == kEpiDgradInject || (EPI == kEpiDgrad && VAR == kH2MaskBits), "variants are of the injecting epilogue");
+    static_assert(VAR == 0 || VAR == kH2MaskBits || (((VAR & 3) == 1 || (VAR & 3) == 2) && (VAR >> 2) >= 1 && (VAR >> 2) <= 3), "h2_variant's codes");
     const bool inj_style = VAR ? (VAR & 1) != 0 : a.inj.sgrad != nullptr;
     const bool inj_content = VAR ? (VAR & 2) != 0 : a.inj.content != nullptr;
+    constexpr bool mask_bits = (VAR >> 2) == 3;
     const bool mask_nibbles = VAR ? (VAR >> 2) == 1 : a.mask_codes != nullptr;
     const bool mask_blob = VAR ? (VAR >> 2) == 2 : !a.mask_codes && a.mask;
     using G = Geo<PB>;
@@ -401,6 +402,10 @@
         const_cast<unsigned char *>(a.mask_codes), 0, a.mask_codes ? a.M * cph * cpw : 0, 0x00020000);
     const __amdgpu_buffer_rsrc_t roc = __builtin_amdgcn_make_buffer_rsrc(
         a.out_codes, 0, a.out_codes ? a.M * cph * cpw : 0, 0x00020000);
+    const int brw = (a.W + 31) >> 5;
+    const unsigned BP4 = (unsigned)(a.H * brw) * 4u;
+    const __amdgpu_buffer_rsrc_t rbits = __builtin_amdgcn_make_buffer_rsrc(
+        const_cast<unsigned *>(a.mask_bits), 0, mask_bits && a.mask_bits ? (int)((unsigned)a.M * BP4) : 0, 0x00020000);
     const int M_ = a.M;
     struct LaneRows {
         int yy;
@@ -596,11 +601,25 @@
         };
         float bs[8];
         f32x2 mk[16], sg[16];
-        unsigned mkb[8];
+        unsigned mkb[8], mkw[16];
+        unsigned bsh = 0u, vbit[2] = {kOob, kOob};
+        if (mask_bits) {
+            int ln = lane;
+            asm volatile("" : "+v"(ln));
+            bsh = 2u * (unsigned)(ln & 15);
+#pragma unroll
+            for (int y = 0; y < 2; ++y)
+                if (lr.yy + y < a.H) vbit[y] = (unsigned)(((ln >> 5) * 4 * a.H + lr.yy + y) * brw + (x0 >> 5)) * 4u;
+        }
 #pragma unroll
         for (int n = 0; n < 8; ++n) {
             const int c = chan(n);
             const unsigned so = (unsigned)c * HW4;
+            if (mask_bits && !(STX_H2_SKIP & 16)) {
+#pragma unroll
+                for (int y = 0; y < 2; ++y)
+                    mkw[2 * n + y] = __builtin_amdgcn_raw_buffer_load_b32(rbits, vbit[y], (unsigned)c * BP4, 0);
+            }
             if (EPI == kEpiForward) {
                 bs[n] = a.bias ? __builtin_bit_cast(float, __builtin_amdgcn_raw_buffer_load_b32(
                                                                rbias, (unsigned)half * 16u, (unsigned)c * 4u, 0))
@@ -662,6 +681,10 @@
                             const unsigned nib = mkb[n] >> (2 * y);
                             v[y].x = (nib & 1u) ? v[y].x : 0.f;
                             v[y].y = (nib & 2u) ? v[y].y : 0.f;
+                        } else if (mask_bits && !(STX_H2_SKIP & 16)) {
+                            const unsigned pair = mkw[2 * n + y] >> bsh;
+                            v[y].x = (pair & 1u) ? v[y].x : 0.f;
+                            v[y].y = (pair & 2u) ? v[y].y : 0.f;
                         } else if (mask_blob && !(STX_H2_SKIP & 16)) {
                             v[y].x = mk[2 * n + y].x > 0.f ? v[y].x : 0.f;
                             v[y].y = mk[2 * n + y].y > 0.f ? v[y].y : 0.f;
@@ -780,6 +803,23 @@
     STX_H2_VAR(kH2Style | kH2MaskNibbles, 1 + STX_POOL_AVE)
     STX_H2_VAR(kH2Style | kH2MaskBlob, 1 + STX_POOL_AVE)
 #undef STX_H2_VAR
+#define STX_H2_VAR_BITS(V, P)                                                                                 \
+    if (var == (V) && pin == (P) && cfg_id != 1)                                                              \
+        return cfg_id == 2 ? h2_launch_epi<kEpiDgradInject, 1, 2, P, V>(s, a, n_wg)                           \
+                           : h2_launch_epi<kEpiDgradInject, 1, 1, P, V>(s, a, n_wg);
+    STX_H2_VAR_BITS(kH2Style | kH2MaskBits, 0)
+    STX_H2_VAR_BITS(kH2Content | kH2MaskBits, 0)
+    STX_H2_VAR_BITS(kH2Style | kH2MaskBits, 1 + STX_POOL_MAX)
+    STX_H2_VAR_BITS(kH2Style | kH2MaskBits, 1 + STX_POOL_AVE)
+#undef STX_H2_VAR_BITS
+#define STX_H2_PLAIN_BITS(P)                                                                                  \
+    if (var == kH2MaskBits && pin == (P) && cfg_id != 1)                                                      \
+        return cfg_id == 2 ? h2_launch_epi<kEpiDgrad, 1, 2, P, kH2MaskBits>(s, a, n_wg)                       \
+                           : h2_launch_epi<kEpiDgrad, 1, 1, P, kH2MaskBits>(s, a, n_wg);
+    STX_H2_PLAIN_BITS(0)
+    STX_H2_PLAIN_BITS(1 + STX_POOL_MAX)
+    STX_H2_PLAIN_BITS(1 + STX_POOL_AVE)
+#undef STX_H2_PLAIN_BITS
     set_error("h2_launch_variant: no specialised body %d for a pooled input of kind %d", var, pin);
     return STX_ERR_UNSUPPORTED;
 }
@@ -975,16 +1015,37 @@
 template __global__ void conv_h2_kernel<3, 2, 1, 0, kH2Content | kH2MaskNibbles>(WinoArgs);
 template __global__ void conv_h2_kernel<3, 1, 2, 1, kH2Style | kH2MaskBlob>(WinoArgs);
 template __global__ void conv_h2_kernel<3, 2, 1, 1, kH2Style | kH2MaskNibbles>(WinoArgs);
+template __global__ void conv_h2_kernel<3, 1, 2, 1, kH2Style | kH2MaskBits>(WinoArgs);
+template __global__ void conv_h2_kernel<3, 1, 2, 2, kH2Style | kH2MaskBits>(WinoArgs);
+template __global__ void conv_h2_kernel<3, 1, 2, 0, kH2Style | kH2MaskBits>(WinoArgs);
+template __global__ void conv_h2_kernel<3, 1, 2, 0, kH2Content | kH2MaskBits>(WinoArgs);
+template __global__ void conv_h2_kernel<3, 1, 1, 0, kH2Style | kH2MaskBits>(WinoArgs);
+template __global__ void conv_h2_kernel<3, 1, 1, 0, kH2Content | kH2MaskBits>(WinoArgs);
+template __global__ void conv_h2_kernel<3, 1, 1, 1, kH2Style | kH2MaskBits>(WinoArgs);
+template __global__ void conv_h2_kernel<3, 1, 1, 2, kH2Style | kH2MaskBits>(WinoArgs);
+template __global__ void conv_h2_kernel<1, 1, 1, 0, kH2MaskBits>(WinoArgs);
+template __global__ void conv_h2_kernel<1, 1, 2, 0, kH2MaskBits>(WinoArgs);
+template __global__ void conv_h2_kernel<1, 1, 1, 1, kH2MaskBits>(WinoArgs);
+template __global__ void conv_h2_kernel<1, 1, 2, 1, kH2MaskBits>(WinoArgs);
+template __global__ void conv_h2_kernel<1, 1, 1, 2, kH2MaskBits>(WinoArgs);
+template __global__ void conv_h2_kernel<1, 1, 2, 2, kH2MaskBits>(WinoArgs);
 #else
-int h2_variant(const ConvProblem &p, int pin, bool split) {
+int h2_variant(const ConvProblem &p, int pin, bool split, bool bits) {
     if (split || p.epilogue != kEpiDgrad) return 0;
     const bool style = p.inject.sgrad != nullptr, content = p.inject.content != nullptr;
+    if (!style && !content) return bits ? kH2MaskBits : 0;
     if (style == content) return 0;
-    if (!p.mask_codes && !p.mask) return 0;
+    if (!bits && !p.mask_codes && !p.mask) return 0;
     if (content && pin) return 0;
     const char *env = sw_env("STX_H2_INJECT_GENERIC");
     if (env && atoi(env) != 0) return 0;
-    return (style ? kH2Style : kH2Content) | (p.mask_codes ? kH2MaskNibbles : kH2MaskBlob);
+    return (style ? kH2Style : kH2Content) | (bits ? kH2MaskBits : p.mask_codes ? kH2MaskNibbles : kH2MaskBlob);
+}
+
+bool h2_reads_relu_bits(const ConvConfig &cfg, const ConvProblem &p, int ksplit) {
+    if (p.epilogue != kEpiDgrad || ksplit > 1 || cfg.id == 1 || !h2_usable(p)) return false;
+    if (!p.inject.sgrad && !p.inject.content) return true;
+    return h2_variant(p, p.pin_codes ? 1 + p.pin_mode : 0, false, true) != 0;
 }
 
 int h2_launch(hipStream_t s, const ConvConfig &cfg, const ConvProblem &p, int ksplit) {
@@ -1049,7 +1110,9 @@
     }
     const int epi = split ? kEpiPartial : inject ? kEpiDgradInject : p.epilogue;
     const int pin_kind = pin ? 1 + p.pin_mode : 0;
-    const int var = h2_variant(p, pin_kind, split);
+    const bool bits = p.mask_bits && !split && h2_reads_relu_bits(cfg, p, ksplit);
+    a.mask_bits = bits ? p.mask_bits : nullptr;
+    const int var = h2_variant(p, pin_kind, split, bits);
     if (p.variant_out) *p.variant_out = var;
     if (var) return h2_launch_variant(s, a, n_wg, cfg.id, pin_kind, var);
 #define STX_H2_CASE(E)                                                                   \
diff --git a/style_transfer_amd/csrc/engine.cpp b/style_transfer_amd/csrc/engine.cpp
--- a/style_transfer_amd/csrc/engine.cpp
+++ b/style_transfer_amd/csrc/engine.cpp
@@ -370,6 +370,7 @@
         b.diff.release();
         b.codes.release();
         b.relu_codes.release();
+        b.relu_bits.release();
     }
     for (hipEvent_t ev : e->fence_events) (void)hipEventDestroy(ev);
     bool last;
@@ -527,6 +528,7 @@
         case STX_Q_TILE_IO_DIRECT: *value = (double)e->n_tile_io_direct; break;
         case STX_Q_INJECT_SPECIALISED: *value = (double)e->n_inject_specialised; break;
         case STX_Q_INJECT_VARIANTS: *value = (double)e->inject_variants; break;
+        case STX_Q_RELU_BITS_LAUNCHES: *value = (double)e->n_relu_bits_launches; break;
         default:
             set_error("stx_engine_query: unknown item %d", what);
             return STX_ERR_ARG;
diff --git a/style_transfer_amd/csrc/engine.h b/style_transfer_amd/csrc/engine.h
--- a/style_transfer_amd/csrc/engine.h
+++ b/style_transfer_amd/csrc/engine.h
@@ -56,6 +56,8 @@
     DevBuf relu_codes;
     bool relu_codes_valid = false;
     bool relu_codes_wanted = false;
+    DevBuf relu_bits;
+    bool relu_bits_valid = false;
     int amax_data = -1, amax_diff = -1;
     size_t count() const { return (size_t)channels * h * w; }
 };
@@ -220,6 +222,7 @@
     size_t n_tile_io_direct = 0;
     size_t n_inject_specialised = 0;
     unsigned inject_variants = 0;
+    size_t n_relu_bits_launches = 0;
     std::vector<hipEvent_t> fence_events;
     size_t fence_next = 0;
     size_t dscalars_cap = 64;
diff --git a/style_transfer_amd/csrc/tile_path.cpp b/style_transfer_amd/csrc/tile_path.cpp
--- a/style_transfer_amd/csrc/tile_path.cpp
+++ b/style_transfer_amd/csrc/tile_path.cpp
@@ -127,7 +127,8 @@
     int var = 0;
     p.variant_out = &var;
     const int rc = conv_dispatch(e->stream, cfg, p, &e->flop_algorithmic, &e->flop_issued);
-    if (var) {
+    if ((var & 12) == kH2MaskBits) ++e->n_relu_bits_launches;
+    if (var & 3) {
         ++e->n_inject_specialised;
         e->inject_variants |= 1u << var;
     }
@@ -178,19 +179,23 @@
     int pool_li;
     bool top_unobserved;
     bool conv_reader;
+    int conv_reader_li;
     bool relu_codes;
 };
 
 static FwdConvPlan plan_fwd_conv(const stx_engine *e, size_t li, const std::vector<char> &needed, int relu_blob,
                                  bool relu_codes, const std::vector<char> &observed) {
     const Layer &L = e->layers[li];
-    FwdConvPlan plan{L.top_blob == relu_blob, nullptr, -1, false, false, relu_codes};
+    FwdConvPlan plan{L.top_blob == relu_blob, nullptr, -1, false, false, -1, relu_codes};
     int readers = 0;
     for (size_t lj = li + 1; lj < e->layers.size(); ++lj) {
         const Layer &P = e->layers[lj];
         if (P.type == STX_LAYER_RELU || P.bottom_blob != L.top_blob) continue;
         ++readers;
-        plan.conv_reader |= P.type == STX_LAYER_CONV && needed[P.top_blob];
+        if (P.type == STX_LAYER_CONV && needed[P.top_blob]) {
+            plan.conv_reader = true;
+            if (plan.conv_reader_li < 0) plan.conv_reader_li = (int)lj;
+        }
         if (!plan.pool && P.type == STX_LAYER_POOL && needed[P.top_blob] && P.ksize == 2 && P.stride == 2 &&
             P.pad == 0 && !e->blobs[P.top_blob].relu && P.top_blob != relu_blob) {
             plan.pool = &P;
@@ -199,6 +204,16 @@
     }
     plan.top_unobserved = plan.pool && !observed[L.top_blob] && L.top_blob != relu_blob && readers == 1;
     return plan;
+}
+
+static ConvProblem conv_backward_shape(stx_engine *e, int li);
+
+static bool first_reader_takes_bits(stx_engine *e, int li) {
+    if (li < 0) return false;
+    const ConvProblem p = conv_backward_shape(e, li);
+    ConvConfig cfg;
+    return p.ksize == 3 && p.M > 4 && conv_choose(p, e->winograd, nullptr, &cfg) == STX_OK &&
+           conv_reads_relu_bits(cfg, p, conv_splitk_factor(cfg, p));
 }
 
 static int run_conv_forward(stx_engine *e, int li, const FwdConvPlan &plan, bool *pooled) {
@@ -215,6 +230,16 @@
         b.relu_codes_valid = false;
         b.relu_codes_wanted = false;
         t.relu_codes_valid = false;
+        unsigned *relu_bits = nullptr;
+        t.relu_bits_valid = false;
+        if (plan.relu_codes && t.relu && p.relu && plan.conv_reader && conv_h2_enabled() &&
+            first_reader_takes_bits(e, plan.conv_reader_li)) {
+            if (const size_t bytes = conv_first_bits_bytes(b.h, b.w)) {
+                STX_TRY(t.relu_bits.ensure(bytes));
+                relu_bits = static_cast<unsigned *>(t.relu_bits.ptr);
+                t.relu_bits_valid = true;
+            }
+        }
         unsigned *y_amax = nullptr;
         t.amax_data = -1;
         if (conv_h2_enabled()) {
@@ -232,7 +257,8 @@
         ProfScope scope(e, "fwd " + L.name, direct);
         e->flop_algorithmic += direct;
         e->flop_issued += direct;
-        return conv_first_launch(e->stream, p.x, cp.w.f(), cp.b.f(), p.y, cp.cin, b.h, b.w, p.relu, gram, y_amax);
+        return conv_first_launch(e->stream, p.x, cp.w.f(), cp.b.f(), p.y, cp.cin, b.h, b.w, p.relu, gram, y_amax,
+                                 relu_bits);
     }
     ConvConfig cfg;
     STX_TRY(choose_conv(e, li, 0, p, &cfg));
@@ -353,6 +379,8 @@
     }
     STX_TRY(get_packed(e, li, 1, cfg, &p.w));
     STX_TRY(attach_splitk(e, cfg, p));
+    if (b.relu && b.relu_bits_valid && conv_reads_relu_bits(cfg, p, conv_splitk_factor(cfg, p)))
+        p.mask_bits = static_cast<const unsigned *>(b.relu_bits.ptr);
     ProfScope scope(e, "bwd " + L.name, conv_flops(cp.cout, cp.cin, b.h, b.w, cp.ks));
     return launch_conv(e, cfg, p);
 }
@@ -475,6 +503,7 @@
     for (Blob &b : e->blobs) {
         b.amax_data = -1;
         b.relu_codes_valid = false;
+        b.relu_bits_valid = false;
     }
     for (size_t li = 1; li < e->layers.size(); ++li) {
         const Layer &L = e->layers[li];
diff --git a/style_transfer_amd/lib.py b/style_transfer_amd/lib.py
--- a/style_transfer_amd/lib.py
+++ b/style_transfer_amd/lib.py
@@ -9,7 +9,8 @@
 LAYER_INPUT, LAYER_CONV, LAYER_RELU, LAYER_POOL = 0, 1, 2, 3
 POOL_MAX, POOL_AVE = 0, 1
 (Q_SHARED_ENGINES, Q_TARGET_UPLOADS, Q_TARGET_BYTES, Q_WEIGHT_BYTES, Q_TILE_EVALS,
- Q_PEERS_WITHOUT_ACCESS, Q_TILE_IO_DIRECT, Q_INJECT_SPECIALISED, Q_INJECT_VARIANTS) = range(9)
+ Q_PEERS_WITHOUT_ACCESS, Q_TILE_IO_DIRECT, Q_INJECT_SPECIALISED, Q_INJECT_VARIANTS,
+ Q_RELU_BITS_LAUNCHES) = range(10)
 
 c_float_p = ctypes.POINTER(ctypes.c_float)
 c_double_p = ctypes.POINTER(ctypes.c_double)
```

Measured after the change: 271.1, median of 3. No clear change (-0.3%).
